# lashhw/rtcuda

Measured on AMD Instinct MI355X. Metric: Msamples/s at 1920x1080, bun_zipper.ply, higher is better.
Workload: dtype f32

## Files before the change

### rtcuda_amd/api.py

```python
from __future__ import annotations

import ctypes
import dataclasses
import os
import subprocess

import numpy as np

from .scenes import SceneArrays

_PKG = os.path.dirname(os.path.abspath(__file__))
LIB_PATH = os.path.join(_PKG, os.environ.get("RT_LIB_NAME", "librtcuda_amd.so"))
CSRC = os.path.join(_PKG, "csrc")

W = 1 << 20
FLAG_TIME_KERNELS = 1
FLAG_DETERMINISTIC = 2
FLAG_RNG_PER_SAMPLE = 4
FLAG_REFERENCE_WALK = 8
SCENE_DEVICE_BVH = 1
FLAG_WATERTIGHT = 16
AOV_CHANNELS = 11
AOV_ALBEDO, AOV_NORMAL, AOV_EMISSION, AOV_DEPTH, AOV_HITS = 0, 3, 6, 9, 10

EXPORTS = [
    "rt_scene_create", "rt_scene_destroy", "rt_scene_info", "rt_scene_build_info", "rt_scene_update", "rt_scene_update_device",
    "rt_scene_refit_info", "rt_scene_create_flags", "rt_scene_rebuild", "rt_scene_rebuild_device", "rt_scene_set_materials",
    "rt_scene_set_lights", "rt_scene_set_triangles", "rt_scene_set_triangles_device", "rt_scene_create_device", "rt_camera_make", "rt_render", "rt_render_multi",
    "rt_render_shard", "rt_render_shard_fixed", "rt_render_rays_device", "rt_render_rays_fixed_device",
    "rt_render_rays_keyed_device", "rt_render_rays_keyed_fixed_device", "rt_post_process", "rt_post_process_fixed", "rt_trace_closest", "rt_trace_any",
    "rt_trace_closest_flags", "rt_trace_any_flags", "rt_query_closest_device", "rt_query_any_device", "rt_query_last_counters",
    "rt_render_aov_fixed", "rt_render_aov_rays_fixed_device", "rt_aov_resolve",
    "rt_denoise_scratch_bytes", "rt_denoise_default_params", "rt_denoise_fixed",
    "rt_denoise_dual_scratch_bytes", "rt_denoise_dual_default_params", "rt_denoise_dual_fixed",
    "rt_render_motion", "rt_temporal_default_params", "rt_temporal_accumulate_fixed",
    "rt_temporal_moments_default_params", "rt_temporal_accumulate_moments_fixed", "rt_denoise_variance_fixed",
    "rt_xorwow_states", "rt_shutdown", "rt_peer_access_log", "rt_last_error", "rt_version", "rt_build_id",
]
TOOLS_LIB_PATH = os.path.join(_PKG, "librtcuda_amd_tools.so")
TOOLS_EXPORTS = ["rt_measure_copy_bandwidth", "rt_calibrate_valu", "rt_calibrate_valu_packed", "rt_probe_issue", "rt_split_probe",
                 "rt_scene_tree_copy", "rt_shade_table", "rt_shade_records", "rt_denoise_pass_time",
                 "rt_denoise_dual_pass_time"]


class RtError(RuntimeError):
    pass


class RtStats(ctypes.Structure):
    _fields_ = [
        ("camera_rays", ctypes.c_int64), ("shade_events", ctypes.c_int64), ("closest_rays", ctypes.c_int64),
        ("any_rays", ctypes.c_int64), ("emission_adds", ctypes.c_int64), ("shadow_adds", ctypes.c_int64),
        ("rr_draws", ctypes.c_int64), ("iterations", ctypes.c_int64), ("bvh_nodes", ctypes.c_int64),
        ("bvh_depth", ctypes.c_int64), ("seconds_render", ctypes.c_double), ("seconds_rng_init", ctypes.c_double),
        ("seconds_trace", ctypes.c_double), ("seconds_reference_tree", ctypes.c_double), ("seconds_advance", ctypes.c_double),
        ("launches_trace", ctypes.c_int64), ("reserved", ctypes.c_int64 * 7),
    ]

    def as_dict(self) -> dict:
        d = {n: getattr(self, n) for n, _ in self._fields_ if n != "reserved"}
        d["lds_top_records"] = int(self.reserved[2])
        d["slot_chunk"] = max((int(self.reserved[1]) & 0xffffffff) - 1, 0)
        d["slot_head"] = int(self.reserved[1]) >> 32
        d["literal_retraces"], d["reference_lost_hits"], d["exact_ties"] = (int(self.reserved[k]) for k in (4, 5, 6))
        return d


class RtDenoiseParams(ctypes.Structure):
    _fields_ = [("passes", ctypes.c_int32), ("sigma_color", ctypes.c_float), ("sigma_depth", ctypes.c_float),
                ("normal_power_log2", ctypes.c_int32), ("flags", ctypes.c_uint32)]


class RtDenoiseDualParams(ctypes.Structure):
    _fields_ = [("passes", ctypes.c_int32), ("sigma_variance", ctypes.c_float), ("sigma_depth", ctypes.c_float),
                ("normal_power_log2", ctypes.c_int32), ("flags", ctypes.c_uint32)]


class RtTemporalParams(ctypes.Structure):
    _fields_ = [("max_history", ctypes.c_int32), ("alpha_min", ctypes.c_float), ("depth_tolerance", ctypes.c_float),
                ("normal_cos_min", ctypes.c_float), ("flags", ctypes.c_uint32)]


class RtTemporalMomentsParams(ctypes.Structure):
    _fields_ = [("max_history", ctypes.c_int32), ("alpha_min", ctypes.c_float), ("depth_tolerance", ctypes.c_float),
                ("normal_cos_min", ctypes.c_float), ("emission_tolerance", ctypes.c_float), ("variance_min_history", ctypes.c_int32),
                ("flags", ctypes.c_uint32)]


def build(verbose: bool = False) -> str:
    out = None if verbose else subprocess.DEVNULL
    subprocess.check_call(["make", "-C", CSRC], stdout=out)
    return LIB_PATH


_lib = None


def _preload_hip_runtime() -> None:
    candidates = []
    try:
        import torch
        candidates.append(os.path.join(os.path.dirname(torch.__file__), "lib", "libamdhip64.so"))
    except ImportError:
        pass
    candidates += ["/opt/rocm/lib/libamdhip64.so", "libamdhip64.so"]
    for c in candidates:
        if os.path.isabs(c) and not os.path.exists(c):
            continue
        try:
            ctypes.CDLL(c, mode=ctypes.RTLD_GLOBAL)
            return
        except OSError:
            continue
    raise ImportError("no HIP runtime (libamdhip64.so) could be loaded")


def lib():
    global _lib
    if _lib is not None:
        return _lib
    if not os.path.exists(LIB_PATH):
        raise ImportError(
            f"{LIB_PATH} not found: the HIP library is the product and there is no fallback. "
            f"Build it with `make -C {CSRC}` (or python -c 'import __graft_entry__ as g; g.build()').")
    _preload_hip_runtime()
    _lib = _bind(ctypes.CDLL(LIB_PATH))
    return _lib


def _bind(L):
    vp, ci, cf = ctypes.c_void_p, ctypes.c_int, ctypes.c_float
    L.rt_last_error.restype = ctypes.c_char_p
    L.rt_version.restype = ctypes.c_char_p
    L.rt_build_id.restype = ctypes.c_char_p
    L.rt_scene_create.argtypes = [vp, ci, vp, vp, vp, ci, vp, ci, ctypes.POINTER(vp)]
    L.rt_scene_destroy.argtypes = [vp]
    L.rt_scene_destroy.restype = None
    L.rt_scene_info.argtypes = [vp, vp]
    L.rt_scene_build_info.argtypes = [vp, ctypes.POINTER(ci), ctypes.POINTER(ctypes.c_double)]
    L.rt_scene_update.argtypes = [vp, vp, ci]
    L.rt_scene_update_device.argtypes = [vp, vp, ci, vp]
    L.rt_scene_refit_info.argtypes = [vp, ctypes.POINTER(ctypes.c_int64), ctypes.POINTER(ctypes.c_double),
                                      ctypes.POINTER(ctypes.c_double)]
    L.rt_scene_create_flags.argtypes = [vp, ci, vp, vp, vp, ci, vp, ci, ctypes.c_uint32, ctypes.POINTER(vp)]
    L.rt_scene_rebuild.argtypes = [vp, vp, ci]
    L.rt_scene_rebuild_device.argtypes = [vp, vp, ci, vp]
    L.rt_scene_set_materials.argtypes = [vp, vp, ci]
    L.rt_scene_set_lights.argtypes = [vp, vp, ci, vp]
    L.rt_scene_set_triangles.argtypes = [vp, vp, ci, vp, vp, vp, ci, vp, ci]
    L.rt_scene_set_triangles_device.argtypes = [vp, vp, ci, vp, vp, vp, ci, vp, ci, vp]
    L.rt_scene_create_device.argtypes = [vp, ci, vp, vp, vp, ci, vp, ci, vp, ctypes.POINTER(vp)]
    L.rt_camera_make.argtypes = [vp, vp, vp, cf, cf, vp]
    L.rt_render.argtypes = [vp, vp, ci, ci, ci, ci, ctypes.c_uint64, ctypes.c_uint32, vp, ctypes.POINTER(RtStats)]
    L.rt_render_multi.argtypes = [vp, vp, ci, ci, ci, ci, ctypes.c_uint64, ctypes.c_uint32, vp, ci, vp, ctypes.POINTER(RtStats)]
    L.rt_render_shard.argtypes = [vp, vp, ci, ci, ci, ci, ctypes.c_uint64, ci, ci, ctypes.c_uint32, vp, vp,
                                  ctypes.POINTER(RtStats)]
    L.rt_post_process.argtypes = [vp, ci, ci, vp]
    L.rt_render_shard_fixed.argtypes = L.rt_render_shard.argtypes
    L.rt_post_process_fixed.argtypes = [vp, vp, ci, ci, vp]
    L.rt_render_rays_device.argtypes = [vp, ctypes.c_int64, vp, vp, vp, ci, ci, ci, ctypes.c_uint64, ctypes.c_uint32, vp, vp,
                                        ctypes.POINTER(RtStats)]
    L.rt_render_rays_fixed_device.argtypes = L.rt_render_rays_device.argtypes
    L.rt_render_rays_keyed_device.argtypes = [vp, ctypes.c_int64, vp, vp, vp, ci, ci, ci, ctypes.c_uint64, ctypes.c_uint64, ctypes.c_uint32,
                                              ctypes.c_uint32, vp, vp, ctypes.POINTER(RtStats)]
    L.rt_render_rays_keyed_fixed_device.argtypes = L.rt_render_rays_keyed_device.argtypes
    L.rt_render_aov_fixed.argtypes = [vp, vp, ci, ci, ci, ctypes.c_uint64, ci, ci, ctypes.c_uint32, vp, vp, vp, ctypes.POINTER(RtStats)]
    L.rt_render_aov_rays_fixed_device.argtypes = [vp, ctypes.c_int64, vp, vp, vp, ci, ci, ctypes.c_uint64, ctypes.c_uint32, ctypes.c_uint32,
                                                  vp, vp, vp, ctypes.POINTER(RtStats)]
    L.rt_aov_resolve.argtypes = [vp, vp, ci, ci, vp]
    L.rt_denoise_scratch_bytes.argtypes = [ci, ci]
    L.rt_denoise_scratch_bytes.restype = ctypes.c_int64
    L.rt_denoise_default_params.argtypes = [ctypes.POINTER(RtDenoiseParams)]
    L.rt_denoise_fixed.argtypes = [vp, ci, vp, ci, ci, ci, ctypes.POINTER(RtDenoiseParams), vp, vp, vp]
    L.rt_denoise_dual_scratch_bytes.argtypes = [ci, ci]
    L.rt_denoise_dual_scratch_bytes.restype = ctypes.c_int64
    L.rt_denoise_dual_default_params.argtypes = [ctypes.POINTER(RtDenoiseDualParams)]
    L.rt_denoise_dual_fixed.argtypes = [vp, ci, vp, ci, vp, ci, ci, ci, ctypes.POINTER(RtDenoiseDualParams), vp, vp, vp]
    L.rt_render_motion.argtypes = [vp, vp, ci, ci, vp, vp, ctypes.c_uint32, vp, vp, ctypes.POINTER(RtStats)]
    L.rt_temporal_default_params.argtypes = [ctypes.POINTER(RtTemporalParams)]
    L.rt_temporal_accumulate_fixed.argtypes = [vp, ci, vp, ci, vp, ci, vp, vp, vp, vp, vp, ci, ci, ci, ctypes.POINTER(RtTemporalParams),
                                               vp, vp, vp, vp]
    L.rt_temporal_moments_default_params.argtypes = [ctypes.POINTER(RtTemporalMomentsParams)]
    L.rt_temporal_accumulate_moments_fixed.argtypes = [vp, ci, vp, ci, vp, ci, vp, vp, vp, vp, vp, ci, vp, vp, ci, ci,
                                                       ctypes.POINTER(RtTemporalMomentsParams), vp, vp, vp, vp, vp, vp]
    L.rt_denoise_variance_fixed.argtypes = [vp, ci, vp, vp, ci, ci, ci, ctypes.POINTER(RtDenoiseDualParams), vp, vp, vp]
    L.rt_trace_closest.argtypes = [vp, ci, vp, vp, vp, vp, vp, vp, vp]
    L.rt_trace_any.argtypes = [vp, ci, vp, vp, vp, vp, vp]
    L.rt_trace_closest_flags.argtypes = [vp, ctypes.c_uint32, ci, vp, vp, vp, vp, vp, vp, vp]
    L.rt_trace_any_flags.argtypes = [vp, ctypes.c_uint32, ci, vp, vp, vp, vp, vp]
    L.rt_query_closest_device.argtypes = [vp, ctypes.c_uint32, ci, vp, vp, vp, vp, vp, vp, vp, vp]
    L.rt_query_any_device.argtypes = [vp, ctypes.c_uint32, ci, vp, vp, vp, vp, vp, vp]
    L.rt_query_last_counters.argtypes = [vp, vp]
    L.rt_xorwow_states.argtypes = [ctypes.c_uint64, ctypes.c_uint32, ctypes.c_uint32, ci, vp, vp]
    L.rt_shutdown.restype = None
    L.rt_peer_access_log.restype = ctypes.c_char_p
    return L


_tools = None


def tools_lib():
    global _tools
    if _tools is not None:
        return _tools
    if not os.path.exists(TOOLS_LIB_PATH):
        raise ImportError(f"{TOOLS_LIB_PATH} not found: build it with `make -C {CSRC}`")
    _preload_hip_runtime()
    L = _bind(ctypes.CDLL(TOOLS_LIB_PATH))
    vp, ci = ctypes.c_void_p, ctypes.c_int
    L.rt_measure_copy_bandwidth.argtypes = [ctypes.c_int64, ci, ctypes.POINTER(ctypes.c_double)]
    L.rt_calibrate_valu.argtypes = [ci, ci, ctypes.POINTER(ctypes.c_double), ctypes.POINTER(ctypes.c_double)]
    L.rt_calibrate_valu_packed.argtypes = [ci, ci, ci, ctypes.POINTER(ctypes.c_double)]
    L.rt_probe_issue.argtypes = [ci, ci, ci, ctypes.POINTER(ctypes.c_double), ctypes.POINTER(ctypes.c_double)]
    L.rt_split_probe.argtypes = [vp, vp, ci, ci, ci, ci, ctypes.c_uint64, ctypes.c_int64, vp, ci]
    L.rt_scene_tree_copy.argtypes = [vp, vp, ctypes.c_int64, vp, ctypes.c_int64, vp]
# ... 913 lines not shown
```

### rtcuda_amd/csrc/rt_device.h

```cpp
#ifndef RT_DEVICE_H
#define RT_DEVICE_H

#include <hip/hip_runtime.h>
#include <stdint.h>

#include "rt_pinned_math.h"

#define RT_DEV __device__ __forceinline__
#ifdef RT_ISA_MARKS
#define RT_MARK(name) __asm__ volatile("; RT_MARK " name)
#else
#define RT_MARK(name)
#endif

namespace rt {

constexpr float kInvPi = 0.31830988618379067153f;
constexpr float kTwoPi = 6.28318530717958647692f;
constexpr int kRrStart = 4;
constexpr float kRrThreshold = 1.f;
constexpr float kFltMax = 3.402823466e+38f;
constexpr float kFltEps = 1.192092896e-07f;

struct V3 {
    float x, y, z;
};
RT_DEV V3 mk(float x, float y, float z) { return V3{x, y, z}; }
RT_DEV V3 neg(V3 a) { return mk(-a.x, -a.y, -a.z); }
RT_DEV V3 add(V3 a, V3 b) { return mk(a.x + b.x, a.y + b.y, a.z + b.z); }
RT_DEV V3 sub(V3 a, V3 b) { return mk(a.x - b.x, a.y - b.y, a.z - b.z); }
RT_DEV V3 mul(V3 a, V3 b) { return mk(a.x * b.x, a.y * b.y, a.z * b.z); }
RT_DEV V3 scale(V3 a, float t) { return mk(a.x * t, a.y * t, a.z * t); }
RT_DEV V3 divf(V3 a, float t) {
    float inv_t = 1.f / t;
    return mk(a.x * inv_t, a.y * inv_t, a.z * inv_t);
}
RT_DEV float dot(V3 a, V3 b) { return a.x * b.x + a.y * b.y + a.z * b.z; }
RT_DEV V3 cross(V3 a, V3 b) {
    return mk(a.y * b.z - a.z * b.y, a.z * b.x - a.x * b.z, a.x * b.y - a.y * b.x);
}
RT_DEV float len2(V3 a) { return a.x * a.x + a.y * a.y + a.z * a.z; }
RT_DEV float len(V3 a) { return sqrtf(a.x * a.x + a.y * a.y + a.z * a.z); }
RT_DEV V3 unit(V3 a) {
    float inv_len = 1.f / len(a);
    return mk(a.x * inv_len, a.y * inv_len, a.z * inv_len);
}
RT_DEV float max3(V3 a) { return fmaxf(fmaxf(a.x, a.y), a.z); }
template <int STEPS = 1>
RT_DEV float rcp_exact_normal(float x) {
    float r = __builtin_amdgcn_rcpf(x);
#pragma unroll
    for (int k = 0; k < STEPS; k++) {
        const float e = fmaf(-x, r, 1.f);
        r = fmaf(e, r, r);
    }
    return r;
}
RT_DEV V3 reflect(V3 v, V3 n) { return sub(v, scale(n, 2.f * dot(v, n))); }
RT_DEV V3 refract4(V3 unit_v, V3 unit_n, float eta_ratio, float cos_theta) {
    V3 v_parallel = scale(add(unit_v, scale(unit_n, cos_theta)), eta_ratio);
    V3 v_perp = scale(unit_n, -sqrtf(1.f - len2(v_parallel)));
    return add(v_parallel, v_perp);
}

struct Rng {
    uint32_t d, v0, v1, v2, v3, v4;
};
RT_DEV uint32_t rng_next(Rng &s) {
    uint32_t t = s.v0 ^ (s.v0 >> 2);
    s.v0 = s.v1;
    s.v1 = s.v2;
    s.v2 = s.v3;
    s.v3 = s.v4;
    s.v4 = (s.v4 ^ (s.v4 << 4)) ^ (t ^ (t << 1));
    s.d += 362437u;
    return s.v4 + s.d;
}
RT_DEV Rng rng_sample_stream(uint32_t seed_lo, uint32_t seed_hi, unsigned long long key) {
    unsigned long long z = (((unsigned long long)seed_hi << 32) | seed_lo) + 0x9E3779B97F4A7C15ull * (key + 1ull);
    z = (z ^ (z >> 30)) * 0xBF58476D1CE4E5B9ull;
    z = (z ^ (z >> 27)) * 0x94D049BB133111EBull;
    z ^= z >> 31;
    const uint32_t s0 = (uint32_t)z ^ 0xaad26b49u, s1 = (uint32_t)(z >> 32) ^ 0xf7dcefddu;
    const uint32_t t0 = 1099087573u * s0, t1 = 2591861531u * s1;
    Rng r;
    r.d = 6615241u + t1 + t0;
    r.v0 = 123456789u + t0;
    r.v1 = 362436069u ^ t0;
    r.v2 = 521288629u + t1;
    r.v3 = 88675123u ^ t1;
    r.v4 = 5783321u + t0;
    return r;
}
RT_DEV float rng_uniform(Rng &s) { return (float)rng_next(s) * 2.3283064e-10f + (2.3283064e-10f / 2.0f); }

struct Tri {
    V3 p0, e1, e2, n;
};
RT_DEV Tri load_tri(const float4 *__restrict__ tris, int k) {
    const float4 *q = (const float4 *)((const char *)tris + __umul24((unsigned)k, 48u));
    float4 a = q[0];
    float4 b = q[1];
    float4 c = q[2];
    Tri t;
    t.p0 = mk(a.x, a.y, a.z);
    t.e1 = mk(a.w, b.x, b.y);
    t.e2 = mk(b.z, b.w, c.x);
    t.n = mk(c.y, c.z, c.w);
    return t;
}
RT_DEV bool tri_intersect(const Tri &tr, V3 o, V3 d, float tmax, float &t_out, float &u_out, float &v_out) {
    V3 c = sub(tr.p0, o);
    V3 r = cross(d, c);
    float inv_det = 1.f / dot(d, tr.n);
    float u = inv_det * dot(tr.e2, r);
    float v = inv_det * dot(tr.e1, r);
    float t = inv_det * dot(c, tr.n);
    t_out = t;
    u_out = u;
    v_out = v;
    return u >= 0.0f && v >= 0.0f && (u + v) <= 1.0f && 0 < t && t <= tmax;
}
RT_DEV V3 tri_point(const Tri &tr, float u, float v) { return add(sub(tr.p0, scale(tr.e1, u)), scale(tr.e2, v)); }
RT_DEV float tri_area(const Tri &tr) { return 0.5f * len(tr.n); }

RT_DEV V3 offset_ray_origin(V3 p, V3 n) {
    const float int_scale = 256.f;
    const float float_scale = 1.f / 65536.f;
    const float origin = 1.f / 32.f;
    int ox = (int)(int_scale * n.x);
    int oy = (int)(int_scale * n.y);
    int oz = (int)(int_scale * n.z);
    float px = __int_as_float(__float_as_int(p.x) + (p.x < 0 ? -ox : ox));
    float py = __int_as_float(__float_as_int(p.y) + (p.y < 0 ? -oy : oy));
    float pz = __int_as_float(__float_as_int(p.z) + (p.z < 0 ? -oz : oz));
    return mk(fabsf(p.x) < origin ? p.x + float_scale * n.x : px,
              fabsf(p.y) < origin ? p.y + float_scale * n.y : py,
              fabsf(p.z) < origin ? p.z + float_scale * n.z : pz);
}
RT_DEV float power_heuristic(float f_pdf, float g_pdf_float) {
    int g = (int)g_pdf_float;
    float f2 = f_pdf * f_pdf;
    return f2 / (f2 + (float)(g * g));
}
RT_DEV bool same_hemisphere(V3 wo, V3 wi, V3 n) { return dot(wo, n) * dot(wi, n) < 0.f; }
RT_DEV V3 uniform_sample_sphere(Rng &rs) {
    float z = 1 - 2 * rng_uniform(rs);
    float r = sqrtf(1 - z * z);
    float phi = kTwoPi * rng_uniform(rs);
    float x, y;
    rt_sincosf(phi, &y, &x);
    return mk(r * x, r * y, z);
}

struct Material {
    float ax, ay, az;
    float ior;
    int type;
};
RT_DEV bool mat_get_f(const Material &m, V3 wo, V3 wi, V3 n, V3 &f, float &pdf) {
    if (m.type == 0) {
        if (same_hemisphere(wo, wi, n)) {
            f = scale(mk(m.ax, m.ay, m.az), kInvPi);
            pdf = dot(wi, n) * kInvPi;
            return true;
        }
    }
    return false;
}
RT_DEV V3 mat_sample_f(const Material &m, V3 wo, Rng &rs, V3 &n, V3 &wi, float &pdf, int &again_draws) {
    again_draws = 0;
    if (m.type == 0 || m.type == 1) {
        if (dot(wo, n) > 0.f) n = neg(n);
        if (m.type == 0) {
            again_draws = 2;
            wi = unit(add(n, uniform_sample_sphere(rs)));
            pdf = dot(wi, n) * kInvPi;
            return scale(mk(m.ax, m.ay, m.az), kInvPi);
        } else {
            wi = reflect(wo, n);
            pdf = 1.f;
            return divf(mk(m.ax, m.ay, m.az), dot(wi, n));
        }
    } else {
        float cos_theta = dot(wo, n);
        bool front = cos_theta < 0.f;
        if (front) cos_theta = -cos_theta;
        float inv_cos = 1.f / cos_theta;
        float eta = front ? 1.f / m.ior : m.ior;
        float sin_theta = sqrtf(1.f - cos_theta * cos_theta);
        bool cannot_refract = eta * sin_theta > 1.f;
        if (cannot_refract) {
            if (!front) n = neg(n);
            wi = reflect(wo, n);
            pdf = 1.f;
            return mk(inv_cos, inv_cos, inv_cos);
        }
        again_draws = 1;
        float r0 = (1 - m.ior) / (1 + m.ior);
        r0 = r0 * r0;
        float reflectance = r0 + (1 - r0) * rt_pow5f(1 - cos_theta);
        if (rng_uniform(rs) < reflectance) {
            if (!front) n = neg(n);
            wi = reflect(wo, n);
            pdf = reflectance;
            float v = pdf * inv_cos;
            return mk(v, v, v);
        } else {
            if (!front) n = neg(n);
            wi = refract4(wo, n, eta, cos_theta);
            n = neg(n);
            pdf = 1.f - reflectance;
            float v = pdf * eta * eta / dot(wi, n);
            return mk(v, v, v);
        }
    }
}
struct Light {
    int type;
    float px, py, pz;
    int tri;
    float lx, ly, lz;
};

struct Camera {
    V3 lookfrom, upper_left, horizontal, vertical;
};
RT_DEV void camera_get_ray(const Camera &c, float x, float y, V3 &o, V3 &d) {
    V3 dir = sub(add(add(c.upper_left, scale(c.horizontal, x)), scale(c.vertical, y)), c.lookfrom);
    o = c.lookfrom;
    d = unit(dir);
}

}
#endif
```

### rtcuda_amd/csrc/rt_frame_kernels.inc

```
#ifndef RT_CHUNK_RELEASE_WAIT
#define RT_CHUNK_RELEASE_WAIT 1
#endif

template <bool LDS_TABLES>
__global__ void __launch_bounds__(kBlock)
RT_K_ADVANCE(DScene sc, DPools p, RT_FRAME_SRC cam, AdvanceParams ap, float *__restrict__ fb, DCounters *__restrict__ ctr,
             DWaveRow *__restrict__ rows, unsigned int *__restrict__ lock_shades) {
    if (ap.lockstep >= 3 && lock_shades[ap.lockstep - 2] == 0u) return;
    __shared__ float s_tab[LDS_TABLES ? kTabDwordsMax : 1];
    const int i = blockIdx.x * blockDim.x + threadIdx.x;
    const bool in_range = i < ap.n;
    SlotState st;
    st.bounces = kDone;
    st.hit_info = -1;
    st.pixel = 0;
    st.gen = 0;
    st.rs = Rng{0, 0, 0, 0, 0, 0};
    st.beta = st.wo = st.isect_p = st.isect_n = mk(0, 0, 0);
    if (in_range) {
        st.bounces = p.bounces(i);
        st.hit_info = p.hit_info(i);
        st.pixel = p.pixel(i);
        st.gen = p.gen(i);
        st.rs = Rng{p.rd(i), p.r0(i), p.r1(i), p.r2(i), p.r3(i), p.r4(i)};
// ... 80 lines not shown
    }
}

template <bool LDS_TABLES, bool WIDE, int MIN_WAVES, bool DRAW_CIDS = false, bool LITERAL = false, bool VERIFY = false>
__global__ void __launch_bounds__(kBlock, MIN_WAVES)
RT_K_PATHS(DScene sc, DPools p, RT_FRAME_SRC cam_arg, AdvanceParams ap_arg, float *__restrict__ fb, DWaveRow *__restrict__ rows,
           int stack_cap, int *overflow, int adv_batch, int debug_no_deposit, unsigned long long *prof, int top_n,
           int prio_period, int rot_wave, int rot_set, int gen_batch, int tri_follow, unsigned int *__restrict__ next_cid,
           unsigned long long *__restrict__ vstat) {
    constexpr bool SPLIT_GEN = MIN_WAVES != 2;
    asm volatile("s_nop 0\n\ts_nop 0");
    extern __shared__ int s_lds[];
    int *stack = s_lds + threadIdx.x;
    float *park = (float *)(s_lds + (stack_cap + 1) * kBlock) + threadIdx.x;
    int *over = overflow + (blockIdx.x * kBlock + threadIdx.x) % kOverStride;
    int *cold = s_lds + (stack_cap + 10) * kBlock + threadIdx.x;
    float *acc = (float *)(s_lds + (stack_cap + 23) * kBlock) + threadIdx.x;
    float *s_tab = (float *)(s_lds + (stack_cap + 26) * kBlock);
    const float *tab = sc.tables;
    const float4 *s_top = (const float4 *)(s_tab + (LDS_TABLES ? ((sc.tab_dwords + 3) & ~3) : 0));
    constexpr bool CHUNKS = RT_PATHS_CHUNKS && SPLIT_GEN && !DRAW_CIDS;
    __shared__ __attribute__((aligned(16))) unsigned s_task[CHUNKS ? 8 : 1];
    __shared__ unsigned s_sem[CHUNKS ? rtchunks::kSemWords : 1];
    const unsigned chunk_g0 = (CHUNKS && top_n > 0) ? (unsigned)top_n & ((1u << rtplan::kChunkHeadShift) - 1u) : 0u;
    const unsigned chunk_head0 = (CHUNKS && top_n > 0) ? (unsigned)top_n >> rtplan::kChunkHeadShift : 0u;
    if (CHUNKS) {
        for (unsigned k = threadIdx.x; k < rtchunks::kSemWords; k += kBlock) s_sem[k] = rtchunks::kSemWordInit;
        if (threadIdx.x == 0) {
            const rtchunks::Multiple m = rtchunks::multiple_of(chunk_g0 ? chunk_g0 : 1u);
            s_task[0] = 0u;
            s_task[1] = chunk_g0;
            s_task[2] = m.inv;
            s_task[3] = m.shift;
            s_task[4] = m.limit;
            s_task[5] = chunk_head0;
        }
    }
    const bool chunk_start = CHUNKS && chunk_g0 && chunk_head0 == 0u;
    if (MIN_WAVES != 2) top_n = 0;
    for (int k = threadIdx.x; k < top_n * 4; k += kBlock) ((float4 *)s_top)[k] = sc.nodes[k];
    if (LDS_TABLES) {
        for (int k = threadIdx.x; k < sc.tab_dwords; k += kBlock) s_tab[k] = sc.tables[k];
        tab = s_tab;
    }
    struct Uniforms {
        RT_FRAME_SRC cam;
        AdvanceParams ap;
    };
    static_assert(sizeof(Uniforms) % 4 == 0, "dword copy");
    Uniforms *s_uni = (Uniforms *)(s_top + 4 * (size_t)top_n);
    {
        Uniforms u;
        u.cam = cam_arg;
        u.ap = ap_arg;
        const int *srcw = (const int *)&u;
        for (int k = threadIdx.x; k < (int)(sizeof(Uniforms) / 4); k += kBlock) ((int *)s_uni)[k] = srcw[k];
    }
    __syncthreads();
    const RT_FRAME_SRC &cam = s_uni->cam;
    const AdvanceParams &ap = s_uni->ap;
    const int ap_n = ap_arg.n, ap_max_bounces = ap_arg.max_bounces, ap_fb_fixed = ap_arg.fb_fixed;
    constexpr bool draw_cids = DRAW_CIDS && SPLIT_GEN;
    int cid_next = 0, cid_end = 0;
    const int lanes_in_grid = (int)(gridDim.x * blockDim.x);
    auto slot_of = [&](int set, unsigned lane_in_wg) {
        return rtchunks::slot_of((unsigned)set, blockIdx.x * blockDim.x + lane_in_wg, (unsigned)lanes_in_grid, (unsigned)rot_wave, (unsigned)rot_set);
    };
    int slot_set = 0;
    int i = slot_of(0, threadIdx.x);
    int bounces = kDone, pixel = 0, gen = 0;
    Rng rs{0, 0, 0, 0, 0, 0};
    V3 beta = mk(0, 0, 0);
    auto load_slot = [&](int k) {
        bounces = p.bounces(k);
        pixel = p.pixel(k);
        gen = p.gen(k);
        rs = Rng{p.rd(k), p.r0(k), p.r1(k), p.r2(k), p.r3(k), p.r4(k)};
        beta = mk(p.br(k), p.bg(k), p.bb(k));
    };
    auto store_slot = [&](int k) {
        p.bounces(k) = bounces;
        p.pixel(k) = pixel;
        p.gen(k) = gen;
        p.hit_info(k) = -1;
        p.stmax(k) = -1.f;
        p.br(k) = beta.x;
        p.bg(k) = beta.y;
        p.bb(k) = beta.z;
        p.rd(k) = rs.d;
        p.r0(k) = rs.v0;
        p.r1(k) = rs.v1;
        p.r2(k) = rs.v2;
        p.r3(k) = rs.v3;
        p.r4(k) = rs.v4;
    };
    auto cold_save = [&]() {
        cold[0 * kBlock] = bounces;
        cold[1 * kBlock] = pixel;
        cold[2 * kBlock] = gen;
        cold[3 * kBlock] = (int)rs.d;
        cold[4 * kBlock] = (int)rs.v0;
        cold[5 * kBlock] = (int)rs.v1;
        cold[6 * kBlock] = (int)rs.v2;
        cold[7 * kBlock] = (int)rs.v3;
        cold[8 * kBlock] = (int)rs.v4;
        cold[9 * kBlock] = __float_as_int(beta.x);
        cold[10 * kBlock] = __float_as_int(beta.y);
        cold[11 * kBlock] = __float_as_int(beta.z);
    };
    auto cold_load = [&]() {
        bounces = cold[0 * kBlock];
        pixel = cold[1 * kBlock];
        gen = cold[2 * kBlock];
        rs = Rng{(uint32_t)cold[3 * kBlock], (uint32_t)cold[4 * kBlock], (uint32_t)cold[5 * kBlock],
                 (uint32_t)cold[6 * kBlock], (uint32_t)cold[7 * kBlock], (uint32_t)cold[8 * kBlock]};
        beta = mk(__int_as_float(cold[9 * kBlock]), __int_as_float(cold[10 * kBlock]), __int_as_float(cold[11 * kBlock]));
    };
    int phase = PH_IDLE;
    int tri = -1;
    V3 o = mk(0, 0, 0), d = mk(0, 0, 0), inv = mk(0, 0, 0);
    float tmax = 0.f, hu = 0.f, hv = 0.f;
    int cur = kEntryDone, sp = 0;
    auto next_slot = [&](int first_phase) {
        cold_load();
        store_slot(i);
        phase = PH_IDLE;
        tri = -1;
        slot_set++;
        i = slot_of(slot_set, threadIdx.x);
        if (i < ap_n) {
            load_slot(i);
            if (bounces != kDone && bounces != kParked) {
                phase = first_phase;
                cold_save();
                cold[12 * kBlock] = -1;
            } else {
                i = ap_n;
            }
        }
    };
    int pend = kEntryDone;
    acc[0 * kBlock] = acc[1 * kBlock] = acc[2 * kBlock] = 0.f;
    if (chunk_start) {
        i = ap_n;
        phase = PH_GEN;
        cold[12 * kBlock] = -1;
    } else if (i < ap_n) {
        load_slot(i);
        phase = (bounces != kDone && bounces != kParked) ? (SPLIT_GEN ? PH_GEN : PH_ADV) : PH_IDLE;
        cold_save();
        cold[12 * kBlock] = -1;
    }
    unsigned long long n_gen = 0, n_shade = 0, n_traced = 0, n_shadow = 0, n_emit = 0, n_deposit = 0, n_rr = 0;
#ifdef RT_TRACE_PROFILE
    unsigned long long pf[16] = {0, 0, 0, 0, 0, 0, 0, 0, 0, 0, 0, 0, 0, 0, 0, 0};
    unsigned long long pf_gen_cycles = 0, pf_fin_cycles = 0, pf_fin_lanes = 0, pf_fin_iters = 0;
    unsigned long long pf_handovers = 0, pf_handover_blocks = 0;
    const unsigned long long pf_t0 = __builtin_readcyclecounter();
    unsigned long long pf_last_work = 0;
#endif

    unsigned prio_tick = 0;
    const unsigned prio_rank = (4u * blockIdx.x) / gridDim.x;
    while (true) {
        RT_MARK("loop.head");
        if (prio_period && (prio_tick++ & ((1u << prio_period) - 1u)) == 0u) {
            unsigned lvl = ((prio_tick >> prio_period) + prio_rank) & 3u;
            lvl = max(lvl, prio_rank >> 1);
            switch (lvl) {
                case 0: __builtin_amdgcn_s_setprio(0); break;
                case 1: __builtin_amdgcn_s_setprio(1); break;
                case 2: __builtin_amdgcn_s_setprio(2); break;
                default: __builtin_amdgcn_s_setprio(3); break;
            }
        }
        bool trav = phase == PH_ANY || phase == PH_CLOSEST;
        bool want_node = trav && cur >= 0;
        bool want_tri = trav && ((cur != kEntryDone && cur < 0) || (kSpeculate && pend != kEntryDone));
        int n_adv = wave_count((phase == PH_ADV));
        const int n_genw = wave_count((phase == PH_GEN));
        int n_node = wave_count((want_node));
        int n_tri = wave_count((want_tri));
        if (n_adv + n_genw + n_node + n_tri == 0) break;
        auto retake = [&]() {
            trav = phase == PH_ANY || phase == PH_CLOSEST;
            want_node = trav && cur >= 0;
            want_tri = trav && ((cur != kEntryDone && cur < 0) || (kSpeculate && pend != kEntryDone));
            n_adv = wave_count((phase == PH_ADV));
            n_node = wave_count((want_node));
            n_tri = wave_count((want_tri));
        };
        const bool run_adv = n_adv > 0 && ((n_adv >= adv_batch && 2 * n_adv >= n_node && 2 * n_adv >= n_tri) || n_node + n_tri == 0);
        if (SPLIT_GEN && !run_adv && n_genw > 0 && (n_genw >= gen_batch || n_node + n_tri == 0)) {
            RT_MARK("gen.begin");
#ifdef RT_TRACE_PROFILE
            pf[12]++; pf[15] += n_genw;
            const unsigned long long pf_tg = __builtin_readcyclecounter();
#endif
            AdvanceOut out;
            out.did_gen = out.new_ray = false;
            out.ray_o = o;
            out.ray_d = d;
            bool hand_back = false;
            long long my_cid = -1;
            if (draw_cids) {
                const unsigned long long m = wave_ballot(phase == PH_GEN);
                const int need = (int)__popcll(m), rank = (int)prefix_popc(m);
                int served = 0;
                while (served < need) {
                    if (cid_next == cid_end) {
                        unsigned base = 0;
                        if (lane_id() == 0) base = atomicAdd(next_cid, (unsigned)kCidChunk);
                        static_assert(0x7ffff000u + (unsigned)kCidChunk < 0x7fffffffu, "cid_end must not overflow int");
                        cid_next = (int)min(__builtin_amdgcn_readfirstlane(base), 0x7ffff000u);
                        cid_end = cid_next + kCidChunk;
                    }
                    const int take = min(need - served, cid_end - cid_next);
                    if (phase == PH_GEN && rank >= served && rank < served + take) my_cid = cid_next + (rank - served);
                    cid_next += take;
                    served += take;
                }
            }
            const unsigned chunk_g = CHUNKS ? __builtin_amdgcn_readfirstlane(s_task[1]) : 0u;
            const bool chunk_was_gen = CHUNKS && phase == PH_GEN;
            const int chunk_acc_pixel = CHUNKS ? cold[1 * kBlock] : 0;
            if (CHUNKS && chunk_g) {
                const rtchunks::Multiple chunk_m{s_task[2], s_task[3], s_task[4]};
                const unsigned chunk_head = __builtin_amdgcn_readfirstlane(s_task[5]);
                bool need = phase == PH_GEN && i >= ap_n;
                const bool at_end = phase == PH_GEN && i < ap_n && slot_set >= (int)chunk_head &&
                                    rtchunks::chunk_ends((unsigned)cold[2 * kBlock], chunk_m, cold[0 * kBlock] == kChunkFresh);
                if (wave_ballot(need || at_end)) {
#ifdef RT_TRACE_PROFILE
                    bool pf_released = false;
#endif
                    if (at_end) {
                        cold_load();
                        const bool ends = gen == ap.last_gen || (long long)gen * kW + (ap.slot_lo + i) >= ap.cam_end;
                        if (!ends) {
                            bounces = ap_max_bounces;
                            store_slot(i);
                            const rtchunks::Owner own = rtchunks::owner_of((unsigned)i, (unsigned)lanes_in_grid, (unsigned)rot_wave, (unsigned)rot_set);
                            const unsigned idx = (own.set - chunk_head) * rtchunks::kLanes + (own.lane_in_grid & (rtchunks::kLanes - 1u));
#if RT_CHUNK_RELEASE_WAIT
                            __builtin_amdgcn_s_waitcnt(0x0f70);
#endif
                            const unsigned old = __hip_atomic_fetch_add(&s_sem[rtchunks::sem_word(idx) & (rtchunks::kSemWords - 1u)], rtchunks::sem_unit(idx),
                                                                        __ATOMIC_RELEASE, __HIP_MEMORY_SCOPE_WORKGROUP);
                            if (!rtchunks::runner_keeps(rtchunks::sem_value(old, idx))) {
                                i = ap_n;
                                need = true;
                            }
#ifdef RT_TRACE_PROFILE
                            pf_released = true;
#endif
                        }
                    }
#ifdef RT_TRACE_PROFILE
                    pf_handovers += wave_count(pf_released);
                    pf_handover_blocks += wave_ballot(pf_released) != 0 ? 1 : 0;
#endif
                    const unsigned chunk_sets = (unsigned)ap_n / (unsigned)lanes_in_grid - chunk_head;
                    const unsigned chunk_tasks = rtchunks::task_count(chunk_sets, (unsigned)ap.last_gen, (unsigned)chunk_g);
                    unsigned long long m;
                    while ((m = wave_ballot(need)) != 0ull) {
                        unsigned base = 0;
                        if (lane_id() == 0) base = atomicAdd(&s_task[0], (unsigned)__popcll(m));
                        const unsigned t = __builtin_amdgcn_readfirstlane(base) + prefix_popc(m);
                        if (need) {
                            if (t >= chunk_tasks) {
                                need = false;
                                phase = PH_IDLE;
                            } else {
                                const rtchunks::Entry e = rtchunks::task_entry(t, chunk_sets);
                                const int k = slot_of((int)(e.set + chunk_head), e.lane);
                                const unsigned idx = e.set * rtchunks::kLanes + e.lane;
                                const unsigned old = k < ap_n ? __hip_atomic_fetch_sub(&s_sem[rtchunks::sem_word(idx) & (rtchunks::kSemWords - 1u)], rtchunks::sem_unit(idx),
                                                                                       __ATOMIC_ACQUIRE, __HIP_MEMORY_SCOPE_WORKGROUP)
                                                              : rtchunks::kSemBias;
                                if (rtchunks::taker_runs(rtchunks::sem_value(old, idx))) {
                                    i = k;
                                    load_slot(i);
                                    cold_save();
                                    cold[0 * kBlock] = kChunkFresh;
                                    cold[12 * kBlock] = -1;
                                    need = false;
                                }
                            }
                        }
                    }
                }
            }
            if (CHUNKS) {
                __builtin_amdgcn_s_waitcnt(0x0f70);
                if (chunk_was_gen) acc_flush(acc, fb, ap_fb_fixed, chunk_acc_pixel);
            }
            if (phase == PH_GEN) {
                SlotState st;
                st.gen = cold[2 * kBlock];
                st.rs = Rng{(uint32_t)cold[3 * kBlock], (uint32_t)cold[4 * kBlock], (uint32_t)cold[5 * kBlock],
                            (uint32_t)cold[6 * kBlock], (uint32_t)cold[7 * kBlock], (uint32_t)cold[8 * kBlock]};
                st.bounces = 0;
                st.pixel = 0;
                st.beta = mk(0, 0, 0);
                int pxy = cold[12 * kBlock];
                if (!CHUNKS) acc_flush(acc, fb, ap_fb_fixed, cold[1 * kBlock]);
                gen_core<true>(cam, ap, ap.slot_lo + i, st, out, &pxy, my_cid);
                cold[0 * kBlock] = st.bounces;
                cold[2 * kBlock] = st.gen;
                cold[3 * kBlock] = (int)st.rs.d;
                cold[4 * kBlock] = (int)st.rs.v0;
                cold[5 * kBlock] = (int)st.rs.v1;
                cold[6 * kBlock] = (int)st.rs.v2;
                cold[7 * kBlock] = (int)st.rs.v3;
                cold[8 * kBlock] = (int)st.rs.v4;
                if (out.new_ray) {
                    cold[1 * kBlock] = st.pixel;
                    cold[9 * kBlock] = __float_as_int(st.beta.x);
                    cold[10 * kBlock] = __float_as_int(st.beta.y);
                    cold[11 * kBlock] = __float_as_int(st.beta.z);
                    cold[12 * kBlock] = pxy;
                } else {
                    hand_back = true;
                }
            }
            const bool nr = out.new_ray;
            o = out.ray_o;
            d = out.ray_d;
            inv = inv_dir(d);
            phase = nr ? (int)PH_CLOSEST : phase;
            tmax = nr ? kFltMax : tmax;
            tri = nr ? -1 : tri;
            cur = nr ? 0 : cur;
            sp = nr ? 0 : sp;
            if (wave_ballot(hand_back)) {
                if (hand_back) {
                    if (draw_cids) {
                        phase = PH_IDLE;
                    } else if (CHUNKS && chunk_g && slot_set + 1 >= (int)s_task[5]) {
                        cold_load();
                        store_slot(i);
                        i = ap_n;
                        tri = -1;
                        slot_set = (int)s_task[5];
                    } else {
                        next_slot(PH_GEN);
                    }
                }
            }
            n_gen += wave_count((out.did_gen));
            n_traced += wave_count((out.new_ray));
#ifdef RT_TRACE_PROFILE
            pf_gen_cycles += __builtin_readcyclecounter() - pf_tg;
#endif
            retake();
            RT_MARK("gen.end");
        }
        if (run_adv) {
#ifdef RT_TRACE_PROFILE
            pf[0]++; pf[1] += n_adv;
            const unsigned long long pf_ta = __builtin_readcyclecounter();
#endif
            RT_MARK("adv.head");
            AdvanceOut out;
            out.did_gen = out.did_shade = out.has_shadow = out.did_emit = out.new_ray = false;
            out.rr_draws = 0;
            if (phase == PH_ADV) {
                cold_load();
                SlotState st;
                st.wo = d;
                st.hit_info = -1;
                st.isect_p = st.isect_n = mk(0, 0, 0);
                if (tri >= 0) {
                    Tri tr = load_tri(sc.tris, tri);
                    float4 sh = sc.tri_shade[(unsigned)tri];
                    RT_MARK("adv.verify");
                    if (VERIFY) {
                        bool bad = (__float_as_uint(hv) >> 31) != 0u;
                        if (bad) atomicAdd(&vstat[V_TIE], 1ull);
                        else bad = !ref_visible(sc, o, d, tr, tri, vstat);
                        if (bad) {
                            atomicAdd(&vstat[V_LITERAL], 1ull);
                            float tm = kFltMax;
                            tri = -1;
                            hu = hv = 0.f;
                            reference_walk<false>(sc, o, d, tm, tri, hu, hv, stack, over, stack_cap);
                            cold_load();
                            if (tri >= 0) {
                                tr = load_tri(sc.tris, tri);
                                sh = sc.tri_shade[(unsigned)tri];
                            }
                        }
                    }
                    RT_MARK("adv.hit_record");
                    if (!VERIFY || tri >= 0) {
                        st.isect_p = tri_point(tr, hu, hv);
                        st.isect_n = mk(sh.x, sh.y, sh.z);
                        st.hit_info = __float_as_int(sh.w);
                    }
                }
                st.bounces = bounces;
                st.pixel = pixel;
                st.gen = gen;
                st.rs = rs;
                st.beta = beta;
                advance_core<SPLIT_GEN, true, true>(sc, tab, cam, ap, ap.slot_lo + i, st, out, fb, acc);
                RT_MARK("adv.tail");
                bounces = st.bounces;
                pixel = st.pixel;
                gen = st.gen;
                rs = st.rs;
                beta = st.beta;
                if (out.has_shadow) {
                    park[0 * kBlock] = out.ray_o.x;
                    park[1 * kBlock] = out.ray_o.y;
                    park[2 * kBlock] = out.ray_o.z;
                    park[3 * kBlock] = out.ray_d.x;
                    park[4 * kBlock] = out.ray_d.y;
                    park[5 * kBlock] = out.ray_d.z;
                    park[6 * kBlock] = out.s_L.x;
                    park[7 * kBlock] = out.s_L.y;
                    park[8 * kBlock] = out.s_L.z;
                    o = out.s_o;
                    d = out.s_d;
                    phase = PH_ANY;
                    tmax = out.s_tmax;
                    tri = out.s_target;
                    hu = 0.f;
                } else if (out.new_ray) {
                    o = out.ray_o;
                    d = out.ray_d;
                    phase = PH_CLOSEST;
                    tmax = kFltMax;
                    tri = -1;
                } else if (SPLIT_GEN) {
                    phase = PH_GEN;
                    tri = -1;
                } else {
                    cold_save();
                    next_slot(PH_ADV);
                }
                if (phase == PH_ANY || phase == PH_CLOSEST) {
                    cur = 0;
                    sp = 0;
                }
                if (phase != PH_IDLE) cold_save();
            }
            inv = inv_dir(d);
            if (!SPLIT_GEN) n_gen += wave_count((out.did_gen));
            n_shade += wave_count((out.did_shade));
            n_traced += wave_count((out.new_ray));
            n_shadow += wave_count((out.has_shadow));
            n_emit += wave_count((out.did_emit));
            int rr = out.rr_draws;
            if (wave_ballot(rr != 0)) {
                for (int off = 32; off > 0; off >>= 1) rr += __shfl_xor(rr, off);
                n_rr += (unsigned long long)rr;
            }
#ifdef RT_TRACE_PROFILE
            pf[8] += __builtin_readcyclecounter() - pf_ta;
#endif
            retake();
            RT_MARK("adv.after");
        }
        const bool is_any = phase == PH_ANY;
        auto node_block = [&](bool want, int n_want) {
#ifdef RT_TRACE_PROFILE
            pf[2]++; pf[3] += n_want; pf[6] += n_adv;
            const unsigned long long pf_tn = __builtin_readcyclecounter();
#endif
            RT_MARK("node.begin");
            if (LITERAL) {
                if (want) {
                    if (is_any) reference_walk<true>(sc, o, d, tmax, tri, hu, hv, stack, over, stack_cap);
                    else reference_walk<false>(sc, o, d, tmax, tri, hu, hv, stack, over, stack_cap);
                    cur = kEntryDone;
                }
            } else if (want) {
                auto step_general = [&]() {
                    if (cur >= 0) {
                        inner_step<WIDE>(sc, o, inv, tmax, cur, sp, stack, over, stack_cap, s_top, top_n);
                    } else if (kSpeculate && cur != kEntryDone && pend == kEntryDone && sp > 0) {
                        pend = cur;
                        cur = stack_pop(stack, over, sp, stack_cap);
                    }
                };
                auto step = [&]() {
                    if (!WIDE || MIN_WAVES == 2) {
                        step_general();
                    } else if (wave_ballot(sp > stack_cap - 3) == 0ull) {
                        if (cur >= 0) {
                            inner_step<WIDE, true>(sc, o, inv, tmax, cur, sp, stack, over, stack_cap);
                        } else if (kSpeculate && cur != kEntryDone && pend == kEntryDone && sp > 0) {
                            pend = cur;
                            sp--;
                            cur = stack[sp * kBlock];
                        }
                    } else {
                        step_general();
                    }
                };
                if (kNodeCont == 0 || !WIDE) {
#pragma unroll
                    for (int rep = 0; rep < (WIDE ? kNodePerStepWide : kNodePerStep); rep++) step();
                } else {
#pragma unroll
                    for (int rep = 0; rep < kNodePerStepWide; rep++) step();
                    if (wave_count(cur >= 0) >= kNodeCont) {
#pragma unroll
                        for (int rep = 0; rep < kNodeExtra; rep++) step();
                    }
                }
            }
#ifdef RT_TRACE_PROFILE
            pf[9] += __builtin_readcyclecounter() - pf_tn;
#endif
            RT_MARK("node.end");
        };
        auto tri_block = [&](bool want, int n_want) {
#ifdef RT_TRACE_PROFILE
            pf[4]++; pf[5] += n_want; pf[7] += n_adv;
            const unsigned long long pf_tt = __builtin_readcyclecounter();
#endif
            RT_MARK("tri.begin");
            if (want) {
                int pd = pend, cu = cur;
                int ks[kTriPerStep] = {};
                bool act[kTriPerStep];
                Tri tr[kTriPerStep];
#pragma unroll
                for (int j = 0; j < kTriPerStep; j++) {
                    const bool fp = kSpeculate && pd != kEntryDone;
                    const bool leaf = cu != kEntryDone && cu < 0;
                    act[j] = fp || leaf;
                    const int enc = fp ? pd : cu;
                    ks[j] = act[j] ? (~enc) >> 3 : ks[0];
                    const bool more = ((~enc) & 7) > 1;
                    const int rest = more ? enc - 7 : kEntryDone;
                    int popped = kEntryDone;
                    if (act[j] && !fp && !more && sp > 0) popped = stack_pop(stack, over, sp, stack_cap);
                    pd = (act[j] && fp) ? rest : pd;
                    cu = (act[j] && !fp) ? (more ? rest : popped) : cu;
                    tr[j] = load_tri(sc.tris, ks[j]);
                }
                bool occluded = false;
                int occ_j = 0;
#pragma unroll
                for (int j = 0; j < kTriPerStep; j++) {
                    if (act[j] && !occluded) {
                        float t, u, v;
                        const bool hit = tri_intersect(tr[j], o, d, tmax, t, u, v);
                        occluded = hit && is_any && ks[j] != tri;
                        occ_j = occluded ? j : occ_j;
                        bool better = hit && !is_any;
                        if (VERIFY) {
                            const bool tie = better && t == tmax && tri >= 0;
                            v = __uint_as_float(__float_as_uint(v) | (tie ? 0x80000000u : 0u));
                        } else if (better && t == tmax && tri >= 0) {
                            better = sc.order[(unsigned)ks[j]] > sc.order[(unsigned)tri];
                        }
                        tmax = better ? t : tmax;
                        hu = occluded ? 1.f : (better ? u : hu);
                        hv = better ? v : hv;
                        tri = better ? ks[j] : tri;
                    }
                }
                pend = occluded ? kEntryDone : pd;
                cur = occluded ? kEntryDone : cu;
                if (VERIFY && occluded) {
                    static_assert(kTriPerStep == 2, "the occluder is picked from two records");
                    Tri tq;
                    tq.p0 = occ_j ? tr[1].p0 : tr[0].p0;
                    tq.e1 = occ_j ? tr[1].e1 : tr[0].e1;
                    tq.e2 = occ_j ? tr[1].e2 : tr[0].e2;
                    tq.n = tq.p0;
                    if (!ref_visible(sc, o, d, tq, occ_j ? ks[1] : ks[0], vstat)) hu = 2.f;
                }
            }
#ifdef RT_TRACE_PROFILE
            pf[10] += __builtin_readcyclecounter() - pf_tt;
#endif
            RT_MARK("tri.end");
        };
        {
            const bool run_node = n_node > 0 && n_node >= n_tri;
            bool w = want_tri;
            int nw = n_tri;
            if (run_node) {
                node_block(want_node, n_node);
                w = tri_follow > 0 && trav && ((cur != kEntryDone && cur < 0) || (kSpeculate && pend != kEntryDone));
                nw = wave_count(w);
                nw = (tri_follow > 0 && nw >= tri_follow) ? nw : 0;
            }
            if (nw > 0) tri_block(w, nw);
        }
        RT_MARK("fin.begin");
        const bool fin = trav && cur == kEntryDone && (!kSpeculate || pend == kEntryDone);
#ifdef RT_TRACE_PROFILE
        const unsigned long long pf_tf = __builtin_readcyclecounter();
        pf_fin_lanes += wave_count(fin);
        pf_fin_iters += wave_ballot(fin) != 0 ? 1 : 0;
#endif
        if (VERIFY) {
            const bool lit = fin && is_any && hu == 2.f;
            if (wave_ballot(lit)) {
                if (lit) {
                    atomicAdd(&vstat[V_LITERAL], 1ull);
                    float tm = tmax, no_v = 0.f;
                    int excluded = tri;
                    hu = 0.f;
                    reference_walk<true>(sc, o, d, tm, excluded, hu, no_v, stack, over, stack_cap);
                }
            }
        }
        n_deposit += wave_count((fin && is_any && hu == 0.f));
        if (fin) {
            if (is_any) {
                if (hu == 0.f && !debug_no_deposit)
                    acc_add(acc, park[6 * kBlock], park[7 * kBlock], park[8 * kBlock]);
                o = mk(park[0 * kBlock], park[1 * kBlock], park[2 * kBlock]);
                d = mk(park[3 * kBlock], park[4 * kBlock], park[5 * kBlock]);
                phase = PH_CLOSEST;
                inv = inv_dir(d);
                tmax = kFltMax;
                tri = -1;
                cur = 0;
                sp = 0;
            } else {
                const int b = cold[0 * kBlock];
                phase = (SPLIT_GEN && (tri < 0 || (b >= ap_max_bounces && b > 0))) ? PH_GEN : PH_ADV;
            }
        }
#ifdef RT_TRACE_PROFILE
        pf_fin_cycles += __builtin_readcyclecounter() - pf_tf;
        pf_last_work = phase != PH_IDLE ? pf_tf - pf_t0 : pf_last_work;
#endif
    }
#ifdef RT_TRACE_PROFILE
    if (prof && lane_id() == 0) { atomicAdd(&prof[17], pf_fin_cycles); atomicAdd(&prof[18], pf_fin_lanes); atomicAdd(&prof[19], pf_fin_iters); }
    const unsigned long long pf_life = __builtin_readcyclecounter() - pf_t0;
    unsigned long long pf_idle = pf_life - pf_last_work, pf_idle_max = pf_idle;
    for (int off = 32; off > 0; off >>= 1) {
        pf_idle += __shfl_xor(pf_idle, off);
        const unsigned long long other = __shfl_xor(pf_idle_max, off);
        pf_idle_max = other > pf_idle_max ? other : pf_idle_max;
    }
    if (prof && lane_id() == 0)
        { pf[11] = pf_life; for (int k = 0; k < 16; k++) atomicAdd(&prof[k], pf[k]); atomicMax(&prof[13], pf[11]); atomicAdd(&prof[14], 1ull); atomicAdd(&prof[16], pf_gen_cycles);
          atomicAdd(&prof[20], pf_idle); atomicAdd(&prof[21], pf_idle_max);
          atomicAdd(&prof[22], pf_handovers); atomicAdd(&prof[23], pf_handover_blocks);
          unsigned long long *rec = prof + 24 + kProfRec * (size_t)((blockIdx.x * kBlock + threadIdx.x) >> 6);
          rec[0] = __builtin_amdgcn_s_getreg((31 << 11) | 4);
          rec[1] = __builtin_amdgcn_s_getreg((31 << 11) | 20);
          rec[2] = pf[11];
          rec[3] = pf[0] + pf[2] + pf[4];
          rec[4] = pf_idle;
          rec[5] = pf_idle_max; }
#endif
    unsigned long long v[C_COUNT] = {n_gen, n_shade, n_traced, n_shadow, n_emit, n_deposit, n_rr, 0ull};
    row_add(rows, v);
}
```

### rtcuda_amd/csrc/rt_host_check.cpp

```cpp
#include <cfloat>
#include <cmath>
#include <cstdint>
#include <cstdio>
#include <cstring>
#include <cstdlib>
#include <vector>

#include "rt_bvh.h"
#include "rt_denoise.h"
#include "rt_launch_plan.h"
#include "rt_ploc.h"
#include "rt_ref_tree.h"
#include "rt_slot_chunks.h"
#include "rt_stats_merge.h"
#include "rt_temporal.h"

namespace {
struct V3 { float x, y, z; };
inline V3 sub(V3 a, V3 b) { return {a.x - b.x, a.y - b.y, a.z - b.z}; }
inline float dot(V3 a, V3 b) { return a.x * b.x + a.y * b.y + a.z * b.z; }
inline V3 cross(V3 a, V3 b) { return {a.y * b.z - a.z * b.y, a.z * b.x - a.x * b.z, a.x * b.y - a.y * b.x}; }
struct Tri { V3 p0, e1, e2, n; };
inline bool tri_hit(const Tri &tr, V3 o, V3 d, float tmax, float &t) {
    V3 c = sub(tr.p0, o);
    V3 r = cross(d, c);
    float inv_det = 1.f / dot(d, tr.n);
    float u = inv_det * dot(tr.e2, r);
    float v = inv_det * dot(tr.e1, r);
    if (u >= 0.0f && v >= 0.0f && (u + v) <= 1.0f) {
        float tt = inv_det * dot(c, tr.n);
        if (0 < tt && tt <= tmax) { t = tt; return true; }
    }
    return false;
}
inline bool box_hit(V3 o, V3 inv, const float *lo, const float *hi, float tmax, float &entry) {
    float ax = (lo[0] - o.x) * inv.x, bx = (hi[0] - o.x) * inv.x;
    float ay = (lo[1] - o.y) * inv.y, by = (hi[1] - o.y) * inv.y;
    float az = (lo[2] - o.z) * inv.z, bz = (hi[2] - o.z) * inv.z;
    float t_in = fmaxf(fmaxf(fminf(ax, bx), fminf(ay, by)), fminf(az, bz));
    float t_out = fminf(fminf(fmaxf(ax, bx), fmaxf(ay, by)), fmaxf(az, bz));
    entry = t_in;
    t_out = t_out * 1.000001f;
    return t_in <= t_out && t_out >= 0.f && t_in <= tmax * rtbvh::kCullTmaxWiden;
}
inline bool box_hit_fma(V3 o, V3 inv, const float *lo, const float *hi, float tmax, float &entry) {
    const float sx = -o.x * inv.x, sy = -o.y * inv.y, sz = -o.z * inv.z;
    float ax = fmaf(lo[0], inv.x, sx), bx = fmaf(hi[0], inv.x, sx);
    float ay = fmaf(lo[1], inv.y, sy), by = fmaf(hi[1], inv.y, sy);
    float az = fmaf(lo[2], inv.z, sz), bz = fmaf(hi[2], inv.z, sz);
    float t_in = fmaxf(fmaxf(fminf(ax, bx), fminf(ay, by)), fminf(az, bz));
    float t_out = fminf(fminf(fmaxf(ax, bx), fmaxf(ay, by)), fmaxf(az, bz));
    entry = t_in;
    t_out = t_out * 1.000001f;
    return fmaxf(t_in, 0.f) <= fminf(t_out, fminf(tmax * rtbvh::kCullTmaxWiden, FLT_MAX));
}
inline V3 inv_dir(V3 d) {
    auto clampinv = [](float x) { return 1.f / ((fabsf(x) < rtbvh::kCullDirFloor) ? copysignf(rtbvh::kCullDirFloor, x) : x); };
    return V3{clampinv(d.x), clampinv(d.y), clampinv(d.z)};
}
std::vector<Tri> leaf_order_triangles(const float *verts, const rtbvh::Result &r, int n) {
    std::vector<Tri> tris(n);
    for (int k = 0; k < n; k++) {
        const float *q = verts + 9 * (size_t)r.order[k];
        V3 p0{q[0], q[1], q[2]}, p1{q[3], q[4], q[5]}, p2{q[6], q[7], q[8]};
        tris[k].p0 = p0; tris[k].e1 = sub(p0, p1); tris[k].e2 = sub(p2, p0); tris[k].n = cross(tris[k].e1, tris[k].e2);
    }
    return tris;
}

struct WalkResult {
    int best = -1;
    float t = 0.f;
    bool occluded = false;
    long long nodes = 0, tris = 0, leaves = 0;
    int max_sp = 0;
    long long sp_hist[32] = {0};
    bool failed = false;
    bool unseen_occluder = false;
    float tie_t = -1.f;
    long long own_fail = 0, leaf_fail = 0;
};

struct RefSlab {
    bool nx, ny, nz;
    V3 inv, so;
    bool neg_zero;
};
inline bool is_neg_zero(float x) { uint32_t b; memcpy(&b, &x, 4); return b == 0x80000000u; }
inline RefSlab ref_slab(V3 o, V3 d) {
    RefSlab s;
    s.nx = d.x < 0; s.ny = d.y < 0; s.nz = d.z < 0;
    auto refinv = [](float x) { return 1.f / ((fabsf(x) < FLT_EPSILON) ? copysignf(FLT_EPSILON, x) : x); };
    s.inv = V3{refinv(d.x), refinv(d.y), refinv(d.z)};
    s.so = V3{(-o.x) * s.inv.x, (-o.y) * s.inv.y, (-o.z) * s.inv.z};
    s.neg_zero = is_neg_zero(d.x) || is_neg_zero(d.y) || is_neg_zero(d.z);
    return s;
}
inline bool ref_box(const RefSlab &s, const float *b, float &entry) {
    const float ex = s.inv.x * b[s.nx ? 1 : 0] + s.so.x;
    const float ey = s.inv.y * b[s.ny ? 3 : 2] + s.so.y;
    const float ez = s.inv.z * b[s.nz ? 5 : 4] + s.so.z;
    entry = fmaxf(ex, fmaxf(ey, ez));
    const float xx = s.inv.x * b[s.nx ? 0 : 1] + s.so.x;
    const float xy = s.inv.y * b[s.ny ? 2 : 3] + s.so.y;
    const float xz = s.inv.z * b[s.nz ? 4 : 5] + s.so.z;
    return entry <= fminf(xx, fminf(xy, xz));
}
struct RefView {
    rtref::Tree tree;
    std::vector<int> leaf_of;
    std::vector<int> parent;
    bool root_leaf = true;
};
inline void own_box(const Tri &tr, float *b) {
    const V3 p1 = sub(tr.p0, tr.e1), p2{tr.p0.x + tr.e2.x, tr.p0.y + tr.e2.y, tr.p0.z + tr.e2.z};
    b[0] = fminf(tr.p0.x, fminf(p1.x, p2.x)); b[1] = fmaxf(tr.p0.x, fmaxf(p1.x, p2.x));
    b[2] = fminf(tr.p0.y, fminf(p1.y, p2.y)); b[3] = fmaxf(tr.p0.y, fmaxf(p1.y, p2.y));
    b[4] = fminf(tr.p0.z, fminf(p1.z, p2.z)); b[5] = fmaxf(tr.p0.z, fmaxf(p1.z, p2.z));
}
inline bool ref_visible(const RefView &rv, const RefSlab &s, const Tri &tr, int caller_index, WalkResult &w) {
    float b[6], e;
    own_box(tr, b);
    if (ref_box(s, b, e) && !s.neg_zero) return true;
    w.own_fail++;
    if (rv.root_leaf) return true;
    int node = rv.leaf_of[(size_t)caller_index];
    bool vis = ref_box(s, rv.tree.nodes[(size_t)node].box.b, e);
    if (vis && s.neg_zero)
        for (node = rv.parent[(size_t)node]; vis && node > 0; node = rv.parent[(size_t)node])
            vis = ref_box(s, rv.tree.nodes[(size_t)node].box.b, e);
    if (!vis) w.leaf_fail++;
    return vis;
}
WalkResult walk_ray(const std::vector<rtbvh::Pair> &rec, bool wide, const std::vector<Tri> &tris, const std::vector<int32_t> &order,
                    int stack_entries, int mode, V3 o, V3 d, float tmax, int excl, const RefView *rv = nullptr) {
    WalkResult w;
    RefSlab slab{};
    if (rv) slab = ref_slab(o, d);
    std::vector<int> stack(stack_entries + 8);
    const V3 inv = inv_dir(d);
    int sp = 0, cur = tris.empty() ? rtbvh::kNoChild : 0;
    long long steps = 0;
    float t;
    while (cur != rtbvh::kNoChild && !w.occluded) {
        if (++steps > 1000000) { w.failed = true; break; }
        if (cur >= 0) {
            w.nodes++;
            w.sp_hist[sp < 31 ? sp : 31]++;
            const float *boxes[4];
            int links[4];
            int nk = 0;
            for (int half = 0; half < (wide ? 2 : 1); half++) {
                const rtbvh::Pair &p = rec[cur + half];
                boxes[nk] = p.lbox; links[nk++] = p.llink;
                boxes[nk] = p.rbox; links[nk++] = p.rlink;
            }
            float e[4];
            bool h[4];
            for (int k = 0; k < nk; k++)
                h[k] = (wide ? box_hit_fma(o, inv, boxes[k], boxes[k] + 3, tmax, e[k]) : box_hit(o, inv, boxes[k], boxes[k] + 3, tmax, e[k])) &&
// ... 589 lines not shown
    for (int k = 0; k < 32; k++) {
        out32[k] = g_sp_hist[k];
        if (reset) g_sp_hist[k] = 0;
    }
}
void rt_hostwalk_stats(long long *out4, int reset) {
    for (int k = 0; k < 4; k++) {
        out4[k] = g_walk_stats[k];
        if (reset) g_walk_stats[k] = 0;
    }
}
int rt_hostwalk_trace(void *h, int mode, int n_rays, const float *o3, const float *d3, const float *tmax_in, const int *excluded,
                      int *out_i, float *out_t) {
    const HostWalk &w = *(const HostWalk *)h;
    const rtbvh::Result &r = w.r;
    const std::vector<rtbvh::Pair> padded = w.wide ? padded_quads(r, n_rays, o3) : std::vector<rtbvh::Pair>();
    const std::vector<rtbvh::Pair> &rec = w.wide ? padded : r.pairs;
    const int stack_entries = w.wide ? r.stack_bound : r.pair_depth + 1;
    int failures = 0;
    long long st_nodes = 0, st_tris = 0, st_leaves = 0;
#pragma omp parallel for schedule(dynamic, 1024) reduction(+ : failures, st_nodes, st_tris, st_leaves)
    for (int i = 0; i < n_rays; i++) {
        V3 o{o3[3 * i], o3[3 * i + 1], o3[3 * i + 2]}, d{d3[3 * i], d3[3 * i + 1], d3[3 * i + 2]};
        const int excl = (mode == 1 && excluded[i] >= 0 && excluded[i] < w.n) ? w.inverse[excluded[i]] : -1;
        WalkResult res = walk_ray(rec, w.wide, w.tris, r.order, stack_entries, mode, o, d, tmax_in[i], excl);
        failures += res.failed ? 1 : 0;
        st_nodes += res.nodes; st_tris += res.tris; st_leaves += res.leaves;
#pragma omp critical
        for (int k = 0; k < 32; k++) g_sp_hist[k] += res.sp_hist[k];
        if (mode == 1) {
            out_i[i] = res.occluded ? 1 : 0;
        } else {
            out_i[i] = res.best >= 0 ? r.order[res.best] : -1;
            out_t[i] = res.t;
        }
    }
    g_walk_stats[0] += n_rays;
    g_walk_stats[1] += st_nodes;
    g_walk_stats[2] += st_tris;
    g_walk_stats[3] += st_leaves;
    return failures;
}
int rt_hostwalk_trace_verified(void *h, int mode, int n_rays, const float *o3, const float *d3, const float *tmax_in,
                               const int *excluded, int *out_i, float *out_t, long long *stats6) {
    const HostWalk &w = *(const HostWalk *)h;
    const rtbvh::Result &r = w.r;
    const std::vector<rtbvh::Pair> padded = w.wide ? padded_quads(r, n_rays, o3) : std::vector<rtbvh::Pair>();
    const std::vector<rtbvh::Pair> &rec = w.wide ? padded : r.pairs;
    const int stack_entries = w.wide ? r.stack_bound : r.pair_depth + 1;
    int failures = 0;
    long long own = 0, leafb = 0, ties = 0, negz = 0, lit = 0;
#pragma omp parallel for schedule(dynamic, 1024) reduction(+ : failures, own, leafb, ties, negz, lit)
    for (int i = 0; i < n_rays; i++) {
        V3 o{o3[3 * i], o3[3 * i + 1], o3[3 * i + 2]}, d{d3[3 * i], d3[3 * i + 1], d3[3 * i + 2]};
        const int excl = (mode == 1 && excluded[i] >= 0 && excluded[i] < w.n) ? w.inverse[excluded[i]] : -1;
        const RefSlab s = ref_slab(o, d);
        WalkResult res;
        negz += s.neg_zero ? 1 : 0;
        if (mode == 1) {
            res = walk_ray(rec, w.wide, w.tris, r.order, stack_entries, 1, o, d, tmax_in[i], excl, &w.ref);
            if (res.unseen_occluder) {
                lit++;
                const bool failed = res.failed;
                const long long of = res.own_fail, lf = res.leaf_fail;
                literal_walk(w, 1, o, d, tmax_in[i], excl, res);
                res.failed = failed; res.own_fail = of; res.leaf_fail = lf;
            }
        } else {
            res = walk_ray(rec, w.wide, w.tris, r.order, stack_entries, 0, o, d, tmax_in[i], -1);
            if (res.best >= 0) {
                const bool tie = res.tie_t == res.t;
                const bool seen = ref_visible(w.ref, s, w.tris[(size_t)res.best], r.order[(size_t)res.best], res);
                ties += tie ? 1 : 0;
                if (tie || !seen) {
                    lit++;
                    const bool failed = res.failed;
                    literal_walk(w, 0, o, d, tmax_in[i], -1, res);
                    res.failed = failed;
                }
            }
        }
        failures += res.failed ? 1 : 0;
        own += res.own_fail; leafb += res.leaf_fail;
        if (mode == 1) {
            out_i[i] = res.occluded ? 1 : 0;
        } else {
            out_i[i] = res.best >= 0 ? r.order[res.best] : -1;
            out_t[i] = res.t;
        }
    }
    if (stats6) { stats6[0] += n_rays; stats6[1] += own; stats6[2] += leafb; stats6[3] += ties; stats6[4] += negz; stats6[5] += lit; }
    return failures;
}
int rt_ref_tree_export(const float *tri9, int n, float *bounds6, int *count, int *link, int *prims, int *depth) {
    const rtref::Tree t = rtref::build(tri9, n);
    if (depth) *depth = t.depth;
    if (bounds6) {
        for (size_t i = 0; i < t.nodes.size(); i++) {
            memcpy(bounds6 + 6 * i, t.nodes[i].box.b, 24);
            count[i] = t.nodes[i].count;
            link[i] = t.nodes[i].link;
        }
        for (size_t i = 0; i < t.prims.size(); i++) prims[i] = t.prims[i];
    }
    return (int)t.nodes.size();
}
void rt_plan_paths_launch(int n, int cus, int wide, int n_nodes, int paths_cap, int lattice, int width, int spp, int64_t fixed_lds_bytes, int64_t *out10) {
    const rtplan::PathsLaunch p = rtplan::plan_paths_launch(n, cus, wide != 0, n_nodes, paths_cap, lattice != 0, width, spp, (size_t)fixed_lds_bytes);
    const int64_t v[10] = {p.blocks, p.few_blocks, (int64_t)p.lds_bytes, p.top_n, p.adv_batch, p.gen_batch, p.tri_follow, p.prio_rotate, p.rot_wave, p.rot_set};
    memcpy(out10, v, sizeof(v));
}
void rt_slot_chunk_tasks(int block, int sets, int lanes_in_grid, int rot_wave, int rot_set, uint32_t t0, int count, int32_t *slots, int32_t *levels) {
    for (int k = 0; k < count; k++) {
        const rtchunks::Entry e = rtchunks::task_entry(t0 + (uint32_t)k, (unsigned)sets);
        slots[k] = rtchunks::slot_of(e.set, (unsigned)block * rtchunks::kLanes + e.lane, (unsigned)lanes_in_grid, (unsigned)rot_wave, (unsigned)rot_set);
        levels[k] = (int32_t)e.level;
    }
}
int rt_slot_chunk_static_slot(int set, int lane_in_grid, int lanes_in_grid, int rot_wave, int rot_set) {
    return rtchunks::slot_of((unsigned)set, (unsigned)lane_in_grid, (unsigned)lanes_in_grid, (unsigned)rot_wave, (unsigned)rot_set);
}
uint32_t rt_slot_chunk_levels(uint32_t rays, uint32_t G) { return rtchunks::levels(rays, G); }
uint32_t rt_slot_chunk_task_count(uint32_t sets, uint32_t rays, uint32_t G) { return rtchunks::task_count(sets, rays, G); }
int rt_slot_chunk_ends(uint32_t gen, uint32_t G, int fresh) { return rtchunks::chunk_ends(gen, rtchunks::multiple_of(G), fresh != 0); }
int rt_slot_chunk_taker_runs(int old_sem) { return rtchunks::taker_runs(old_sem); }
int rt_slot_chunk_runner_keeps(int old_sem) { return rtchunks::runner_keeps(old_sem); }
int rt_plan_slot_chunk(int n, int cus, int chain) {
    return rtplan::slot_chunk_for(rtplan::plan_paths_launch(n, cus, true, 70000, 10, true, 1920, 256, 0), chain);
}
int rt_plan_slot_head(int n, int cus, int *sets_out) {
    const rtplan::PathsLaunch p = rtplan::plan_paths_launch(n, cus, true, 70000, 10, true, 1920, 256, 0);
    const int sets = n / (p.blocks * rtplan::kBlock);
    if (sets_out) *sets_out = sets;
    return rtplan::slot_head_for(p, sets);
}
int rt_plan_slot_chunk_if_resident(int chunk, int workgroups_per_cu) { return rtplan::slot_chunk_if_resident(chunk, workgroups_per_cu); }
void rt_slot_chunk_head_tasks(int block, int sets, int head, int lanes_in_grid, int rot_wave, int rot_set, uint32_t t0, int count, int32_t *slots, int32_t *levels, int32_t *idx) {
    for (int k = 0; k < count; k++) {
        const rtchunks::Entry e = rtchunks::task_entry(t0 + (uint32_t)k, (unsigned)(sets - head));
        slots[k] = rtchunks::slot_of(e.set + (unsigned)head, (unsigned)block * rtchunks::kLanes + e.lane, (unsigned)lanes_in_grid, (unsigned)rot_wave, (unsigned)rot_set);
        levels[k] = (int32_t)e.level;
        idx[k] = (int32_t)(e.set * rtchunks::kLanes + e.lane);
    }
}
void rt_slot_chunk_owner(int slot, int lanes_in_grid, int rot_wave, int rot_set, int32_t *out2) {
    const rtchunks::Owner o = rtchunks::owner_of((unsigned)slot, (unsigned)lanes_in_grid, (unsigned)rot_wave, (unsigned)rot_set);
    out2[0] = (int32_t)o.set;
    out2[1] = (int32_t)o.lane_in_grid;
}
uint32_t rt_slot_chunk_sem_word(uint32_t idx) { return rtchunks::sem_word(idx); }
uint32_t rt_slot_chunk_sem_unit(uint32_t idx) { return rtchunks::sem_unit(idx); }
int rt_slot_chunk_sem_value(uint32_t word, uint32_t idx) { return rtchunks::sem_value(word, idx); }
uint32_t rt_slot_chunk_sem_init() { return rtchunks::kSemWordInit; }
int hc_denoise(const int64_t *sum_fixed, int num_samples, const int64_t *aov_fixed, int aov_samples, int width, int height, int passes,
               float sigma_color, float sigma_depth, int normal_power_log2, float *rgb_out) {
    if (!sum_fixed || !aov_fixed || !rgb_out || width < 1 || height < 1 || num_samples < 1 || aov_samples < 1) return 1;
    if (passes < 0 || passes > DN_MAX_PASSES || normal_power_log2 < 0 || normal_power_log2 > DN_MAX_NORMAL_POWER_LOG2) return 1;
    if (!(std::isfinite(sigma_color) && sigma_color > 0.f && std::isfinite(sigma_depth) && sigma_depth > 0.f)) return 1;
    const float sc2 = sigma_color * sigma_color, sd2 = sigma_depth * sigma_depth;
    const float kz = 1.f / sd2;
    float kc[DN_MAX_PASSES];
    for (int i = 0; i < passes; i++) {
        kc[i] = (float)(1 << (2 * i)) / sc2;
        if (!(std::isfinite(kc[i]) && kc[i] > 0.f)) return 1;
    }
    if (!(std::isfinite(kz) && kz > 0.f)) return 1;
    const size_t n = (size_t)width * (size_t)height;
    const float inv_spp = 1.f / (float)num_samples, inv_aov = 1.f / (float)aov_samples;
    std::vector<DnPixel> px(n);
    std::vector<float> uv(4 * n, 0.f);
    for (size_t p = 0; p < n; p++) {
        dn_prepare(sum_fixed + 3 * p, aov_fixed + DN_AOV_CHANNELS * p, inv_spp, inv_aov, &px[p]);
        for (int k = 0; k < 3; k++) uv[4 * p + k] = px[p].u[k];
    }
    dn_walk<false>(uv, px, width, height, passes, kc, kz, normal_power_log2);
    for (size_t p = 0; p < n; p++) dn_finish(&uv[4 * p], px[p].d, px[p].e, rgb_out + 3 * p);
    return 0;
}
void hc_expnegf(const float *x, float *y, int n) {
    for (int k = 0; k < n; k++) y[k] = rt_expnegf(x[k]);
}
int hc_denoise_dual(const int64_t *sum_a, int samples_a, const int64_t *sum_b, int samples_b, const int64_t *aov_fixed, int aov_samples,
                    int width, int height, int passes, float sigma_variance, float sigma_depth, int normal_power_log2, float *rgb_out,
                    float *var_out) {
    if (!sum_a || !sum_b || !aov_fixed || !rgb_out || width < 1 || height < 1 || samples_a < 1 || samples_b < 1 || aov_samples < 1) return 1;
    if ((long long)samples_a + samples_b > 0x7fffffffll) return 1;
    if (passes < 0 || passes > DN_MAX_PASSES || normal_power_log2 < 0 || normal_power_log2 > DN_MAX_NORMAL_POWER_LOG2) return 1;
    if (!(std::isfinite(sigma_variance) && sigma_variance > 0.f && std::isfinite(sigma_depth) && sigma_depth > 0.f)) return 1;
    const float ks = sigma_variance * sigma_variance, sd2 = sigma_depth * sigma_depth;
    const float kz = 1.f / sd2;
    if (!(std::isfinite(ks) && ks > 0.f && std::isfinite(kz) && kz > 0.f)) return 1;
    const int ns = samples_a + samples_b;
    const float kv = (float)((double)samples_a * (double)samples_b / ((double)ns * (double)ns));
    const float inv_a = 1.f / (float)samples_a, inv_b = 1.f / (float)samples_b, inv_n = 1.f / (float)ns, inv_aov = 1.f / (float)aov_samples;
    const size_t n = (size_t)width * (size_t)height;
    std::vector<DnPixel> px(n);
    std::vector<float> uv(4 * n);
    for (size_t p = 0; p < n; p++) {
        uv[4 * p + 3] = dn_prepare_dual(sum_a + 3 * p, sum_b + 3 * p, aov_fixed + DN_AOV_CHANNELS * p, inv_a, inv_b, inv_n, inv_aov, kv, &px[p]);
        for (int k = 0; k < 3; k++) uv[4 * p + k] = px[p].u[k];
    }
    const float k[DN_MAX_PASSES] = {ks, ks, ks, ks, ks, ks, ks, ks};
    dn_walk<true>(uv, px, width, height, passes, k, kz, normal_power_log2);
    for (size_t p = 0; p < n; p++) {
        dn_finish(&uv[4 * p], px[p].d, px[p].e, rgb_out + 3 * p);
        if (var_out) var_out[p] = uv[4 * p + 3];
    }
    return 0;
}
int hc_motion_records(int n, const int32_t *tri, const float *u, const float *v, const float *prev_tris, int n_tris, const float *prev_cam12,
                      int width, int height, float *motion4) {
    if (n < 0 || !tri || !u || !v || !prev_tris || !prev_cam12 || !motion4 || width < 1 || height < 1) return 1;
    for (int p = 0; p < n; p++)
        if (tri[p] >= n_tris) return 1;
    TmCamera c;
    tm_camera(prev_cam12, width, height, &c);
    for (int p = 0; p < n; p++) {
        float *rec = motion4 + 4 * (size_t)p;
        const int32_t k = tri[p] < 0 ? -1 : tri[p];
        rec[0] = rec[1] = rec[2] = 0.f;
        if (k >= 0) {
            float P[3];
            tm_point_of_vertices(prev_tris + 9 * (size_t)k, u[p], v[p], P);
            tm_project(&c, P, rec);
        }
        memcpy(rec + 3, &k, 4);
    }
    return 0;
}
int hc_temporal_accumulate(const int64_t *sum_a, int samples_a, const int64_t *sum_b, int samples_b, const int64_t *aov_fixed, int aov_samples,
                           const float *motion4, const int64_t *hist_a_in, const int64_t *hist_b_in, const int32_t *len_in,
                           const int64_t *prev_aov_fixed, int prev_aov_samples, int width, int height, int max_history, float alpha_min,
                           float depth_tolerance, float normal_cos_min, int64_t *hist_a_out, int64_t *hist_b_out, int32_t *len_out) {
    if (!sum_a || !aov_fixed || !motion4 || !hist_a_out || !len_out || width < 1 || height < 1 || samples_a < 1 || aov_samples < 1) return 1;
    const bool two = sum_b != nullptr, history = hist_a_in != nullptr;
    if (two != (hist_b_out != nullptr) || (two && samples_b < 1)) return 1;
    if (!history && (hist_b_in || len_in || prev_aov_fixed)) return 1;
    if (history && (!len_in || !prev_aov_fixed || prev_aov_samples < 1 || two != (hist_b_in != nullptr))) return 1;
    if (max_history < 1 || !(alpha_min > 0.f && alpha_min <= 1.f) || !(std::isfinite(depth_tolerance) && depth_tolerance > 0.f)) return 1;
    if (!(normal_cos_min >= -1.f && normal_cos_min <= 1.f)) return 1;
    const float inv_a = 1.f / (float)samples_a, inv_b = two ? 1.f / (float)samples_b : 0.f, inv_aov = 1.f / (float)aov_samples;
    const float inv_prev = history ? 1.f / (float)prev_aov_samples : 0.f;
    for (int y = 0; y < height; y++)
        for (int x = 0; x < width; x++)
            tm_accumulate_pixel(x, y, width, height, sum_a, inv_a, sum_b, inv_b, aov_fixed, inv_aov, motion4 + 4 * ((size_t)y * width + x), hist_a_in,
                                hist_b_in, len_in, prev_aov_fixed, inv_prev, max_history, alpha_min, depth_tolerance, normal_cos_min, hist_a_out,
                                hist_b_out, len_out);
    return 0;
}
int hc_temporal_accumulate_moments(const int64_t *sum_a, int samples_a, const int64_t *sum_b, int samples_b, const int64_t *aov_fixed,
                                   int aov_samples, const float *motion4, const int64_t *hist_a_in, const int64_t *hist_b_in,
                                   const int32_t *len_in, const int64_t *prev_aov_fixed, int prev_aov_samples, const float *prev_motion4,
                                   const float *moments_in, int width, int height, int max_history, float alpha_min, float depth_tolerance,
                                   float normal_cos_min, float emission_tolerance, int variance_min_history, int64_t *hist_a_out,
                                   int64_t *hist_b_out, int32_t *len_out, float *moments_out, float *variance_out) {
    if (!sum_a || !aov_fixed || !motion4 || !hist_a_out || !len_out || width < 1 || height < 1 || samples_a < 1 || aov_samples < 1) return 1;
    const bool two = sum_b != nullptr, history = hist_a_in != nullptr, moments = moments_out != nullptr;
    if (two != (hist_b_out != nullptr) || (two && samples_b < 1)) return 1;
    if (!history && (hist_b_in || len_in || prev_aov_fixed || moments_in || prev_motion4)) return 1;
    if (history && (!len_in || !prev_aov_fixed || prev_aov_samples < 1 || two != (hist_b_in != nullptr))) return 1;
    if (moments != (variance_out != nullptr) || (moments_in && !moments)) return 1;
    if (moments && two && (long long)samples_a + samples_b > 0x7fffffffll) return 1;
    if (max_history < 1 || !(alpha_min > 0.f && alpha_min <= 1.f) || !(std::isfinite(depth_tolerance) && depth_tolerance > 0.f)) return 1;
    if (!(normal_cos_min >= -1.f && normal_cos_min <= 1.f) || !(emission_tolerance >= 0.f) || variance_min_history < 1) return 1;
    TmMoments t{};
    t.sum_a = sum_a, t.sum_b = sum_b, t.aov = aov_fixed, t.hist_a_in = hist_a_in, t.hist_b_in = hist_b_in, t.prev_aov = prev_aov_fixed;
    t.motion = motion4, t.prev_motion = prev_motion4, t.moments_in = moments_in, t.len_in = len_in;
    t.out_a = hist_a_out, t.out_b = hist_b_out, t.len_out = len_out, t.moments_out = moments_out, t.variance_out = variance_out;
    t.width = width, t.height = height, t.tiles_x = 0;
    t.max_history = max_history, t.variance_min_history = variance_min_history;
    t.use_emission = emission_tolerance <= 3.402823466e+38f;
    t.inv_a = 1.f / (float)samples_a;
    t.inv_b = two ? 1.f / (float)samples_b : 0.f;
    t.inv_n = 1.f / (float)(two && moments ? samples_a + samples_b : samples_a);
    t.inv_aov = 1.f / (float)aov_samples;
    t.inv_prev_aov = history ? 1.f / (float)prev_aov_samples : 0.f;
    t.alpha_min = alpha_min, t.depth_tolerance = depth_tolerance, t.normal_cos_min = normal_cos_min, t.emission_tolerance = emission_tolerance;
    for (int y = 0; y < height; y++)
        for (int x = 0; x < width; x++) tm_accumulate_moments_pixel(&t, x, y, motion4 + 4 * ((size_t)y * width + x));
    return 0;
}
int hc_denoise_variance(const int64_t *sum_fixed, int num_samples, const float *variance, const int64_t *aov_fixed, int aov_samples, int width,
                        int height, int passes, float sigma_variance, float sigma_depth, int normal_power_log2, float *rgb_out, float *var_out) {
    if (!sum_fixed || !variance || !aov_fixed || !rgb_out || width < 1 || height < 1 || num_samples < 1 || aov_samples < 1) return 1;
    if (passes < 0 || passes > DN_MAX_PASSES || normal_power_log2 < 0 || normal_power_log2 > DN_MAX_NORMAL_POWER_LOG2) return 1;
    if (!(std::isfinite(sigma_variance) && sigma_variance > 0.f && std::isfinite(sigma_depth) && sigma_depth > 0.f)) return 1;
    const float ks = sigma_variance * sigma_variance, sd2 = sigma_depth * sigma_depth;
    const float kz = 1.f / sd2;
    if (!(std::isfinite(ks) && ks > 0.f && std::isfinite(kz) && kz > 0.f)) return 1;
    const float inv_spp = 1.f / (float)num_samples, inv_aov = 1.f / (float)aov_samples;
    const size_t n = (size_t)width * (size_t)height;
    std::vector<DnPixel> px(n);
    std::vector<float> uv(4 * n);
    for (size_t p = 0; p < n; p++) {
        uv[4 * p + 3] = dn_prepare_var(sum_fixed + 3 * p, aov_fixed + DN_AOV_CHANNELS * p, variance[p], inv_spp, inv_aov, &px[p]);
        for (int k = 0; k < 3; k++) uv[4 * p + k] = px[p].u[k];
    }
    const float k[DN_MAX_PASSES] = {ks, ks, ks, ks, ks, ks, ks, ks};
    dn_walk<true>(uv, px, width, height, passes, k, kz, normal_power_log2);
    for (size_t p = 0; p < n; p++) {
        dn_finish(&uv[4 * p], px[p].d, px[p].e, rgb_out + 3 * p);
        if (var_out) var_out[p] = uv[4 * p + 3];
    }
    return 0;
}
void hc_merge_shard_stats(const rt_stats *sub, int n, int sub_shards, rt_stats *out) { *out = merge_shard_stats(sub, n, sub_shards != 0); }
// ... 2 lines not shown
```

### rtcuda_amd/csrc/rt_host_render.inc

```
struct Context {
    int device = -1;
    int n = 0;
    int lane = 0;
    DPools pools{};
    std::vector<void *> allocs;
    DCounters *d_ctr = nullptr;
    DCounters *h_ctr = nullptr;
    DWaveRow *d_rows = nullptr;
    int n_rows = 0;
    uint32_t *d_jump = nullptr;
    hipEvent_t ev_ring[4] = {nullptr, nullptr, nullptr, nullptr};
    hipEvent_t ev_a = nullptr, ev_b = nullptr, ev_c = nullptr;
    uint64_t rng_seed = 0;
    int rng_lo = -1;
    bool rng_valid = false;
    uint32_t *rng_backup = nullptr;
    std::vector<hipEvent_t> timing_events;
    unsigned int *d_lock = nullptr;
    int lock_cap = 0;
    int *d_over = nullptr;
    int over_levels = 0;
    std::mutex busy;
    Context() = default;
    Context(const Context &) = delete;
    Context &operator=(const Context &) = delete;
    ~Context() {
        int saved = 0;
        const bool hop = device >= 0 && hipGetDevice(&saved) == hipSuccess && saved != device && hipSetDevice(device) == hipSuccess;
        for (void *q : allocs) (void)hipFree(q);
        (void)hipFree(d_lock);
        (void)hipFree(d_over);
        if (h_ctr) (void)hipHostFree(h_ctr);
        for (hipEvent_t e : ev_ring) if (e) (void)hipEventDestroy(e);
        for (hipEvent_t e : {ev_a, ev_b, ev_c}) if (e) (void)hipEventDestroy(e);
        for (hipEvent_t e : timing_events) (void)hipEventDestroy(e);
        if (hop) (void)hipSetDevice(saved);
    }
};
std::mutex g_ctx_mutex;
std::vector<std::unique_ptr<Context>> g_contexts;

struct OutBuffer {
    int device = -1, slot = 0;
    void *ptr = nullptr;
    size_t bytes = 0;
};
constexpr int kMaxDevices = 64;
std::mutex g_dev_busy[kMaxDevices];
std::mutex g_out_mutex;
std::vector<OutBuffer> g_out_buffers;
void *out_buffer(int device, int slot, size_t bytes) {
    std::lock_guard<std::mutex> list_lock(g_out_mutex);
    for (OutBuffer &b : g_out_buffers)
        if (b.device == device && b.slot == slot) {
            if (b.bytes >= bytes) return b.ptr;
            (void)hipFree(b.ptr);
            b.ptr = nullptr;
            b.bytes = 0;
            if (hipMalloc(&b.ptr, bytes) != hipSuccess) return nullptr;
            b.bytes = bytes;
            return b.ptr;
        }
    OutBuffer b;
    b.device = device;
    b.slot = slot;
    if (hipMalloc(&b.ptr, bytes) != hipSuccess) return nullptr;
    b.bytes = bytes;
    g_out_buffers.push_back(b);
    return b.ptr;
}

void shutdown_impl() {
    int saved = 0;
    const bool have = hipGetDevice(&saved) == hipSuccess;
    {
        std::lock_guard<std::mutex> lock(g_ctx_mutex);
        g_contexts.clear();
    }
    {
        std::lock_guard<std::mutex> list_lock(g_out_mutex);
        for (OutBuffer &b : g_out_buffers) {
            if (hipSetDevice(b.device) == hipSuccess) (void)hipFree(b.ptr);
        }
        g_out_buffers.clear();
    }
    if (have) (void)hipSetDevice(saved);
}

template <typename T>
int dev_alloc(Context &c, T *&ptr, size_t count) {
    void *raw = nullptr;
    HIP_TRY(hipMalloc(&raw, count * sizeof(T)));
    c.allocs.push_back(raw);
    ptr = (T *)raw;
    return 0;
}

int get_context(int n, int lane, Context **out) {
    int dev = 0;
    HIP_TRY(hipGetDevice(&dev));
    std::lock_guard<std::mutex> lock(g_ctx_mutex);
    for (auto &c : g_contexts)
        if (c->device == dev && c->n == n && c->lane == lane) {
            *out = c.get();
            return 0;
        }
    auto c = std::make_unique<Context>();
    c->device = dev;
    c->n = n;
    c->lane = lane;
    DPools &p = c->pools;
    p.n = n;
    if (dev_alloc(*c, p.base, (size_t)A_COUNT * n)) return 1;
    if (dev_alloc(*c, c->rng_backup, (size_t)6 * n)) return 1;
    if (dev_alloc(*c, c->d_ctr, 1)) return 1;
    c->n_rows = ((n + kBlock - 1) / kBlock) * (kBlock / 64);
    if (dev_alloc(*c, c->d_rows, (size_t)c->n_rows)) return 1;
    if (dev_alloc(*c, c->d_jump, (size_t)20 * 800)) return 1;
    HIP_TRY(hipMemcpy(c->d_jump, jump_powers().data(), sizeof(uint32_t) * 20 * 800, hipMemcpyHostToDevice));
    HIP_TRY(hipHostMalloc((void **)&c->h_ctr, sizeof(DCounters) * 4, hipHostMallocDefault));
    for (auto &e : c->ev_ring) HIP_TRY(hipEventCreate(&e));
    HIP_TRY(hipEventCreate(&c->ev_a));
    HIP_TRY(hipEventCreate(&c->ev_b));
    HIP_TRY(hipEventCreate(&c->ev_c));
    *out = c.get();
    g_contexts.push_back(std::move(c));
    return 0;
}

int grid_for(int n) { return (n + kBlock - 1) / kBlock; }

static int lds_stack_cap(const rt_scene *scene, int limit) {
    int cap = std::min(limit, std::max(1, scene->stack_bound));
    if (const char *e = knob("RT_STACK_CAP")) cap = std::max(1, std::min(cap, atoi(e)));
    return cap;
}

using AdvanceKernel = decltype(&k_advance<false>);
using TraceKernel = decltype(&k_trace<false>);
using PathsKernel = decltype(&k_paths<false, false, 4, false, false, false>);

static AdvanceKernel advance_kernel(bool lds_tables) { return lds_tables ? k_advance<true> : k_advance<false>; }

static TraceKernel trace_kernel(bool literal, bool verify, bool wide) {
    if (literal) return k_trace<false, true>;
    if (verify) return wide ? k_trace<true, false, true> : k_trace<false, false, true>;
    return wide ? k_trace<true> : k_trace<false>;
}

template <bool LDS_TABLES, bool WIDE>
static PathsKernel paths_kernel_of(bool few_blocks, bool per_sample, bool literal, bool verify) {
    if (literal) return few_blocks ? k_paths<LDS_TABLES, false, 2, false, true, false> : k_paths<LDS_TABLES, false, 4, false, true, false>;
    if (per_sample && !few_blocks) return k_paths<LDS_TABLES, WIDE, 4, true, false, false>;
    if (few_blocks) return verify ? k_paths<LDS_TABLES, WIDE, 2, false, false, true> : k_paths<LDS_TABLES, WIDE, 2, false, false, false>;
    return verify ? k_paths<LDS_TABLES, WIDE, 4, false, false, true> : k_paths<LDS_TABLES, WIDE, 4, false, false, false>;
}
template <bool LDS_TABLES, bool WIDE>
static PathsKernel paths_chunked_kernel_of(bool literal, bool verify) {
    if (literal) return k_paths_chunked<LDS_TABLES, false, 4, false, true, false>;
    return verify ? k_paths_chunked<LDS_TABLES, WIDE, 4, false, false, true> : k_paths_chunked<LDS_TABLES, WIDE, 4, false, false, false>;
}
static PathsKernel paths_chunked_kernel(bool lds_tables, bool wide, bool literal, bool verify) {
    if (lds_tables) return (wide ? paths_chunked_kernel_of<true, true> : paths_chunked_kernel_of<true, false>)(literal, verify);
    return (wide ? paths_chunked_kernel_of<false, true> : paths_chunked_kernel_of<false, false>)(literal, verify);
}
static PathsKernel paths_kernel(bool lds_tables, bool wide, bool few_blocks, bool per_sample, bool literal, bool verify) {
    if (lds_tables) return (wide ? paths_kernel_of<true, true> : paths_kernel_of<true, false>)(few_blocks, per_sample, literal, verify);
    return (wide ? paths_kernel_of<false, true> : paths_kernel_of<false, false>)(few_blocks, per_sample, literal, verify);
}

using AdvanceRaysKernel = decltype(&k_advance_rays<false>);
using PathsRaysKernel = decltype(&k_paths_rays<false, true, 4, false, false, false>);
static AdvanceRaysKernel advance_rays_kernel(bool lds_tables) { return lds_tables ? k_advance_rays<true> : k_advance_rays<false>; }
template <bool LDS_TABLES>
static PathsRaysKernel paths_rays_kernel_of(bool few_blocks, bool verify) {
    if (few_blocks) return verify ? k_paths_rays<LDS_TABLES, true, 2, false, false, true> : k_paths_rays<LDS_TABLES, true, 2, false, false, false>;
    return verify ? k_paths_rays<LDS_TABLES, true, 4, false, false, true> : k_paths_rays<LDS_TABLES, true, 4, false, false, false>;
}
static PathsRaysKernel paths_rays_kernel(bool lds_tables, bool few_blocks, bool verify) {
    return (lds_tables ? paths_rays_kernel_of<true> : paths_rays_kernel_of<false>)(few_blocks, verify);
}

using PathsKeyedKernel = decltype(&k_paths_keyed<false, true, 4, true, false, false>);
static PathsKeyedKernel paths_keyed_kernel(bool lds_tables, bool few_blocks) {
    if (few_blocks) return lds_tables ? k_paths_keyed<true, true, 2, false, false, false> : k_paths_keyed<false, true, 2, false, false, false>;
    return lds_tables ? k_paths_keyed<true, true, 4, true, false, false> : k_paths_keyed<false, true, 4, true, false, false>;
}

int ensure_overflow(int *&ptr, int &have_levels, int levels) {
    levels = std::max(levels, 1);
    if (ptr && have_levels >= levels) return 0;
    if (ptr) {
        HIP_TRY(hipDeviceSynchronize());
        (void)hipFree(ptr);
        ptr = nullptr;
        have_levels = 0;
    }
    HIP_TRY(hipMalloc((void **)&ptr, sizeof(int) * (size_t)levels * kOverStride));
    have_levels = levels;
    return 0;
}

int ensure_rng(Context &c, uint64_t seed, int slot_lo, hipStream_t st, double *seconds) {
    const size_t bytes = sizeof(uint32_t) * (size_t)c.n;
    uint32_t *parts[6];
    for (int k = 0; k < 6; k++) parts[k] = (uint32_t *)c.pools.array(A_RD + k);
    *seconds = 0.0;
    if (!(c.rng_valid && c.rng_seed == seed && c.rng_lo == slot_lo)) {
        HIP_TRY(hipEventRecord(c.ev_a, st));
        hipLaunchKernelGGL(k_rng_init, dim3(grid_for(c.n)), dim3(kBlock), 0, st, c.pools, c.n, slot_lo,
                           xorwow_seed(seed), c.d_jump);
        HIP_TRY(hipGetLastError());
        for (int k = 0; k < 6; k++)
            HIP_TRY(hipMemcpyAsync(c.rng_backup + (size_t)k * c.n, parts[k], bytes, hipMemcpyDeviceToDevice, st));
        HIP_TRY(hipEventRecord(c.ev_b, st));
        HIP_TRY(hipEventSynchronize(c.ev_b));
        float ms = 0.f;
        HIP_TRY(hipEventElapsedTime(&ms, c.ev_a, c.ev_b));
        *seconds = ms * 1e-3;
        c.rng_valid = true;
        c.rng_seed = seed;
        c.rng_lo = slot_lo;
    } else {
        for (int k = 0; k < 6; k++)
            HIP_TRY(hipMemcpyAsync(parts[k], c.rng_backup + (size_t)k * c.n, bytes, hipMemcpyDeviceToDevice, st));
    }
    return 0;
}

struct RayFrame {
    RayTable table;
    long long n_rays;
    bool keyed = false;
    KeyedRayTable keyed_table{};
};
struct FrameRun {
    Context &c;
    const rt_scene *scene;
    const RayFrame *rays;
    hipStream_t st;
    float *d_sum;
    uint32_t flags;
    bool per_sample;
    HitMode mode;
    bool lds_tables = false, persistent = true, finished = false, ran_lockstep = false;
    int cus = 0, stack_cap = 0, top_records_in_lds = 0, slot_chunk = 0, slot_head = 0, lock_enqueued = 0;
    DScene sc{};
    Camera cam{};
    AdvanceParams ap{};
    TraceParams tpp{};
    size_t lds_bytes = 0, ev_used = 0;
    dim3 grid_trace;
    TraceKernel trace = nullptr;
    hipEvent_t ev_start = nullptr, ev_stop = nullptr;
    long long rounds = 0;
    float ms_paths = 0.f;
    double rng_seconds = 0.0, ref_tree_seconds = 0.0;
    ~FrameRun() {
        if (ev_start) (void)hipEventDestroy(ev_start);
        if (ev_stop) (void)hipEventDestroy(ev_stop);
    }
    void launch_advance() {
        const dim3 grid(grid_for(ap.n)), block(kBlock);
        if (rays) hipLaunchKernelGGL(advance_rays_kernel(lds_tables), grid, block, 0, st, sc, c.pools, rays->table, ap, d_sum, c.d_ctr, c.d_rows, c.d_lock);
        else hipLaunchKernelGGL(advance_kernel(lds_tables), grid, block, 0, st, sc, c.pools, cam, ap, d_sum, c.d_ctr, c.d_rows, c.d_lock);
    }
    void launch_trace() { hipLaunchKernelGGL(trace, grid_trace, dim3(kBlock), lds_bytes, st, sc, c.pools, tpp, stack_cap, c.d_over); }
    int run_persistent(), run_rounds(), run_lockstep(), frame_stats(rt_stats *stats);
    int next_event(hipEvent_t *out) {
        if (ev_used == c.timing_events.size()) {
            hipEvent_t e;
            HIP_TRY(hipEventCreate(&e));
            c.timing_events.push_back(e);
        }
        *out = c.timing_events[ev_used++];
        return 0;
    }
};

#ifdef RT_TRACE_PROFILE
static int report_paths_profile(unsigned long long *paths_prof, int paths_blocks) {
    unsigned long long h[24];
    HIP_TRY(hipMemcpy(h, paths_prof, 192, hipMemcpyDeviceToHost));
    fprintf(stderr, "k_paths cycles: ADV %.1f%% (%.0f / block) node %.1f%% (%.0f) tri %.1f%% (%.0f) rest %.1f%%\n",
            100.0 * h[8] / h[11], h[0] ? (double)h[8] / h[0] : 0.0, 100.0 * h[9] / h[11], h[2] ? (double)h[9] / h[2] : 0.0,
            100.0 * h[10] / h[11], h[4] ? (double)h[10] / h[4] : 0.0, 100.0 * (double)(h[11] - h[8] - h[9] - h[10]) / h[11]);
    fprintf(stderr, "k_paths GEN blocks: %llu avg lanes %.1f, %.1f %% of wave time (%.0f cycles / block; inside `rest` above)\n", h[12],
            h[12] ? (double)h[15] / h[12] : 0.0, 100.0 * h[16] / h[11], h[12] ? (double)h[16] / h[12] : 0.0);
    fprintf(stderr, "k_paths GEN cycles per wave %.0f; chunked deal: %.2f hand-overs per lane, made in %.2f %% of the GEN blocks\n", h[14] ? (double)h[16] / h[14] : 0.0,
            h[14] ? (double)h[22] / (64.0 * h[14]) : 0.0, h[12] ? 100.0 * h[23] / h[12] : 0.0);
    fprintf(stderr, "k_paths waves: %llu, mean lifetime %.0f cycles, longest %.0f cycles (x%.3f)\n", h[14], (double)h[11] / h[14], (double)h[13],
            (double)h[13] * h[14] / h[11]);
    fprintf(stderr, "k_paths lane-idle tail: %.2f %% of wave time x 64 lanes; a wave's first lane is idle for good %.2f %% of the wave's time before its exit\n",
            100.0 * h[20] / (64.0 * h[11]), 100.0 * h[21] / h[11]);
    fprintf(stderr, "k_paths fin section: %.1f %% of wave time, entered in %llu iterations (avg %.1f finished lanes), %.0f cycles each\n",
            100.0 * h[17] / h[11], h[19], h[19] ? (double)h[18] / h[19] : 0.0, h[19] ? (double)h[17] / h[19] : 0.0);
    fprintf(stderr, "k_paths profile: ADV blocks %llu avg lanes %.1f | node steps %llu avg lanes %.1f (ADV-waiting %.1f) | tri steps %llu avg lanes %.1f (ADV-waiting %.1f)\n",
            h[0], h[0] ? (double)h[1] / h[0] : 0.0, h[2], h[2] ? (double)h[3] / h[2] : 0.0, h[2] ? (double)h[6] / h[2] : 0.0, h[4],
            h[4] ? (double)h[5] / h[4] : 0.0, h[4] ? (double)h[7] / h[4] : 0.0);
    if (const char *dump = knob("RT_PROF_DUMP")) {
        std::vector<unsigned long long> recs(kProfRec * (size_t)paths_blocks * (kBlock / 64));
        HIP_TRY(hipMemcpy(recs.data(), paths_prof + 24, recs.size() * 8, hipMemcpyDeviceToHost));
        if (FILE *f = fopen(dump, "w")) {
            for (size_t k = 0; k < recs.size(); k += kProfRec)
                fprintf(f, "%zu %llu %llu %llu %llu %llu %llu\n", k / kProfRec, recs[k], recs[k + 1], recs[k + 2], recs[k + 3], recs[k + 4], recs[k + 5]);
            fclose(f);
        }
    }
    (void)hipFree(paths_prof);
    return 0;
}
static int report_trace_profile(unsigned long long *d_prof) {
    unsigned long long h[16];
    HIP_TRY(hipMemcpy(h, d_prof, sizeof(h), hipMemcpyDeviceToHost));
    fprintf(stderr, "trace profile: waves %llu outer_it %llu refills %llu | inner_it %llu avg_lanes %.1f | leaf_it %llu avg_lanes %.1f | "
                    "tri_it %llu avg_lanes %.1f | active lanes at loop top %.1f | finalised lanes per refill %.1f\n",
            h[10], h[0], h[1], h[2], h[2] ? (double)h[3] / h[2] : 0.0, h[4], h[4] ? (double)h[5] / h[4] : 0.0, h[6],
            h[6] ? (double)h[7] / h[6] : 0.0, h[0] ? (double)h[8] / h[0] : 0.0, h[1] ? (double)h[9] / h[1] : 0.0);
    (void)hipFree(d_prof);
    return 0;
}
#endif

int FrameRun::run_persistent() {
    const int paths_cap = lds_stack_cap(scene, kPathsLdsStack);
    const size_t fixed_lds = (lds_tables ? sizeof(float) * (size_t)((scene->tab_dwords + 3) & ~3) : 0) + sizeof(Camera) + sizeof(AdvanceParams);
    const rtplan::PathsLaunch p = rtplan::plan_paths_launch(c.n, cus, scene->wide, scene->n_nodes, paths_cap, !rays, ap.width, ap.spp, fixed_lds);
    top_records_in_lds = p.top_n;
    unsigned long long *paths_prof = nullptr;
#ifdef RT_TRACE_PROFILE
    const size_t prof_bytes = 192 + 8 * kProfRec * (size_t)(grid_for(c.n) * (kBlock / 64));
    HIP_TRY(hipMalloc((void **)&paths_prof, prof_bytes));
    HIP_TRY(hipMemset(paths_prof, 0, prof_bytes));
#endif
    auto launch_paths = [&](auto kernel, const auto &src, int top_n) {
        hipLaunchKernelGGL(kernel, dim3(p.blocks), dim3(kBlock), p.lds_bytes, st, sc, c.pools, src, ap, d_sum, c.d_rows, paths_cap, c.d_over,
                           p.adv_batch, (flags & 0x100u) ? 1 : 0, paths_prof, top_n, p.prio_rotate, p.rot_wave, p.rot_set, p.gen_batch, p.tri_follow, &c.d_ctr->pad2[0],
                           &c.d_ctr->vstat[0]);
    };
    HIP_TRY(hipEventRecord(c.ev_a, st));
    int chunk = (rays || p.few_blocks || per_sample || ap.last_gen < 1 || ap.n != c.n) ? 0 : rtplan::slot_chunk_for(p, ap.last_gen);
    const PathsKernel chunked = paths_chunked_kernel(lds_tables, scene->wide, mode.literal, mode.verify);
    if (chunk > 0) {
        int per_cu = 0;
        HIP_TRY(hipOccupancyMaxActiveBlocksPerMultiprocessor(&per_cu, chunked, kBlock, p.lds_bytes));
        chunk = rtplan::slot_chunk_if_resident(chunk, per_cu);
    }
    slot_head = chunk > 0 ? rtplan::slot_head_for(p, ap.n / (p.blocks * kBlock)) : 0;
    static_assert(rtplan::kDealtSetsMax == (int)rtchunks::kDealtSetsMax, "the plan deals what the semaphores hold");
    slot_chunk = chunk;
    if (rays && rays->keyed) launch_paths(paths_keyed_kernel(lds_tables, p.few_blocks), rays->keyed_table, p.top_n);
    else if (rays) launch_paths(paths_rays_kernel(lds_tables, p.few_blocks, mode.verify), rays->table, p.top_n);
    else if (chunk > 0) launch_paths(chunked, cam, chunk | (slot_head << rtplan::kChunkHeadShift));
    else launch_paths(paths_kernel(lds_tables, scene->wide, p.few_blocks, per_sample, mode.literal, mode.verify), cam, mode.literal ? 0 : p.top_n);
    HIP_TRY(hipGetLastError());
    HIP_TRY(hipEventRecord(c.ev_b, st));
    HIP_TRY(hipEventSynchronize(c.ev_b));
    HIP_TRY(hipEventElapsedTime(&ms_paths, c.ev_a, c.ev_b));
#ifdef RT_TRACE_PROFILE
    if (report_paths_profile(paths_prof, p.blocks)) return 1;
#endif
    finished = true;
    return 0;
}

int FrameRun::run_rounds() {
    const int kBatch = 8;
    const int kTimeStride = 4;
    const bool time_kernels = (flags & RT_FLAG_TIME_KERNELS) != 0;
    const long long generations = (ap.cam_end + kW - 1) / kW;
    const long long max_rounds = (generations + 1) * (long long)(ap.max_bounces + 2) + 64;
    int batch = 0;
    while (!finished && rounds < max_rounds) {
        for (int k = 0; k < kBatch; k++) {
            ap.round = (int)(rounds & 0x3fffffff);
            const bool timed = time_kernels && (rounds % kTimeStride) == 0;
            hipEvent_t e0 = nullptr, e1 = nullptr, e2 = nullptr, e3 = nullptr;
            if (timed && (next_event(&e0) || next_event(&e1) || next_event(&e2) || next_event(&e3))) return 1;
            if (timed) HIP_TRY(hipEventRecord(e0, st));
            launch_advance();
            if (timed) HIP_TRY(hipEventRecord(e1, st));
            launch_trace();
            if (timed) HIP_TRY(hipEventRecord(e2, st));
            if (timed) HIP_TRY(hipEventRecord(e3, st));
            rounds++;
        }
        HIP_TRY(hipGetLastError());
        HIP_TRY(hipMemcpyAsync(&c.h_ctr[batch & 3], c.d_ctr, sizeof(DCounters), hipMemcpyDeviceToHost, st));
        HIP_TRY(hipEventRecord(c.ev_ring[batch & 3], st));
        if (batch >= 1) {
            int prev = (batch - 1) & 3;
            HIP_TRY(hipEventSynchronize(c.ev_ring[prev]));
            if ((long long)c.h_ctr[prev].last_live_round < (long long)batch * kBatch - 1) finished = true;
        }
        batch++;
    }
    return 0;
}

int FrameRun::run_lockstep() {
    const int n_lock = ap.max_bounces + 2;
    ran_lockstep = finished && !per_sample;
    if (!ran_lockstep) return 0;
    if (n_lock > c.lock_cap) {
        HIP_TRY(hipStreamSynchronize(st));
        (void)hipFree(c.d_lock);
        c.d_lock = nullptr;
        c.lock_cap = 0;
        HIP_TRY(hipMalloc((void **)&c.d_lock, sizeof(unsigned) * (size_t)std::max(n_lock, 64)));
        c.lock_cap = std::max(n_lock, 64);
    }
    HIP_TRY(hipMemsetAsync(c.d_lock, 0, sizeof(unsigned) * (size_t)n_lock, st));
    while (lock_enqueued < n_lock) {
        const int hi = std::min(n_lock, lock_enqueued + kLockChunk);
        for (int j = lock_enqueued; j < hi; j++) {
            ap.round = (int)((rounds + j) & 0x3fffffff);
            ap.lockstep = 1 + j;
            launch_advance();
            tpp.lock_shades = c.d_lock;
            tpp.lock_round = j;
            launch_trace();
        }
        HIP_TRY(hipGetLastError());
        lock_enqueued = hi;
        if (hi < n_lock) {
            unsigned last = 1u;
            HIP_TRY(hipMemcpyAsync(&last, c.d_lock + (hi - 1), sizeof(unsigned), hipMemcpyDeviceToHost, st));
            HIP_TRY(hipStreamSynchronize(st));
            if (last == 0u && hi - 1 >= 1) break;
        }
    }
    return 0;
}

int FrameRun::frame_stats(rt_stats *stats) {
    if (ran_lockstep) {
        std::vector<unsigned> h_lock((size_t)lock_enqueued);
        HIP_TRY(hipMemcpy(h_lock.data(), c.d_lock, sizeof(unsigned) * (size_t)lock_enqueued, hipMemcpyDeviceToHost));
        int ran = lock_enqueued;
        for (int j = 1; j < lock_enqueued; j++)
            if (h_lock[(size_t)j] == 0u) {
                ran = j + 1;
                break;
            }
        rounds += ran;
    }
#ifdef RT_TRACE_PROFILE
    if (report_trace_profile(tpp.prof)) return 1;
#endif
    float ms_total = 0.f;
    HIP_TRY(hipEventElapsedTime(&ms_total, ev_start, ev_stop));
    DCounters h_final{};
    HIP_TRY(hipMemcpy(&h_final, c.d_ctr, sizeof(DCounters), hipMemcpyDeviceToHost));
    std::vector<DWaveRow> h_rows((size_t)c.n_rows);
    HIP_TRY(hipMemcpy(h_rows.data(), c.d_rows, sizeof(DWaveRow) * (size_t)c.n_rows, hipMemcpyDeviceToHost));
    unsigned long long fin[C_COUNT] = {0, 0, 0, 0, 0, 0, 0, 0};
    for (const DWaveRow &r : h_rows)
        for (int k = 0; k < C_COUNT; k++) fin[k] += r.c[k];
    const std::vector<hipEvent_t> &evs = c.timing_events;
    double t_adv = 0, t_ch = 0;
    long long n_sampled = (long long)(ev_used / 4);
    for (size_t q = 0; q + 3 < ev_used; q += 4) {
        float ms;
        HIP_TRY(hipEventElapsedTime(&ms, evs[q], evs[q + 1]));
        t_adv += ms;
        HIP_TRY(hipEventElapsedTime(&ms, evs[q + 1], evs[q + 2]));
        t_ch += ms;
        HIP_TRY(hipEventElapsedTime(&ms, evs[q + 2], evs[q + 3]));
    }
    if (!finished) return fail("rt_render_shard: round limit reached before the path pool drained");
    if (!stats) return 0;
    memset(stats, 0, sizeof(*stats));
    stats->camera_rays = (int64_t)fin[C_CAMERA];
    stats->shade_events = (int64_t)fin[C_SHADE];
    stats->closest_rays = (int64_t)fin[C_CLOSEST];
    stats->any_rays = (int64_t)fin[C_ANY];
    stats->emission_adds = (int64_t)fin[C_EMIT];
    stats->shadow_adds = (int64_t)fin[C_SHADOW_ADD];
    stats->rr_draws = (int64_t)fin[C_RR];
    stats->iterations = rounds;
    stats->bvh_nodes = scene->n_nodes;
    stats->bvh_depth = scene->max_depth;
    stats->seconds_render = ms_total * 1e-3;
    stats->seconds_rng_init = rng_seconds;
    double scale_up = n_sampled > 0 ? (double)rounds / (double)n_sampled : 0.0;
    stats->seconds_trace = t_ch * 1e-3 * scale_up;
    stats->seconds_reference_tree = ref_tree_seconds;
    stats->seconds_advance = t_adv * 1e-3 * scale_up;
    stats->launches_trace = rounds;
    stats->reserved[0] = n_sampled;
    if (persistent) {
        stats->seconds_trace = ms_paths * 1e-3;
        stats->seconds_advance = 0.0;
        stats->launches_trace = 1;
        stats->reserved[0] = 1;
        stats->reserved[1] = 1 + slot_chunk + ((int64_t)slot_head << 32);
        stats->reserved[2] = top_records_in_lds;
    }
    rare_path_counters(h_final.vstat, &stats->reserved[4]);
    return 0;
}

int render_shard_impl(const rt_scene *scene, const rt_camera *camera, int width, int height, int spp,
                      int max_bounces, uint64_t seed, int shard_index, int shard_count, uint32_t flags,
                      float *d_sum, hipStream_t st, rt_stats *stats, int ctx_lane = 0, const RayFrame *rays = nullptr) {
    if (!scene || (!camera && !rays) || !d_sum) return fail("rt_render_shard: null argument");
    if (width <= 0 || height <= 0 || spp <= 0 || max_bounces < 0) return fail("rt_render_shard: bad dimensions");
    if (max_bounces > (1 << 24)) return fail("rt_render_shard: max_bounces exceeds 16777216");
    if (shard_count <= 0 || kW % shard_count != 0 || shard_index < 0 || shard_index >= shard_count)
        return fail("rt_render_shard: shard_count must divide 1048576 and 0 <= shard_index < shard_count");
    if ((long long)width * height > (long long)(0x7fffffff / 3))
        return fail("rt_render_shard: width*height exceeds 715827882 pixels");
    if (!rays)
        if (int rc = ensure_origin_radius(scene, camera->lookfrom)) return rc;
    const bool per_sample = (flags & RT_FLAG_RNG_PER_SAMPLE) != 0;
    const HitMode mode = hit_mode(flags, per_sample);
    if (mode.literal && per_sample) return fail("rt_render_shard: RT_FLAG_REFERENCE_WALK is a parity mode and RT_FLAG_RNG_PER_SAMPLE is not: pick one");
    if (refuse_both_hit_flags("rt_render_shard", flags)) return 1;
    if (per_sample) {
        if (spp % shard_count != 0) return fail("rt_render_shard: RT_FLAG_RNG_PER_SAMPLE needs num_samples divisible by shard_count");
        spp /= shard_count;
    }
    const long long cam_end = rays ? rays->n_rays : (long long)width * height * spp;
    if (cam_end + 13LL * kW >= (1LL << 31))
        return fail("rt_render_shard: width*height*spp exceeds the reference's int32 camera-ray range");
    int dev = 0;
    HIP_TRY(hipGetDevice(&dev));
    if (dev != scene->device) return fail("rt_render_shard: scene was created on another device");
    double ref_tree_seconds = 0.0;
    if (mode.ref_tree()) {
        bool built = false;
        if (ensure_ref_tree(scene, &built)) return 1;
        if (built) ref_tree_seconds = scene->build_seconds_ref;
    }
    const int n = per_sample ? kW : kW / shard_count;
    const int slot_lo = per_sample ? 0 : shard_index * n;
    Context *cp = nullptr;
    if (get_context(n, ctx_lane, &cp)) return 1;
    Context &c = *cp;
    std::lock_guard<std::mutex> busy_lock(c.busy);
    FrameRun f{c, scene, rays, st, d_sum, flags, per_sample, mode};
    f.ref_tree_seconds = ref_tree_seconds;
    if (ensure_rng(c, seed, slot_lo, st, &f.rng_seconds)) return 1;

    f.sc = scene->dev();
    if (!rays) memcpy(&f.cam, camera, sizeof(Camera));
    {
        DCounters zero{};
        zero.last_live_round = -1;
        c.h_ctr[0] = zero;
        HIP_TRY(hipMemcpyAsync(c.d_ctr, &c.h_ctr[0], sizeof(DCounters), hipMemcpyHostToDevice, st));
        HIP_TRY(hipMemsetAsync(c.d_rows, 0, sizeof(DWaveRow) * (size_t)c.n_rows, st));
        HIP_TRY(hipStreamSynchronize(st));
    }
    f.stack_cap = lds_stack_cap(scene, kLdsStack);
    f.lds_bytes = sizeof(int) * (size_t)kBlock * (size_t)(f.stack_cap + 2);
    const int stack_need = std::max(scene->stack_bound, mode.ref_tree() ? 32 : 0);
    if (ensure_overflow(c.d_over, c.over_levels, stack_need - std::min(f.stack_cap, lds_stack_cap(scene, kPathsLdsStack)))) return 1;
    const int n_live = per_sample ? n : (int)std::max<long long>(1, std::min<long long>(n, cam_end - (long long)slot_lo));
    hipLaunchKernelGGL(k_pool_init, dim3(grid_for(n_live)), dim3(kBlock), 0, st, c.pools, n_live, max_bounces);
    HIP_TRY(hipGetLastError());

    AdvanceParams &ap = f.ap;
    ap.n = n_live;
    ap.slot_lo = slot_lo;
    ap.width = width;
    ap.height = height;
    ap.spp = spp;
    ap.max_bounces = max_bounces;
    ap.cam_end = cam_end;
    ap.last_gen = per_sample ? 0x7fffffff : (int)((cam_end + kW - 1) / kW) - 1;
    ap.per_sample = per_sample ? 1 : 0;
    ap.key_mul = per_sample ? shard_count : 1;
    ap.key_add = per_sample ? shard_index : 0;
    ap.seed_lo = (uint32_t)seed;
    ap.seed_hi = (uint32_t)(seed >> 32);
    ap.batch_mask = 7;
    ap.fb_fixed = (flags & kFlagFixedFb) ? 1 : 0;
    ap.w_over_spp = (kW % spp == 0 && !rays) ? kW / spp : 0;
    ap.dpx = ap.w_over_spp % width;
    ap.dpy = (ap.w_over_spp > 0 && width < 32768 && height < 32768) ? ap.w_over_spp / width : -1;
    f.lds_tables = scene->n_mats <= kLdsTable && scene->n_lights <= kLdsTable;

    HIP_TRY(hipEventCreate(&f.ev_start));
    HIP_TRY(hipEventCreate(&f.ev_stop));
    HIP_TRY(hipEventRecord(f.ev_start, st));

    int occ_c = 0;
    HIP_TRY(hipDeviceGetAttribute(&f.cus, hipDeviceAttributeMultiprocessorCount, dev));
    f.trace = trace_kernel(mode.literal, mode.verify, scene->wide);
    HIP_TRY(hipOccupancyMaxActiveBlocksPerMultiprocessor(&occ_c, f.trace, kBlock, f.lds_bytes));
    int per_cu = std::max(1, occ_c);
    if (const char *e = knob("RT_TRACE_BLOCKS_PER_CU")) per_cu = std::max(1, std::min(per_cu, atoi(e)));
    f.grid_trace = dim3(std::min(grid_for(n_live), std::max(1, f.cus * per_cu)));
    f.tpp.total = n_live;
    f.tpp.fb = d_sum;
    f.tpp.rows = c.d_rows;
    f.tpp.debug_no_deposit = (flags & 0x100u) ? 1 : 0;
    f.tpp.fb_fixed = (flags & kFlagFixedFb) ? 1 : 0;
    f.tpp.vstat = &c.d_ctr->vstat[0];
#ifdef RT_TRACE_PROFILE
    HIP_TRY(hipMalloc((void **)&f.tpp.prof, sizeof(unsigned long long) * 16));
    HIP_TRY(hipMemset(f.tpp.prof, 0, sizeof(unsigned long long) * 16));
#endif
    if (const char *e = knob("RT_PERSISTENT")) f.persistent = atoi(e) != 0;
    if (rays && !scene->wide) f.persistent = false;
    if (per_sample && !f.persistent) return fail("rt_render_shard: RT_FLAG_RNG_PER_SAMPLE runs on the persistent kernel only");
    if (f.persistent ? f.run_persistent() : f.run_rounds()) return 1;
    if (f.run_lockstep()) return 1;
    HIP_TRY(hipEventRecord(f.ev_stop, st));
    HIP_TRY(hipEventSynchronize(f.ev_stop));
    return f.frame_stats(stats);
}

template <class KERNEL>
static int resident_grid(KERNEL kernel, size_t lds_bytes, int cus, int n, int *grid) {
    int per_cu = 0;
    HIP_TRY(hipOccupancyMaxActiveBlocksPerMultiprocessor(&per_cu, kernel, kBlock, lds_bytes));
    const int resident = std::min(std::max(per_cu, 1) * std::max(cus, 1), kOverStride / kBlock);
    *grid = std::max(1, std::min(resident, (int)(((size_t)n + kBlock - 1) / kBlock)));
    return 0;
}

using QueryKernel = decltype(&k_query<Q_CLOSEST, false, false, false>);
template <int KIND>
static QueryKernel query_kernel(bool literal, bool verify, bool wide) {
    if (literal) return k_query<KIND, false, true, false>;
    if (verify) return wide ? k_query<KIND, true, false, true> : k_query<KIND, false, false, true>;
    return wide ? k_query<KIND, true, false, false> : k_query<KIND, false, false, false>;
}
template <int KIND>
static int run_query(const rt_scene *scene, HitMode mode, QueryParams qp, hipStream_t st, int64_t counters_out[3]) {
    rt_scene::QueryState &q = scene->query;
    if (KIND == Q_ANY && qp.excluded && !q.d_inverse && scene->n_tris > 0) {
        HIP_TRY(hipMalloc((void **)&q.d_inverse, sizeof(int) * (size_t)scene->n_tris));
        hipLaunchKernelGGL(k_query_inverse, dim3((scene->n_tris + 255) / 256), dim3(256), 0, st, scene->d_order, scene->n_tris, q.d_inverse);
    }
    const int stack_cap = lds_stack_cap(scene, kLdsStack);
    if (ensure_overflow(q.d_over, q.over_levels, std::max(scene->stack_bound, 32) - stack_cap)) return 1;
    qp.n_tris = scene->n_tris;
    qp.inverse = q.d_inverse;
    qp.vstat = q.d_words->vstat;
    const QueryKernel kernel = query_kernel<KIND>(mode.literal, mode.verify, scene->wide);
    const size_t lds = sizeof(int) * kBlock * (size_t)(stack_cap + 1);
    int grid = 0;
    if (resident_grid(kernel, lds, q.cus, qp.n, &grid)) return 1;
    hipLaunchKernelGGL(kernel, dim3(grid), dim3(kBlock), lds, st, scene->dev(), qp, stack_cap, q.d_over);
    HIP_TRY(hipGetLastError());
    HIP_TRY(hipMemcpyAsync(q.h_words->vstat, q.d_words->vstat, sizeof(q.h_words->vstat), hipMemcpyDeviceToHost, st));
    HIP_TRY(hipStreamSynchronize(st));
    rare_path_counters(q.h_words->vstat, counters_out);
    return 0;
}

template <int KIND>
static int query_impl(const rt_scene *scene, uint32_t flags, int n, const float *d_o, const float *d_d, const float *d_tmax,
                      const int32_t *d_excluded, int32_t *d_out_i, float *d_t, float *d_u, float *d_v, hipStream_t st) {
    const std::string w(KIND == Q_CLOSEST ? "rt_query_closest_device" : "rt_query_any_device");
    if (!scene) return fail(w + ": null scene");
    if (n < 0 || n > (1 << 30)) return fail(w + ": n = " + std::to_string(n) + " is outside 0 .. 2^30");
    if (flags & ~(uint32_t)(RT_FLAG_REFERENCE_WALK | RT_FLAG_WATERTIGHT)) return fail(w + ": flags other than RT_FLAG_REFERENCE_WALK / RT_FLAG_WATERTIGHT");
    if (refuse_both_hit_flags(w, flags)) return 1;
    if (n > 0 && (!d_o || !d_d || !d_out_i))
        return fail(w + ": null " + (!d_o ? "d_origin_xyz" : !d_d ? "d_dir_xyz" : KIND == Q_CLOSEST ? "d_hit_tri" : "d_occluded"));
    if (n == 0) return 0;
    const HitMode mode = hit_mode(flags);
    rt_scene::QueryState &q = scene->query;
    std::lock_guard<std::mutex> lock(q.mutex);
    DeviceGuard dev;
    if (dev.enter(scene->device)) return 1;
    if (ensure_query_state(scene, false)) return 1;
    if (mode.ref_tree() && ensure_ref_tree(scene)) return 1;
    if (int rc = validate_table(scene, w, n, d_o, d_d, nullptr, 0, st)) return rc;
    QueryParams qp{};
    qp.n = n;
    qp.o3 = d_o;
    qp.d3 = d_d;
    qp.tmax = d_tmax;
    qp.excluded = d_excluded;
    qp.out_i = d_out_i;
    qp.out_t = d_t;
    qp.out_u = d_u;
    qp.out_v = d_v;
    return run_query<KIND>(scene, mode, qp, st, q.counters);
}

template <int KIND>
static int trace_hook(const rt_scene *scene, uint32_t flags, int n, const float *origin_xyz, const float *dir_xyz, const float *tmax,
                      const int32_t *excluded_tri, int32_t *out_i, float *t, float *u, float *v) {
    const HitMode mode = hit_mode(flags);
    rt_scene::QueryState &q = scene->query;
    std::lock_guard<std::mutex> lock(q.mutex);
    DeviceGuard dev;
    if (dev.enter(scene->device)) return 1;
    if (ensure_query_state(scene, false)) return 1;
    if (mode.ref_tree() && ensure_ref_tree(scene)) return 1;
    {
        float need[3] = {0.f, 0.f, 0.f};
        for (int i = 0; i < n; i++)
            for (int a = 0; a < 3; a++)
                if (std::isfinite(origin_xyz[3 * (size_t)i + a])) need[a] = std::max(need[a], std::fabs(origin_xyz[3 * (size_t)i + a]));
        if (int rc = ensure_origin_radius(scene, need)) return rc;
    }
    DevScope tmp;
    QueryParams qp{};
    qp.n = n;
    if (stage(tmp, origin_xyz, 3 * (size_t)n, nullptr, qp.o3) || stage(tmp, dir_xyz, 3 * (size_t)n, nullptr, qp.d3) ||
        stage(tmp, tmax, (size_t)n, nullptr, qp.tmax) || (KIND == Q_ANY && stage(tmp, excluded_tri, (size_t)n, nullptr, qp.excluded)))
        return 1;
    if (tmp.alloc(qp.out_i, (size_t)n)) return 1;
    if (KIND == Q_CLOSEST && (tmp.alloc(qp.out_t, (size_t)n) || tmp.alloc(qp.out_u, (size_t)n) || tmp.alloc(qp.out_v, (size_t)n))) return 1;
    HIP_TRY(hipMemsetAsync(q.d_words, 0, sizeof(QueryWords), nullptr));
    HIP_TRY(hipStreamSynchronize(nullptr));
    int64_t counters[3];
    if (int rc = run_query<KIND>(scene, mode, qp, nullptr, counters)) return rc;
    HIP_TRY(hipMemcpy(out_i, qp.out_i, sizeof(int) * (size_t)n, hipMemcpyDeviceToHost));
    if (KIND == Q_CLOSEST) {
        HIP_TRY(hipMemcpy(t, qp.out_t, sizeof(float) * (size_t)n, hipMemcpyDeviceToHost));
        HIP_TRY(hipMemcpy(u, qp.out_u, sizeof(float) * (size_t)n, hipMemcpyDeviceToHost));
        HIP_TRY(hipMemcpy(v, qp.out_v, sizeof(float) * (size_t)n, hipMemcpyDeviceToHost));
    }
    return 0;
}
static int trace_closest_impl(const rt_scene *scene, uint32_t flags, int n, const float *origin_xyz, const float *dir_xyz, const float *tmax,
                              int32_t *hit_tri, float *t, float *u, float *v) {
    if (!scene || n < 0 || (n > 0 && (!origin_xyz || !dir_xyz || !tmax || !hit_tri || !t || !u || !v)))
        return fail("rt_trace_closest: bad argument");
    if (n == 0) return 0;
    return trace_hook<Q_CLOSEST>(scene, flags, n, origin_xyz, dir_xyz, tmax, nullptr, hit_tri, t, u, v);
}
static int trace_any_impl(const rt_scene *scene, uint32_t flags, int n, const float *origin_xyz, const float *dir_xyz, const float *tmax,
                          const int32_t *excluded_tri, int32_t *occluded) {
    if (!scene || n < 0 || (n > 0 && (!origin_xyz || !dir_xyz || !tmax || !excluded_tri || !occluded)))
        return fail("rt_trace_any: bad argument");
// ... 211 lines not shown
```

### rtcuda_amd/csrc/rtcuda_amd.hip

```cpp
#include <hip/hip_runtime.h>

#include <algorithm>
#include <chrono>
#include <cmath>
#include <cstdio>
#include <cstring>
#include <memory>
#include <mutex>
#include <thread>
#include <type_traits>
#include <string>
#include <vector>

#include "../../include/rtcuda_amd.h"
#include "rt_bvh.h"
#include "rt_denoise.h"
#include "rt_device.h"
#include "rt_launch_plan.h"
#include "rt_ploc.h"
#include "rt_ref_tree.h"
#include "rt_slot_chunks.h"
#include "rt_stats_merge.h"
#include "rt_temporal.h"

using namespace rt;

namespace {
thread_local std::string g_last_error;
std::string g_peer_log;
int fail(const std::string &msg) {
    g_last_error = msg;
    return 1;
}
#define HIP_TRY(expr)                                                                          \
    do {                                                                                       \
        hipError_t _e = (expr);                                                                \
        if (_e != hipSuccess)                                                                  \
            return fail(std::string(#expr) + ": " + hipGetErrorString(_e) + " (" __FILE__ ":" + \
                        std::to_string(__LINE__) + ")");                                       \
    } while (0)

using rtbvh::knob;

constexpr int kW = RT_NUM_WORKING_PATHS;
constexpr uint32_t kFlagFixedFb = 0x200u;
constexpr int kBlock = 256;
static_assert(rtplan::kBlock == kBlock && rtplan::kSlots == kW, "rt_launch_plan.h plans for this workgroup and this pool");
constexpr int kLdsStack = 16;
constexpr int kPathsLdsStack = 10;
constexpr int kOverStride = 1 << 20;
constexpr int kMaxStackBound = 160;
constexpr int kLockChunk = 16;
}

struct DScene {
    const float4 *nodes;
    const float4 *tris;
    const int2 *tri_info;
    const float4 *tri_shade;
    const int *order;
    const Material *mats;
    const Light *lights;
    int num_lights;
    int num_mats;
    const float *tables;
    int tab_dwords;
    const float4 *ref_nodes;
    const int *ref_prims;
    int ref_n_prims;
    const int *ref_leaf_of;
    const int *ref_parent;
    int ref_root_leaf;
};
__device__ __host__ inline int tab_off_lights(int n_mats) { return 5 * n_mats; }
__device__ __host__ inline int tab_off_ltri(int n_mats, int n_lights) { return 5 * n_mats + 8 * n_lights; }
__device__ __host__ inline int tab_off_lpre(int n_mats, int n_lights) { return 5 * n_mats + 20 * n_lights; }
constexpr int kTabPerMat = 5, kTabPerLight = 8 + 12 + 4;
inline int tab_dwords(int n_mats, int n_lights) { return kTabPerMat * n_mats + kTabPerLight * n_lights; }

enum { A_OX, A_OY, A_OZ, A_DX, A_DY, A_DZ, A_HPX, A_HPY, A_HPZ, A_HNX, A_HNY, A_HNZ, A_BR, A_BG, A_BB, A_SOX, A_SOY, A_SOZ, A_SDX, A_SDY, A_SDZ, A_STMAX, A_SLR, A_SLG, A_SLB, A_HIT_INFO, A_BOUNCES, A_PIXEL, A_GEN, A_STARGET, A_RD, A_R0, A_R1, A_R2, A_R3, A_R4, A_COUNT };
struct DPools {
    float *base;
    int n;
    __device__ __forceinline__ float &ox(int i) const { return base[(unsigned)(A_OX * n + i)]; }
    __device__ __forceinline__ float &oy(int i) const { return base[(unsigned)(A_OY * n + i)]; }
    __device__ __forceinline__ float &oz(int i) const { return base[(unsigned)(A_OZ * n + i)]; }
    __device__ __forceinline__ float &dx(int i) const { return base[(unsigned)(A_DX * n + i)]; }
    __device__ __forceinline__ float &dy(int i) const { return base[(unsigned)(A_DY * n + i)]; }
    __device__ __forceinline__ float &dz(int i) const { return base[(unsigned)(A_DZ * n + i)]; }
    __device__ __forceinline__ float &hpx(int i) const { return base[(unsigned)(A_HPX * n + i)]; }
    __device__ __forceinline__ float &hpy(int i) const { return base[(unsigned)(A_HPY * n + i)]; }
    __device__ __forceinline__ float &hpz(int i) const { return base[(unsigned)(A_HPZ * n + i)]; }
    __device__ __forceinline__ float &hnx(int i) const { return base[(unsigned)(A_HNX * n + i)]; }
    __device__ __forceinline__ float &hny(int i) const { return base[(unsigned)(A_HNY * n + i)]; }
    __device__ __forceinline__ float &hnz(int i) const { return base[(unsigned)(A_HNZ * n + i)]; }
    __device__ __forceinline__ float &br(int i) const { return base[(unsigned)(A_BR * n + i)]; }
    __device__ __forceinline__ float &bg(int i) const { return base[(unsigned)(A_BG * n + i)]; }
    __device__ __forceinline__ float &bb(int i) const { return base[(unsigned)(A_BB * n + i)]; }
    __device__ __forceinline__ float &sox(int i) const { return base[(unsigned)(A_SOX * n + i)]; }
    __device__ __forceinline__ float &soy(int i) const { return base[(unsigned)(A_SOY * n + i)]; }
    __device__ __forceinline__ float &soz(int i) const { return base[(unsigned)(A_SOZ * n + i)]; }
    __device__ __forceinline__ float &sdx(int i) const { return base[(unsigned)(A_SDX * n + i)]; }
    __device__ __forceinline__ float &sdy(int i) const { return base[(unsigned)(A_SDY * n + i)]; }
    __device__ __forceinline__ float &sdz(int i) const { return base[(unsigned)(A_SDZ * n + i)]; }
    __device__ __forceinline__ float &stmax(int i) const { return base[(unsigned)(A_STMAX * n + i)]; }
    __device__ __forceinline__ float &slr(int i) const { return base[(unsigned)(A_SLR * n + i)]; }
    __device__ __forceinline__ float &slg(int i) const { return base[(unsigned)(A_SLG * n + i)]; }
    __device__ __forceinline__ float &slb(int i) const { return base[(unsigned)(A_SLB * n + i)]; }
    __device__ __forceinline__ int &hit_info(int i) const { return ((int *)base)[(unsigned)(A_HIT_INFO * n + i)]; }
    __device__ __forceinline__ int &bounces(int i) const { return ((int *)base)[(unsigned)(A_BOUNCES * n + i)]; }
    __device__ __forceinline__ int &pixel(int i) const { return ((int *)base)[(unsigned)(A_PIXEL * n + i)]; }
    __device__ __forceinline__ int &gen(int i) const { return ((int *)base)[(unsigned)(A_GEN * n + i)]; }
    __device__ __forceinline__ int &starget(int i) const { return ((int *)base)[(unsigned)(A_STARGET * n + i)]; }
    __device__ __forceinline__ uint32_t &rd(int i) const { return ((uint32_t *)base)[(unsigned)(A_RD * n + i)]; }
    __device__ __forceinline__ uint32_t &r0(int i) const { return ((uint32_t *)base)[(unsigned)(A_R0 * n + i)]; }
    __device__ __forceinline__ uint32_t &r1(int i) const { return ((uint32_t *)base)[(unsigned)(A_R1 * n + i)]; }
    __device__ __forceinline__ uint32_t &r2(int i) const { return ((uint32_t *)base)[(unsigned)(A_R2 * n + i)]; }
    __device__ __forceinline__ uint32_t &r3(int i) const { return ((uint32_t *)base)[(unsigned)(A_R3 * n + i)]; }
    __device__ __forceinline__ uint32_t &r4(int i) const { return ((uint32_t *)base)[(unsigned)(A_R4 * n + i)]; }
    float *array(int k) const { return base + (size_t)k * n; }
};

struct DCounters {
    int last_live_round;
    unsigned int unused0;
    unsigned int pad2[2];
    unsigned long long vstat[4];
};
enum { V_OWN_FAIL = 0, V_LOST = 1, V_TIE = 2, V_LITERAL = 3 };
enum { C_CAMERA = 0, C_SHADE, C_CLOSEST, C_ANY, C_EMIT, C_SHADOW_ADD, C_RR, C_UNUSED, C_COUNT };
struct DWaveRow {
    unsigned long long c[C_COUNT];
};

constexpr int kDone = -0x7fffffff;
constexpr int kParked = -0x7ffffffe;
constexpr int kChunkFresh = 0x7ffffffe;

__device__ __forceinline__ unsigned lane_id() {
    return __builtin_amdgcn_mbcnt_hi(~0u, __builtin_amdgcn_mbcnt_lo(~0u, 0u));
}
__device__ __forceinline__ unsigned prefix_popc(unsigned long long mask) {
    return __builtin_amdgcn_mbcnt_hi((unsigned)(mask >> 32), __builtin_amdgcn_mbcnt_lo((unsigned)mask, 0u));
}
__device__ __forceinline__ unsigned long long wave_ballot(bool p) { return __builtin_amdgcn_ballot_w64(p); }
__device__ __forceinline__ int wave_count(bool p) { return (int)__builtin_popcountll(__builtin_amdgcn_ballot_w64(p)); }
__device__ __forceinline__ unsigned wave_index() { return (blockIdx.x * blockDim.x + threadIdx.x) >> 6; }
__device__ __forceinline__ void row_add(DWaveRow *rows, const unsigned long long (&v)[C_COUNT]) {
    unsigned l = lane_id();
    unsigned long long mine = 0;
#pragma unroll
    for (int k = 0; k < C_COUNT; k++) mine = (l == (unsigned)k) ? v[k] : mine;
    if (l < C_COUNT && mine != 0) atomicAdd(&rows[wave_index()].c[l], mine);
}

__global__ void k_rng_init(DPools p, int n, int slot_lo, Rng seed_state, const uint32_t *__restrict__ jump_pow) {
    int i = blockIdx.x * blockDim.x + threadIdx.x;
    if (i >= n) return;
    uint32_t slot = (uint32_t)(slot_lo + i);
    uint32_t v[5] = {seed_state.v0, seed_state.v1, seed_state.v2, seed_state.v3, seed_state.v4};
    for (int k = 0; k < 20; k++) {
        if (!((slot >> k) & 1u)) continue;
        const uint32_t *m = jump_pow + (size_t)k * 160 * 5;
        uint32_t r[5] = {0, 0, 0, 0, 0};
#pragma unroll
        for (int w = 0; w < 5; w++) {
            uint32_t bits = v[w];
            for (int b = 0; b < 32; b++) {
                uint32_t sel = 0u - ((bits >> b) & 1u);
                const uint32_t *row = m + (w * 32 + b) * 5;
                r[0] ^= row[0] & sel;
                r[1] ^= row[1] & sel;
                r[2] ^= row[2] & sel;
                r[3] ^= row[3] & sel;
                r[4] ^= row[4] & sel;
            }
        }
#pragma unroll
        for (int w = 0; w < 5; w++) v[w] = r[w];
    }
    p.rd(i) = seed_state.d;
    p.r0(i) = v[0];
    p.r1(i) = v[1];
    p.r2(i) = v[2];
    p.r3(i) = v[3];
    p.r4(i) = v[4];
}

__global__ void k_pool_init(DPools p, int n, int max_bounces) {
    int i = blockIdx.x * blockDim.x + threadIdx.x;
    if (i >= n) return;
    p.hit_info(i) = -1;
    p.bounces(i) = max_bounces;
    p.gen(i) = 0;
    p.pixel(i) = 0;
}

struct AdvanceParams {
    int n;
    int slot_lo;
    int width, height, spp, max_bounces;
    long long cam_end;
    int round;
    int batch_mask;
    int last_gen;
    int lockstep;
    int fb_fixed;
    int w_over_spp;
    int dpx, dpy;
    int per_sample, key_mul, key_add;
    uint32_t seed_lo, seed_hi;
};

constexpr int kLdsTable = 64;
constexpr int kTabDwordsMax = kLdsTable * (kTabPerMat + kTabPerLight);

__global__ void k_build_tri_shade(const float4 *__restrict__ tris, const int2 *__restrict__ tri_info, int n,
                                  float4 *__restrict__ out) {
    int k = blockIdx.x * blockDim.x + threadIdx.x;
    if (k >= n) return;
    Tri tr = load_tri(tris, k);
    V3 un = neg(unit(tr.n));
    int2 ml = tri_info[k];
    out[k] = make_float4(un.x, un.y, un.z, __int_as_float((ml.x & 0xffff) | ((ml.y + 1) << 16)));
}

__global__ void k_build_tables(const Material *mats, int n_mats, const Light *lights, int n_lights,
                               const float4 *tris, float *tab) {
    int t = blockIdx.x * blockDim.x + threadIdx.x;
    if (t < n_mats) {
        const float *src = (const float *)&mats[t];
        for (int k = 0; k < 5; k++) tab[5 * t + k] = src[k];
    }
    if (t < n_lights) {
        const float *src = (const float *)&lights[t];
        float *dl = tab + tab_off_lights(n_mats) + 8 * t;
        for (int k = 0; k < 8; k++) dl[k] = src[k];
        float *dt = tab + tab_off_ltri(n_mats, n_lights) + 12 * t;
        float *dp = tab + tab_off_lpre(n_mats, n_lights) + 4 * t;
        Light l = lights[t];
        if (l.type == 1) {
            Tri lt = load_tri(tris, l.tri);
            const float *q = (const float *)(tris + 3 * (size_t)l.tri);
            for (int k = 0; k < 12; k++) dt[k] = q[k];
            V3 un = unit(lt.n);
            dp[0] = 1.f / tri_area(lt);
            dp[1] = un.x;
            dp[2] = un.y;
            dp[3] = un.z;
        } else {
            for (int k = 0; k < 12; k++) dt[k] = 0.f;
            dp[0] = dp[1] = dp[2] = dp[3] = 0.f;
        }
    }
}

__device__ __forceinline__ Material tab_material(const float *tab, int i) {
    const float *q = tab + 5 * i;
    Material m;
    m.ax = q[0];
    m.ay = q[1];
    m.az = q[2];
    m.ior = q[3];
    m.type = __float_as_int(q[4]);
    return m;
}
__device__ __forceinline__ Light tab_light(const float *tab, int n_mats, int i) {
    const float *q = tab + tab_off_lights(n_mats) + 8 * i;
    Light l;
    l.type = __float_as_int(q[0]);
    l.px = q[1];
    l.py = q[2];
    l.pz = q[3];
    l.tri = __float_as_int(q[4]);
    l.lx = q[5];
    l.ly = q[6];
    l.lz = q[7];
    return l;
}

constexpr float kFixedScale = 1073741824.f;
__device__ __forceinline__ long long to_fixed(float x) {
    if (!(fabsf(x) <= 2147483648.f)) x = (x == x) ? copysignf(2147483648.f, x) : 0.f;
    return __float2ll_rn(x * kFixedScale);
}
__device__ __forceinline__ void deposit(float *__restrict__ fb, int fixed, int pixel, float r, float g, float b) {
    const unsigned k = (unsigned)(3 * pixel);
    if (fixed) {
        unsigned long long *f = (unsigned long long *)fb;
        atomicAdd(&f[k + 0], (unsigned long long)to_fixed(r));
        atomicAdd(&f[k + 1], (unsigned long long)to_fixed(g));
        atomicAdd(&f[k + 2], (unsigned long long)to_fixed(b));
    } else {
        atomicAdd(&fb[k + 0], r);
        atomicAdd(&fb[k + 1], g);
        atomicAdd(&fb[k + 2], b);
    }
}

__device__ __forceinline__ void acc_add(float *acc, float r, float g, float b) {
    acc[0 * kBlock] += r;
    acc[1 * kBlock] += g;
    acc[2 * kBlock] += b;
}
__device__ __forceinline__ void acc_flush(float *acc, float *__restrict__ fb, int fixed, int pixel) {
    const float r = acc[0 * kBlock], g = acc[1 * kBlock], b = acc[2 * kBlock];
    if (r != 0.f || g != 0.f || b != 0.f) {
        deposit(fb, fixed, pixel, r, g, b);
        acc[0 * kBlock] = 0.f;
        acc[1 * kBlock] = 0.f;
        acc[2 * kBlock] = 0.f;
    }
}

struct SlotState {
    int bounces, hit_info, pixel, gen;
    Rng rs;
    V3 beta, wo, isect_p, isect_n;
};
struct AdvanceOut {
    bool did_gen, did_shade, has_shadow, did_emit, new_ray;
    bool wants_gen;
    int rr_draws;
    V3 ray_o, ray_d;
    V3 s_o, s_d, s_L;
    float s_tmax;
    int s_target;
};

struct RayTable {
    const float *o3, *d3;
    const int *pixel;
};
struct KeyedRayTable {
    const float *o3, *d3;
    const int *pixel;
    unsigned long long key_first;
    uint32_t key_stride, rays_per_pixel;
    int pix_first;
    uint32_t rem_first;
};
static_assert(sizeof(KeyedRayTable) <= sizeof(Camera), "k_paths' dynamic LDS is sized for a Camera in the uniforms");
#ifndef RT_RAYS_NONTEMPORAL
#define RT_RAYS_NONTEMPORAL 1
#endif
template <class T>
__device__ __forceinline__ T table_load(const T *q) {
    return RT_RAYS_NONTEMPORAL ? __builtin_nontemporal_load(q) : *q;
}

template <bool NEVER_LOCKSTEP = false, class SRC>
__device__ __forceinline__ void gen_core(const SRC &cam, const AdvanceParams &ap, int slot_global, SlotState &st,
                                         AdvanceOut &out, int *pxy = nullptr, long long cid_given = -1) {
    const bool lockstep = NEVER_LOCKSTEP ? false : (ap.lockstep != 0);
    long long cid = cid_given >= 0 ? cid_given : (long long)st.gen * kW + slot_global;
    if (cid >= ap.cam_end) {
        st.bounces = kDone;
        return;
    }
    if (!lockstep && st.gen == ap.last_gen) {
        st.bounces = kParked;
        return;
    }
    st.gen = st.gen + 1;
    if constexpr (std::is_same<SRC, KeyedRayTable>::value) {
        const unsigned c = (unsigned)cid;
        const unsigned long long ck = (unsigned long long)c * cam.key_stride;
        st.rs = rng_sample_stream(ap.seed_lo, ap.seed_hi, cam.key_first + ck);
        rng_next(st.rs);
        rng_next(st.rs);
        const float *o3 = cam.o3 + 3 * (size_t)c, *d3 = cam.d3 + 3 * (size_t)c;
        out.ray_o = mk(table_load(o3), table_load(o3 + 1), table_load(o3 + 2));
        out.ray_d = mk(table_load(d3), table_load(d3 + 1), table_load(d3 + 2));
        if (cam.pixel) {
            st.pixel = table_load(cam.pixel + c);
        } else {
            const unsigned long long t = cam.rem_first + ck;
            const unsigned q = (t >> 32) ? (unsigned)(t / cam.rays_per_pixel) : (unsigned)t / cam.rays_per_pixel;
            st.pixel = cam.pix_first + (int)q;
        }
        out.new_ray = true;
        st.bounces = 0;
        st.beta = mk(1.f, 1.f, 1.f);
        out.did_gen = true;
        return;
    } else if constexpr (std::is_same<SRC, RayTable>::value) {
        const unsigned c = (unsigned)cid;
        rng_next(st.rs);
        rng_next(st.rs);
        const float *o3 = cam.o3 + 3 * (size_t)c, *d3 = cam.d3 + 3 * (size_t)c;
        out.ray_o = mk(table_load(o3), table_load(o3 + 1), table_load(o3 + 2));
        out.ray_d = mk(table_load(d3), table_load(d3 + 1), table_load(d3 + 2));
        st.pixel = cam.pixel ? table_load(cam.pixel + c) : (int)(c / (unsigned)ap.spp);
        out.new_ray = true;
        st.bounces = 0;
        st.beta = mk(1.f, 1.f, 1.f);
        out.did_gen = true;
        return;
    } else {
    int px, py;
    if (cid_given >= 0) {
        st.pixel = (int)((unsigned)cid / (unsigned)ap.spp);
        py = (int)((unsigned)st.pixel / (unsigned)ap.width);
        px = st.pixel - py * ap.width;
    } else if (pxy && ap.dpy >= 0 && *pxy >= 0) {
        px = (*pxy & 0xffff) + ap.dpx;
        py = (*pxy >> 16) + ap.dpy;
        if (px >= ap.width) {
            px -= ap.width;
            py++;
        }
        st.pixel = py * ap.width + px;
    } else {
        if (ap.w_over_spp) st.pixel = (st.gen - 1) * ap.w_over_spp + (int)((unsigned)slot_global / (unsigned)ap.spp);
        else st.pixel = (int)(cid / ap.spp);
        py = (int)((unsigned)st.pixel / (unsigned)ap.width);
        px = st.pixel - py * ap.width;
    }
    if (pxy) *pxy = px | (py << 16);
    if (ap.per_sample) st.rs = rng_sample_stream(ap.seed_lo, ap.seed_hi, (unsigned long long)cid * (unsigned)ap.key_mul + (unsigned)ap.key_add);
    float jx = rng_uniform(st.rs);
    float jy = rng_uniform(st.rs);
    camera_get_ray(cam, (px + jx) / ap.width, (py + jy) / ap.height, out.ray_o, out.ray_d);
    out.new_ray = true;
    st.bounces = 0;
    st.beta = mk(1.f, 1.f, 1.f);
    out.did_gen = true;
    }
}

template <bool DEFER_GEN, bool NEVER_LOCKSTEP = false, bool USE_ACC = false, class SRC>
__device__ __forceinline__ void advance_core(const DScene &sc, const float *tab, const SRC &cam,
                                             const AdvanceParams &ap, int slot_global, SlotState &st, AdvanceOut &out,
                                             float *__restrict__ fb, float *acc = nullptr) {
    const bool lockstep = NEVER_LOCKSTEP ? false : (ap.lockstep != 0);
    const int off_ltri = tab_off_ltri(sc.num_mats, sc.num_lights);
    const int off_lpre = tab_off_lpre(sc.num_mats, sc.num_lights);
    out.did_gen = out.did_shade = out.has_shadow = out.did_emit = out.new_ray = out.wants_gen = false;
    out.rr_draws = 0;
    const bool hit = st.hit_info >= 0;
    const int light_of_hit = hit ? ((st.hit_info >> 16) & 0xffff) - 1 : -1;
    RT_MARK("adv.init");
    if (st.bounces == 0 && hit && light_of_hit >= 0) {
        Light l = tab_light(tab, sc.num_mats, light_of_hit);
        if (USE_ACC) acc_add(acc, l.lx, l.ly, l.lz);
        else deposit(fb, ap.fb_fixed, st.pixel, l.lx, l.ly, l.lz);
        out.did_emit = true;
    }
    const bool cont = st.bounces < ap.max_bounces;
    if (cont && hit) {
        bool shade = true;
        if (st.bounces > kRrStart && max3(st.beta) < kRrThreshold) {
            const float pt = fmaxf(0.05f, 1 - max3(st.beta));
            shade = false;
            while (true) {
                out.rr_draws++;
                const bool kill = rng_uniform(st.rs) < pt;
                st.bounces = st.bounces + 1;
                if (!kill) {
                    st.beta = divf(st.beta, 1 - pt);
                    shade = true;
                    break;
                }
                if (lockstep || !(st.bounces < ap.max_bounces)) break;
            }
        } else {
            st.bounces = st.bounces + 1;
        }
        if (shade) out.did_shade = true;
        else if (lockstep) return;
    } else {
        if (cont && lockstep) {
            st.bounces = st.bounces + 1;
            return;
        }
    }
    if (!out.did_shade) {
        if (DEFER_GEN) {
            out.wants_gen = true;
            return;
        }
        if (USE_ACC) acc_flush(acc, fb, ap.fb_fixed, st.pixel);
        gen_core<NEVER_LOCKSTEP>(cam, ap, slot_global, st, out);
        return;
    }
    RT_MARK("adv.mat.sample_f");
    Material m = tab_material(tab, st.hit_info & 0xffff);
    V3 multiplier = scale(st.beta, (float)sc.num_lights);
    int again_draws;
    {
        V3 n = st.isect_n, wi;
        float pdf;
        V3 f = mat_sample_f(m, st.wo, st.rs, n, wi, pdf, again_draws);
        out.ray_o = offset_ray_origin(st.isect_p, n);
        out.ray_d = wi;
        out.new_ray = true;
        st.beta = mul(st.beta, divf(scale(f, dot(wi, n)), pdf));
    }
    RT_MARK("adv.mat.light_sample");
    if (sc.num_lights > 0) {
        int light_idx = min((int)(rng_uniform(st.rs) * sc.num_lights), sc.num_lights - 1);
        Light light = tab_light(tab, sc.num_mats, light_idx);
        V3 wi, Li;
        float lt, lpdf;
        if (light.type == 0) {
            wi = sub(mk(light.px, light.py, light.pz), st.isect_p);
            lt = len(wi);
            Li = divf(mk(light.lx, light.ly, light.lz), lt * lt);
            wi = divf(wi, lt);
            lpdf = 1.f;
        } else {
            const float *q = tab + off_ltri + 12 * light_idx;
            const float *pre = tab + off_lpre + 4 * light_idx;
            Tri lt_tri;
            lt_tri.p0 = mk(q[0], q[1], q[2]);
            lt_tri.e1 = mk(q[3], q[4], q[5]);
            lt_tri.e2 = mk(q[6], q[7], q[8]);
            lt_tri.n = mk(q[9], q[10], q[11]);
            lpdf = pre[0];
            V3 lun = mk(pre[1], pre[2], pre[3]);
            float a = sqrtf(rng_uniform(st.rs));
            float u2 = rng_uniform(st.rs);
            V3 tp = tri_point(lt_tri, 1 - a, u2 * a);
            wi = sub(tp, st.isect_p);
            lt = len(wi);
            wi = divf(wi, lt);
            Li = mk(light.lx, light.ly, light.lz);
            lpdf *= len2(sub(tp, st.isect_p)) / fabsf(dot(lun, wi));
        }
        RT_MARK("adv.mat.nee");
        V3 n = dot(st.isect_n, wi) > 0.f ? st.isect_n : neg(st.isect_n);
        V3 f;
        float spdf;
        if (mat_get_f(m, st.wo, wi, n, f, spdf)) {
            f = scale(f, dot(wi, n));
            out.s_o = offset_ray_origin(st.isect_p, n);
            out.s_d = wi;
            out.s_tmax = lt;
            out.s_target = light.type == 1 ? light.tri : -1;
            if (light.type == 0) {
                out.s_L = divf(mul(mul(multiplier, f), Li), lpdf);
            } else {
                float weight = power_heuristic(lpdf, spdf);
                out.s_L = divf(scale(mul(mul(multiplier, f), Li), weight), lpdf);
            }
            out.has_shadow = true;
        }
        RT_MARK("adv.mat.burn");
        if (light.type != 0) {
            if (again_draws >= 1) rng_next(st.rs);
            if (again_draws >= 2) rng_next(st.rs);
        }
    }
    RT_MARK("adv.mat.end");
}


#include "rt_walk.inc"
#include "rt_stream_kernels.inc"

enum { PH_ADV = 0, PH_ANY = 1, PH_CLOSEST = 2, PH_IDLE = 3, PH_GEN = 4 };
#ifndef RT_TRI_PER_STEP
#define RT_TRI_PER_STEP 2
#endif
constexpr int kCidChunk = 512;
constexpr int kTriPerStep = RT_TRI_PER_STEP;
#ifndef RT_NODE_PER_STEP
#define RT_NODE_PER_STEP 8
#endif
constexpr int kNodePerStep = RT_NODE_PER_STEP;
#ifndef RT_NODE_PER_STEP_WIDE
#define RT_NODE_PER_STEP_WIDE 2
#endif
constexpr int kNodePerStepWide = RT_NODE_PER_STEP_WIDE;
#ifndef RT_NODE_CONT
#define RT_NODE_CONT 36
#endif
#ifndef RT_NODE_EXTRA
#define RT_NODE_EXTRA 2
#endif
constexpr int kNodeCont = RT_NODE_CONT, kNodeExtra = RT_NODE_EXTRA;
#ifndef RT_SPECULATE
#define RT_SPECULATE 1
#endif

constexpr bool kSpeculate = RT_SPECULATE != 0;

#ifdef RT_TRACE_PROFILE
constexpr int kProfRec = 6;
#endif
#define RT_PATHS_CHUNKS 0
#define RT_FRAME_SRC Camera
#define RT_K_ADVANCE k_advance
#define RT_K_PATHS k_paths
#include "rt_frame_kernels.inc"
#undef RT_FRAME_SRC
#undef RT_K_ADVANCE
#undef RT_K_PATHS
#define RT_FRAME_SRC RayTable
#define RT_K_ADVANCE k_advance_rays
#define RT_K_PATHS k_paths_rays
#include "rt_frame_kernels.inc"
#undef RT_FRAME_SRC
#undef RT_K_ADVANCE
#undef RT_K_PATHS
#define RT_FRAME_SRC KeyedRayTable
#define RT_K_ADVANCE k_advance_keyed
#define RT_K_PATHS k_paths_keyed
#include "rt_frame_kernels.inc"
#undef RT_FRAME_SRC
#undef RT_K_ADVANCE
#undef RT_K_PATHS
#undef RT_PATHS_CHUNKS
#define RT_PATHS_CHUNKS 1
#define RT_FRAME_SRC Camera
#define RT_K_ADVANCE k_advance_chunked_unused
#define RT_K_PATHS k_paths_chunked
#include "rt_frame_kernels.inc"
#undef RT_FRAME_SRC
#undef RT_K_ADVANCE
#undef RT_K_PATHS
#undef RT_PATHS_CHUNKS

__global__ void k_post_process(float *fb, int n_values, float inv_spp) {
    int i = blockIdx.x * blockDim.x + threadIdx.x;
    if (i < n_values) fb[i] = sqrtf(fb[i] * inv_spp);
}

__global__ void k_post_process_fixed(const long long *__restrict__ sums, float *__restrict__ out, int n_values, float inv_spp) {
    int i = blockIdx.x * blockDim.x + threadIdx.x;
    if (i < n_values) out[i] = sqrtf((float)((double)sums[i] * (1.0 / 1073741824.0)) * inv_spp);
}

__global__ void k_accumulate_f32(float *__restrict__ dst, const float *__restrict__ src, int n) {
    int i = blockIdx.x * blockDim.x + threadIdx.x;
    if (i < n) dst[i] += src[i];
}
__global__ void k_accumulate_i64(long long *__restrict__ dst, const long long *__restrict__ src, int n) {
    int i = blockIdx.x * blockDim.x + threadIdx.x;
    if (i < n) dst[i] += src[i];
}

__global__ void k_test_draw(DPools p, int n, int draws, uint32_t *__restrict__ state6, float *__restrict__ uni) {
    int i = blockIdx.x * blockDim.x + threadIdx.x;
    if (i >= n) return;
    Rng rs{p.rd(i), p.r0(i), p.r1(i), p.r2(i), p.r3(i), p.r4(i)};
    for (int k = 0; k < draws; k++) uni[(size_t)i * draws + k] = rng_uniform(rs);
    state6[6 * (size_t)i + 0] = rs.d;
    state6[6 * (size_t)i + 1] = rs.v0;
    state6[6 * (size_t)i + 2] = rs.v1;
    state6[6 * (size_t)i + 3] = rs.v2;
    state6[6 * (size_t)i + 4] = rs.v3;
    state6[6 * (size_t)i + 5] = rs.v4;
}
#include "rt_build_kernels.inc"
#include "rt_denoise_kernels.inc"
#include "rt_temporal_kernels.inc"

#include "rt_host_scene.inc"
#include "rt_host_render.inc"
#include "rt_host_frame.inc"
#include "rt_host_denoise.inc"
#include "rt_host_temporal.inc"
}

extern "C" {

const char *rt_last_error(void) { return g_last_error.c_str(); }
const char *rt_peer_access_log(void) { return g_peer_log.c_str(); }
const char *rt_version(void) { return "rtcuda_amd 0.1 (gfx950)"; }
#ifndef RT_BUILD_ID
#define RT_BUILD_ID "unknown"
#endif
const char *rt_build_id(void) { return RT_BUILD_ID; }

int rt_scene_create(const float *tri_p0p1p2, int n_tris, const int32_t *tri_material, const int32_t *tri_light,
                    const rt_material *materials, int n_materials, const rt_light *lights, int n_lights,
                    rt_scene **out_scene) {
    return scene_create_impl(tri_p0p1p2, n_tris, tri_material, tri_light, materials, n_materials, lights, n_lights, 0u, out_scene);
}

int rt_scene_create_flags(const float *tri_p0p1p2, int n_tris, const int32_t *tri_material, const int32_t *tri_light,
                          const rt_material *materials, int n_materials, const rt_light *lights, int n_lights,
                          uint32_t scene_flags, rt_scene **out_scene) {
    return scene_create_impl(tri_p0p1p2, n_tris, tri_material, tri_light, materials, n_materials, lights, n_lights, scene_flags, out_scene);
}

void rt_scene_destroy(rt_scene *scene) { delete scene; }

int rt_scene_info(const rt_scene *scene, int64_t out[4]) {
    if (!scene || !out) return fail("rt_scene_info: null argument");
    out[0] = scene->n_nodes;
    out[1] = scene->n_tris;
    out[2] = scene->max_depth;
    out[3] = scene->n_leaves;
    return 0;
}

int rt_scene_build_info(const rt_scene *scene, int *builder, double *seconds) {
    if (!scene || !builder || !seconds) return fail("rt_scene_build_info: null argument");
    *builder = scene->builder;
    *seconds = scene->build_seconds;
    return 0;
}

int rt_scene_update(rt_scene *scene, const float *tri_p0p1p2, int n_tris) {
    return scene_update_impl(scene, tri_p0p1p2, n_tris, false, nullptr, "rt_scene_update");
}

int rt_scene_update_device(rt_scene *scene, const float *d_tri_p0p1p2, int n_tris, void *stream) {
    return scene_update_impl(scene, d_tri_p0p1p2, n_tris, true, (hipStream_t)stream, "rt_scene_update_device");
}

int rt_scene_rebuild(rt_scene *scene, const float *tri_p0p1p2, int n_tris) {
    return scene_rebuild_impl(scene, tri_p0p1p2, n_tris, false, nullptr, "rt_scene_rebuild");
}

int rt_scene_rebuild_device(rt_scene *scene, const float *d_tri_p0p1p2, int n_tris, void *stream) {
    return scene_rebuild_impl(scene, d_tri_p0p1p2, n_tris, true, (hipStream_t)stream, "rt_scene_rebuild_device");
}

int rt_scene_set_materials(rt_scene *scene, const rt_material *materials, int n_materials) {
    return scene_set_materials_impl(scene, materials, n_materials);
}

int rt_scene_set_lights(rt_scene *scene, const rt_light *lights, int n_lights, const int32_t *tri_light) {
    return scene_set_lights_impl(scene, lights, n_lights, tri_light);
}

int rt_scene_set_triangles(rt_scene *scene, const float *tri_p0p1p2, int n_tris, const int32_t *tri_material, const int32_t *tri_light,
                           const rt_material *materials, int n_materials, const rt_light *lights, int n_lights) {
    return scene_set_triangles_impl(scene, tri_p0p1p2, n_tris, tri_material, tri_light, materials, n_materials, lights, n_lights, false,
                                    nullptr, "rt_scene_set_triangles");
}

int rt_scene_set_triangles_device(rt_scene *scene, const float *d_tri_p0p1p2, int n_tris, const int32_t *d_tri_material,
                                  const int32_t *d_tri_light, const rt_material *materials, int n_materials, const rt_light *lights,
                                  int n_lights, void *stream) {
    return scene_set_triangles_impl(scene, d_tri_p0p1p2, n_tris, d_tri_material, d_tri_light, materials, n_materials, lights, n_lights,
                                    true, (hipStream_t)stream, "rt_scene_set_triangles_device");
}

int rt_scene_create_device(const float *d_tri_p0p1p2, int n_tris, const int32_t *d_tri_material, const int32_t *d_tri_light,
                           const rt_material *materials, int n_materials, const rt_light *lights, int n_lights, void *stream,
                           rt_scene **out_scene) {
    return scene_create_device_impl(d_tri_p0p1p2, n_tris, d_tri_material, d_tri_light, materials, n_materials, lights, n_lights,
                                    (hipStream_t)stream, out_scene);
}

int rt_scene_refit_info(const rt_scene *scene, int64_t *refits, double *seconds_last, double *sah_ratio) {
    if (!scene || !refits || !seconds_last || !sah_ratio) return fail("rt_scene_refit_info: null argument");
    *refits = scene->refits;
    *seconds_last = scene->refit_seconds;
    *sah_ratio = scene->sah_build > 0.0 ? scene->sah_now / scene->sah_build : 1.0;
    return 0;
}

int rt_camera_make(const float lookfrom[3], const float lookat[3], const float up[3], float vfov_deg,
                   float aspect_ratio, rt_camera *out) {
    if (!lookfrom || !lookat || !up || !out) return fail("rt_camera_make: null argument");
    const float pi = 3.14159265358979323846f;
    float vfov_rad = vfov_deg * (pi / 180.f);
    float vh = 2.f * tanf(vfov_rad * 0.5f);
    float vw = vh * aspect_ratio;
    auto sub3 = [](const float *a, const float *b, float *r) { r[0] = a[0] - b[0]; r[1] = a[1] - b[1]; r[2] = a[2] - b[2]; };
    auto dot3 = [](const float *a, const float *b) { return a[0] * b[0] + a[1] * b[1] + a[2] * b[2]; };
    auto unit3 = [&](float *a) {
        float inv = 1.f / sqrtf(a[0] * a[0] + a[1] * a[1] + a[2] * a[2]);
        a[0] *= inv; a[1] *= inv; a[2] *= inv;
    };
    float w[3], v[3], u[3];
    sub3(lookfrom, lookat, w);
    unit3(w);
    float duw = dot3(up, w);
    v[0] = up[0] - duw * w[0];
// ... 251 lines not shown
```

Measured before the change: 5120.

## Skip camera samples whose pixels fall outside the scene's projected bounds

```diff
diff --git a/rtcuda_amd/api.py b/rtcuda_amd/api.py
--- a/rtcuda_amd/api.py
+++ b/rtcuda_amd/api.py
@@ -61,7 +61,8 @@
         d = {n: getattr(self, n) for n, _ in self._fields_ if n != "reserved"}
         d["lds_top_records"] = int(self.reserved[2])
         d["slot_chunk"] = max((int(self.reserved[1]) & 0xffffffff) - 1, 0)
-        d["slot_head"] = int(self.reserved[1]) >> 32
+        d["slot_head"] = (int(self.reserved[1]) >> 32) & 0xffff
+        d["background_skip"] = (int(self.reserved[1]) >> 48) & 1
         d["literal_retraces"], d["reference_lost_hits"], d["exact_ties"] = (int(self.reserved[k]) for k in (4, 5, 6))
         return d
 
diff --git a/rtcuda_amd/csrc/rt_background.h b/rtcuda_amd/csrc/rt_background.h
--- /dev/null
+++ b/rtcuda_amd/csrc/rt_background.h
@@ -0,0 +1,112 @@
+#pragma once
+
+#include <cmath>
+
+namespace rtbg {
+
+struct Rect {
+    int x0, y0, x1, y1;
+};
+
+inline Rect background_rect(const float cam12[12], int width, int height, const float lo3[3], const float hi3[3],
+                            const float *radius3 = nullptr) {
+    const Rect whole{0, 0, width, height}, empty{0, 0, 0, 0};
+    if (width <= 0 || height <= 0) return empty;
+    double lf[3], w0[3], hz[3], vt[3];
+    for (int a = 0; a < 3; a++) {
+        lf[a] = cam12[a];
+        w0[a] = (double)cam12[3 + a] - (double)cam12[a];
+        hz[a] = cam12[6 + a];
+        vt[a] = cam12[9 + a];
+    }
+    for (int k = 0; k < 12; k++)
+        if (!std::isfinite(cam12[k])) return whole;
+    bool any_box = true;
+    for (int a = 0; a < 3; a++) {
+        if (std::isnan(lo3[a]) || std::isnan(hi3[a])) return whole;
+        if (!(lo3[a] <= hi3[a])) any_box = false;
+    }
+    if (!any_box) return empty;
+    for (int a = 0; a < 3; a++)
+        if (!std::isfinite(lo3[a]) || !std::isfinite(hi3[a])) return whole;
+    double n[3] = {hz[1] * vt[2] - hz[2] * vt[1], hz[2] * vt[0] - hz[0] * vt[2], hz[0] * vt[1] - hz[1] * vt[0]};
+    const double hh = hz[0] * hz[0] + hz[1] * hz[1] + hz[2] * hz[2], vv = vt[0] * vt[0] + vt[1] * vt[1] + vt[2] * vt[2];
+    const double hv = hz[0] * vt[0] + hz[1] * vt[1] + hz[2] * vt[2];
+    const double nn = n[0] * n[0] + n[1] * n[1] + n[2] * n[2];
+    const double wn = w0[0] * n[0] + w0[1] * n[1] + w0[2] * n[2];
+    const double ww = w0[0] * w0[0] + w0[1] * w0[1] + w0[2] * w0[2];
+    if (!(hh > 0.0) || !(vv > 0.0) || !std::isfinite(hh * vv) || !std::isfinite(nn) || !std::isfinite(wn)) return whole;
+    if (!(nn > 1e-12 * hh * vv)) return whole;
+    if (!(wn * wn > 1e-12 * nn * ww)) return whole;
+    {
+        double mag = 0.0;
+        for (int k = 0; k < 12; k++) mag = std::fmax(mag, std::fabs((double)cam12[k]));
+        const double err = std::ldexp(4.0 * mag, -20);
+        if (!(err < 0.25 * std::sqrt(hh) / width) || !(err < 0.25 * std::sqrt(vv) / height)) return whole;
+    }
+    double dist = 0.0;
+    for (int a = 0; a < 3; a++) dist += std::fmax(std::fabs(lo3[a]), std::fabs(hi3[a])) + std::fabs(lf[a]);
+    double blo[3], bhi[3];
+    for (int a = 0; a < 3; a++) {
+        const double big = std::fmax(std::fabs((double)lo3[a]), std::fabs((double)hi3[a]));
+        double rad = 4.0 * std::fmax(big, std::fabs(lf[a]));
+        if (radius3 && std::isfinite(radius3[a])) rad = std::fmax(rad, std::fabs((double)radius3[a]));
+        const double m = 1e-4 * ((double)hi3[a] - (double)lo3[a]) + std::ldexp(rad, -22) + std::ldexp(big, -20) + std::ldexp(2.0 * dist, -17);
+        blo[a] = (double)lo3[a] - m;
+        bhi[a] = (double)hi3[a] + m;
+    }
+    double u0 = INFINITY, u1 = -INFINITY, v0 = INFINITY, v1 = -INFINITY;
+    int behind = 0;
+    for (int k = 0; k < 8; k++) {
+        double q[3];
+        for (int a = 0; a < 3; a++) q[a] = (((k >> a) & 1) ? bhi[a] : blo[a]) - lf[a];
+        const double depth = (q[0] * n[0] + q[1] * n[1] + q[2] * n[2]) / wn;
+        const double qq = q[0] * q[0] + q[1] * q[1] + q[2] * q[2];
+        behind += (depth < 0.0 && depth * depth * ww > 1e-12 * qq) ? 1 : 0;
+    }
+    if (behind == 8) return empty;
+    for (int k = 0; k < 8; k++) {
+        double q[3];
+        for (int a = 0; a < 3; a++) q[a] = (((k >> a) & 1) ? bhi[a] : blo[a]) - lf[a];
+        const double depth = (q[0] * n[0] + q[1] * n[1] + q[2] * n[2]) / wn;
+        const double qq = q[0] * q[0] + q[1] * q[1] + q[2] * q[2];
+        if (!(depth > 0.0) || !(depth * depth * ww > 1e-12 * qq)) return whole;
+        double r[3];
+        for (int a = 0; a < 3; a++) r[a] = q[a] - depth * w0[a];
+        const double rh = r[0] * hz[0] + r[1] * hz[1] + r[2] * hz[2], rv = r[0] * vt[0] + r[1] * vt[1] + r[2] * vt[2];
+        const double b = (rh * vv - rv * hv) / nn, c = (rv * hh - rh * hv) / nn;
+        const double u = b / depth, v = c / depth;
+        if (!std::isfinite(u) || !std::isfinite(v)) return whole;
+        u0 = std::fmin(u0, u);
+        u1 = std::fmax(u1, u);
+        v0 = std::fmin(v0, v);
+        v1 = std::fmax(v1, v);
+    }
+    auto lo_px = [](double t, int size) { return (int)std::fmin(std::fmax(std::floor(t * size) - 1.0, 0.0), (double)size); };
+    auto hi_px = [](double t, int size) { return (int)std::fmin(std::fmax(std::ceil(t * size) + 1.0, 0.0), (double)size); };
+    const Rect r{lo_px(u0, width), lo_px(v0, height), hi_px(u1, width), hi_px(v1, height)};
+    if (r.x0 >= r.x1 || r.y0 >= r.y1) return empty;
+    return r;
+}
+
+template <class PAIR>
+inline bool root_bounds(const PAIR *root2, int absent, float lo3[3], float hi3[3]) {
+    bool any = false;
+    for (int a = 0; a < 3; a++) {
+        lo3[a] = INFINITY;
+        hi3[a] = -INFINITY;
+    }
+    for (int k = 0; k < 4; k++) {
+        const PAIR &p = root2[k >> 1];
+        if (((k & 1) ? p.rlink : p.llink) == absent) continue;
+        const float *b = (k & 1) ? p.rbox : p.lbox;
+        any = true;
+        for (int a = 0; a < 3; a++) {
+            lo3[a] = std::fmin(lo3[a], b[a]);
+            hi3[a] = std::fmax(hi3[a], b[3 + a]);
+        }
+    }
+    return any;
+}
+
+}
diff --git a/rtcuda_amd/csrc/rt_device.h b/rtcuda_amd/csrc/rt_device.h
--- a/rtcuda_amd/csrc/rt_device.h
+++ b/rtcuda_amd/csrc/rt_device.h
@@ -92,7 +92,8 @@
     r.v4 = 5783321u + t0;
     return r;
 }
-RT_DEV float rng_uniform(Rng &s) { return (float)rng_next(s) * 2.3283064e-10f + (2.3283064e-10f / 2.0f); }
+RT_DEV float rng_to_uniform(uint32_t draw) { return (float)draw * 2.3283064e-10f + (2.3283064e-10f / 2.0f); }
+RT_DEV float rng_uniform(Rng &s) { return rng_to_uniform(rng_next(s)); }
 
 struct Tri {
     V3 p0, e1, e2, n;
diff --git a/rtcuda_amd/csrc/rt_frame_kernels.inc b/rtcuda_amd/csrc/rt_frame_kernels.inc
--- a/rtcuda_amd/csrc/rt_frame_kernels.inc
+++ b/rtcuda_amd/csrc/rt_frame_kernels.inc
@@ -256,6 +256,7 @@
         cold[12 * kBlock] = -1;
     }
     unsigned long long n_gen = 0, n_shade = 0, n_traced = 0, n_shadow = 0, n_emit = 0, n_deposit = 0, n_rr = 0;
+    unsigned n_bg_lane = 0;
 #ifdef RT_TRACE_PROFILE
     unsigned long long pf[16] = {0, 0, 0, 0, 0, 0, 0, 0, 0, 0, 0, 0, 0, 0, 0, 0};
     unsigned long long pf_gen_cycles = 0, pf_fin_cycles = 0, pf_fin_lanes = 0, pf_fin_iters = 0;
@@ -399,6 +400,104 @@
                 __builtin_amdgcn_s_waitcnt(0x0f70);
                 if (chunk_was_gen) acc_flush(acc, fb, ap_fb_fixed, chunk_acc_pixel);
             }
+#if RT_PATHS_BG
+            {
+                static_assert((kW & (kW - 1)) == 0, "a slot's camera rays are counted with a shift");
+                const bool was_gen = phase == PH_GEN;
+                const int f_width = __builtin_amdgcn_readfirstlane(ap.width), f_dpx = __builtin_amdgcn_readfirstlane(ap.dpx);
+                const int f_dpy = __builtin_amdgcn_readfirstlane(ap.dpy), f_last_gen = __builtin_amdgcn_readfirstlane(ap.last_gen);
+                const int f_cam_end = __builtin_amdgcn_readfirstlane((int)ap.cam_end);
+                const int f_slot_lo = __builtin_amdgcn_readfirstlane(ap.slot_lo);
+                const int f_x0 = __builtin_amdgcn_readfirstlane(ap.bg_x0), f_y0 = __builtin_amdgcn_readfirstlane(ap.bg_y0);
+                const unsigned f_w = (unsigned)__builtin_amdgcn_readfirstlane(ap.bg_w), f_h = (unsigned)__builtin_amdgcn_readfirstlane(ap.bg_h);
+                const bool can_loop = !draw_cids && f_dpy >= 0;
+                const rtchunks::Multiple bg_m{CHUNKS ? __builtin_amdgcn_readfirstlane(s_task[2]) : 1u, CHUNKS ? __builtin_amdgcn_readfirstlane(s_task[3]) : 0u,
+                                              CHUNKS ? __builtin_amdgcn_readfirstlane(s_task[4]) : 0u};
+                const bool dealt = CHUNKS && chunk_g && slot_set >= (int)__builtin_amdgcn_readfirstlane(s_task[5]);
+                Rng g_rs{0, 0, 0, 0, 0, 0};
+                int g_gen = 0, g_stop = 0, px = 0, py = 0;
+                uint32_t draw_x = 0, draw_y = 0;
+                bool looking = false, made = false;
+                if (was_gen) {
+                    g_gen = cold[2 * kBlock];
+                    g_rs = Rng{(uint32_t)cold[3 * kBlock], (uint32_t)cold[4 * kBlock], (uint32_t)cold[5 * kBlock],
+                               (uint32_t)cold[6 * kBlock], (uint32_t)cold[7 * kBlock], (uint32_t)cold[8 * kBlock]};
+                    const int pxy = cold[12 * kBlock];
+                    if (!CHUNKS) acc_flush(acc, fb, ap_fb_fixed, cold[1 * kBlock]);
+                    const int slot = f_slot_lo + i;
+                    if (draw_cids) g_stop = my_cid >= (long long)f_cam_end ? g_gen : 0x7fffffff;
+                    else g_stop = min(f_last_gen, (f_cam_end - slot + (kW - 1)) >> __builtin_ctz((unsigned)kW));
+                    looking = g_gen < g_stop;
+                    px = pxy & 0xffff;
+                    py = pxy >> 16;
+                    if (looking && (pxy < 0 || !can_loop)) {
+                        SlotState t;
+                        t.gen = g_gen + 1;
+                        int qx, qy;
+                        gen_pixel(ap, slot, t, nullptr, my_cid, my_cid >= 0 ? my_cid : (long long)g_gen * kW + slot, qx, qy);
+                        px = qx - f_dpx;
+                        py = qy - f_dpy;
+                        if (px < 0) {
+                            px += f_width;
+                            py--;
+                        }
+                    }
+                }
+                if (looking) {
+                    bool bg;
+                    do {
+                        g_gen++;
+                        px += f_dpx;
+                        py += f_dpy;
+                        if (px >= f_width) {
+                            px -= f_width;
+                            py++;
+                        }
+                        bg = (unsigned)(px - f_x0) >= f_w || (unsigned)(py - f_y0) >= f_h;
+                        if (draw_cids) {
+                            if (!bg) {
+                                g_rs = rng_sample_stream(ap.seed_lo, ap.seed_hi, (unsigned long long)my_cid * (unsigned)ap.key_mul + (unsigned)ap.key_add);
+                                draw_x = rng_next(g_rs);
+                                draw_y = rng_next(g_rs);
+                            }
+                        } else {
+                            draw_x = rng_next(g_rs);
+                            draw_y = rng_next(g_rs);
+                        }
+                        n_bg_lane += bg ? 1u : 0u;
+                    } while (bg && can_loop && g_gen < g_stop && !(dealt && rtchunks::chunk_ends((unsigned)g_gen, bg_m, false)));
+                    made = !bg;
+                }
+                if (made) {
+                    camera_get_ray(cam, (px + rng_to_uniform(draw_x)) / ap.width, (py + rng_to_uniform(draw_y)) / ap.height, out.ray_o, out.ray_d);
+                    out.new_ray = true;
+                    out.did_gen = true;
+                }
+                if (was_gen) {
+                    int b = 0;
+                    if (!made && g_gen >= g_stop) {
+                        const long long cid = my_cid >= 0 ? my_cid : (long long)g_gen * kW + (f_slot_lo + i);
+                        b = cid >= ap.cam_end ? kDone : kParked;
+                        hand_back = true;
+                    }
+                    cold[0 * kBlock] = b;
+                    cold[2 * kBlock] = g_gen;
+                    cold[3 * kBlock] = (int)g_rs.d;
+                    cold[4 * kBlock] = (int)g_rs.v0;
+                    cold[5 * kBlock] = (int)g_rs.v1;
+                    cold[6 * kBlock] = (int)g_rs.v2;
+                    cold[7 * kBlock] = (int)g_rs.v3;
+                    cold[8 * kBlock] = (int)g_rs.v4;
+                    cold[12 * kBlock] = px | (py << 16);
+                    if (made) {
+                        cold[1 * kBlock] = py * f_width + px;
+                        cold[9 * kBlock] = __float_as_int(1.f);
+                        cold[10 * kBlock] = __float_as_int(1.f);
+                        cold[11 * kBlock] = __float_as_int(1.f);
+                    }
+                }
+            }
+#else
             if (phase == PH_GEN) {
                 SlotState st;
                 st.gen = cold[2 * kBlock];
@@ -428,6 +527,7 @@
                     hand_back = true;
                 }
             }
+#endif
             const bool nr = out.new_ray;
             o = out.ray_o;
             d = out.ray_d;
@@ -469,6 +569,7 @@
             AdvanceOut out;
             out.did_gen = out.did_shade = out.has_shadow = out.did_emit = out.new_ray = false;
             out.rr_draws = 0;
+            out.bg_skipped = 0;
             if (phase == PH_ADV) {
                 cold_load();
                 SlotState st;
@@ -508,7 +609,7 @@
                 st.gen = gen;
                 st.rs = rs;
                 st.beta = beta;
-                advance_core<SPLIT_GEN, true, true>(sc, tab, cam, ap, ap.slot_lo + i, st, out, fb, acc);
+                advance_core<SPLIT_GEN, true, true, RT_PATHS_BG != 0>(sc, tab, cam, ap, ap.slot_lo + i, st, out, fb, acc);
                 RT_MARK("adv.tail");
                 bounces = st.bounces;
                 pixel = st.pixel;
@@ -552,6 +653,14 @@
             }
             inv = inv_dir(d);
             if (!SPLIT_GEN) n_gen += wave_count((out.did_gen));
+            if (!SPLIT_GEN && RT_PATHS_BG) {
+                int bg = out.bg_skipped;
+                if (wave_ballot(bg != 0)) {
+                    for (int off = 32; off > 0; off >>= 1) bg += __shfl_xor(bg, off);
+                    n_gen += (unsigned long long)bg;
+                    n_traced += (unsigned long long)bg;
+                }
+            }
             n_shade += wave_count((out.did_shade));
             n_traced += wave_count((out.new_ray));
             n_shadow += wave_count((out.has_shadow));
@@ -761,6 +870,14 @@
           rec[4] = pf_idle;
           rec[5] = pf_idle_max; }
 #endif
+#if RT_PATHS_BG
+    if (SPLIT_GEN) {
+        unsigned long long bg = n_bg_lane;
+        for (int off = 32; off > 0; off >>= 1) bg += __shfl_xor(bg, off);
+        n_gen += bg;
+        n_traced += bg;
+    }
+#endif
     unsigned long long v[C_COUNT] = {n_gen, n_shade, n_traced, n_shadow, n_emit, n_deposit, n_rr, 0ull};
     row_add(rows, v);
 }
diff --git a/rtcuda_amd/csrc/rt_host_check.cpp b/rtcuda_amd/csrc/rt_host_check.cpp
--- a/rtcuda_amd/csrc/rt_host_check.cpp
+++ b/rtcuda_amd/csrc/rt_host_check.cpp
@@ -6,6 +6,7 @@
 #include <cstdlib>
 #include <vector>
 
+#include "rt_background.h"
 #include "rt_bvh.h"
 #include "rt_denoise.h"
 #include "rt_launch_plan.h"
@@ -901,6 +902,15 @@
 uint32_t rt_slot_chunk_sem_unit(uint32_t idx) { return rtchunks::sem_unit(idx); }
 int rt_slot_chunk_sem_value(uint32_t word, uint32_t idx) { return rtchunks::sem_value(word, idx); }
 uint32_t rt_slot_chunk_sem_init() { return rtchunks::kSemWordInit; }
+int rt_background_rect(const float cam12[12], int width, int height, const float lo[3], const float hi[3], int out4[4]) {
+    if (!cam12 || !lo || !hi || !out4 || width <= 0 || height <= 0) return 1;
+    const rtbg::Rect r = rtbg::background_rect(cam12, width, height, lo, hi);
+    out4[0] = r.x0;
+    out4[1] = r.y0;
+    out4[2] = r.x1;
+    out4[3] = r.y1;
+    return 0;
+}
 int hc_denoise(const int64_t *sum_fixed, int num_samples, const int64_t *aov_fixed, int aov_samples, int width, int height, int passes,
                float sigma_color, float sigma_depth, int normal_power_log2, float *rgb_out) {
     if (!sum_fixed || !aov_fixed || !rgb_out || width < 1 || height < 1 || num_samples < 1 || aov_samples < 1) return 1;
diff --git a/rtcuda_amd/csrc/rt_host_render.inc b/rtcuda_amd/csrc/rt_host_render.inc
--- a/rtcuda_amd/csrc/rt_host_render.inc
+++ b/rtcuda_amd/csrc/rt_host_render.inc
@@ -148,23 +148,39 @@
     return wide ? k_trace<true> : k_trace<false>;
 }
 
-template <bool LDS_TABLES, bool WIDE>
-static PathsKernel paths_kernel_of(bool few_blocks, bool per_sample, bool literal, bool verify) {
-    if (literal) return few_blocks ? k_paths<LDS_TABLES, false, 2, false, true, false> : k_paths<LDS_TABLES, false, 4, false, true, false>;
-    if (per_sample && !few_blocks) return k_paths<LDS_TABLES, WIDE, 4, true, false, false>;
-    if (few_blocks) return verify ? k_paths<LDS_TABLES, WIDE, 2, false, false, true> : k_paths<LDS_TABLES, WIDE, 2, false, false, false>;
-    return verify ? k_paths<LDS_TABLES, WIDE, 4, false, false, true> : k_paths<LDS_TABLES, WIDE, 4, false, false, false>;
-}
-template <bool LDS_TABLES, bool WIDE>
-static PathsKernel paths_chunked_kernel_of(bool literal, bool verify) {
-    if (literal) return k_paths_chunked<LDS_TABLES, false, 4, false, true, false>;
-    return verify ? k_paths_chunked<LDS_TABLES, WIDE, 4, false, false, true> : k_paths_chunked<LDS_TABLES, WIDE, 4, false, false, false>;
-}
-static PathsKernel paths_chunked_kernel(bool lds_tables, bool wide, bool literal, bool verify) {
+#define RT_PATHS_KERNELS_OF(NAME, K_PATHS)                                                                                          \
+    template <bool LDS_TABLES, bool WIDE>                                                                                             \
+    static PathsKernel NAME(bool few_blocks, bool per_sample, bool literal, bool verify) {                                            \
+        if (literal) return few_blocks ? K_PATHS<LDS_TABLES, false, 2, false, true, false> : K_PATHS<LDS_TABLES, false, 4, false, true, false>; \
+        if (per_sample && !few_blocks) return K_PATHS<LDS_TABLES, WIDE, 4, true, false, false>;                                       \
+        if (few_blocks) return verify ? K_PATHS<LDS_TABLES, WIDE, 2, false, false, true> : K_PATHS<LDS_TABLES, WIDE, 2, false, false, false>; \
+        return verify ? K_PATHS<LDS_TABLES, WIDE, 4, false, false, true> : K_PATHS<LDS_TABLES, WIDE, 4, false, false, false>;         \
+    }
+RT_PATHS_KERNELS_OF(paths_kernel_of, k_paths)
+RT_PATHS_KERNELS_OF(paths_bg_kernel_of, k_paths_bg)
+#undef RT_PATHS_KERNELS_OF
+#define RT_PATHS_CHUNKED_KERNELS_OF(NAME, K_PATHS)                                                                                  \
+    template <bool LDS_TABLES, bool WIDE>                                                                                             \
+    static PathsKernel NAME(bool literal, bool verify) {                                                                              \
+        if (literal) return K_PATHS<LDS_TABLES, false, 4, false, true, false>;                                                        \
+        return verify ? K_PATHS<LDS_TABLES, WIDE, 4, false, false, true> : K_PATHS<LDS_TABLES, WIDE, 4, false, false, false>;         \
+    }
+RT_PATHS_CHUNKED_KERNELS_OF(paths_chunked_kernel_of, k_paths_chunked)
+RT_PATHS_CHUNKED_KERNELS_OF(paths_chunked_bg_kernel_of, k_paths_chunked_bg)
+#undef RT_PATHS_CHUNKED_KERNELS_OF
+static PathsKernel paths_chunked_kernel(bool lds_tables, bool wide, bool literal, bool verify, bool bg) {
+    if (bg) {
+        if (lds_tables) return (wide ? paths_chunked_bg_kernel_of<true, true> : paths_chunked_bg_kernel_of<true, false>)(literal, verify);
+        return (wide ? paths_chunked_bg_kernel_of<false, true> : paths_chunked_bg_kernel_of<false, false>)(literal, verify);
+    }
     if (lds_tables) return (wide ? paths_chunked_kernel_of<true, true> : paths_chunked_kernel_of<true, false>)(literal, verify);
     return (wide ? paths_chunked_kernel_of<false, true> : paths_chunked_kernel_of<false, false>)(literal, verify);
 }
-static PathsKernel paths_kernel(bool lds_tables, bool wide, bool few_blocks, bool per_sample, bool literal, bool verify) {
+static PathsKernel paths_kernel(bool lds_tables, bool wide, bool few_blocks, bool per_sample, bool literal, bool verify, bool bg) {
+    if (bg) {
+        if (lds_tables) return (wide ? paths_bg_kernel_of<true, true> : paths_bg_kernel_of<true, false>)(few_blocks, per_sample, literal, verify);
+        return (wide ? paths_bg_kernel_of<false, true> : paths_bg_kernel_of<false, false>)(few_blocks, per_sample, literal, verify);
+    }
     if (lds_tables) return (wide ? paths_kernel_of<true, true> : paths_kernel_of<true, false>)(few_blocks, per_sample, literal, verify);
     return (wide ? paths_kernel_of<false, true> : paths_kernel_of<false, false>)(few_blocks, per_sample, literal, verify);
 }
@@ -245,6 +261,7 @@
     HitMode mode;
     bool lds_tables = false, persistent = true, finished = false, ran_lockstep = false;
     int cus = 0, stack_cap = 0, top_records_in_lds = 0, slot_chunk = 0, slot_head = 0, lock_enqueued = 0;
+    bool ran_bg = false;
     DScene sc{};
     Camera cam{};
     AdvanceParams ap{};
@@ -340,7 +357,9 @@
     };
     HIP_TRY(hipEventRecord(c.ev_a, st));
     int chunk = (rays || p.few_blocks || per_sample || ap.last_gen < 1 || ap.n != c.n) ? 0 : rtplan::slot_chunk_for(p, ap.last_gen);
-    const PathsKernel chunked = paths_chunked_kernel(lds_tables, scene->wide, mode.literal, mode.verify);
+    const bool bg = !rays && (long long)ap.bg_w * ap.bg_h < (long long)ap.width * ap.height;
+    ran_bg = bg;
+    const PathsKernel chunked = paths_chunked_kernel(lds_tables, scene->wide, mode.literal, mode.verify, bg);
     if (chunk > 0) {
         int per_cu = 0;
         HIP_TRY(hipOccupancyMaxActiveBlocksPerMultiprocessor(&per_cu, chunked, kBlock, p.lds_bytes));
@@ -352,7 +371,7 @@
     if (rays && rays->keyed) launch_paths(paths_keyed_kernel(lds_tables, p.few_blocks), rays->keyed_table, p.top_n);
     else if (rays) launch_paths(paths_rays_kernel(lds_tables, p.few_blocks, mode.verify), rays->table, p.top_n);
     else if (chunk > 0) launch_paths(chunked, cam, chunk | (slot_head << rtplan::kChunkHeadShift));
-    else launch_paths(paths_kernel(lds_tables, scene->wide, p.few_blocks, per_sample, mode.literal, mode.verify), cam, mode.literal ? 0 : p.top_n);
+    else launch_paths(paths_kernel(lds_tables, scene->wide, p.few_blocks, per_sample, mode.literal, mode.verify, bg), cam, mode.literal ? 0 : p.top_n);
     HIP_TRY(hipGetLastError());
     HIP_TRY(hipEventRecord(c.ev_b, st));
     HIP_TRY(hipEventSynchronize(c.ev_b));
@@ -494,7 +513,7 @@
         stats->seconds_advance = 0.0;
         stats->launches_trace = 1;
         stats->reserved[0] = 1;
-        stats->reserved[1] = 1 + slot_chunk + ((int64_t)slot_head << 32);
+        stats->reserved[1] = 1 + slot_chunk + ((int64_t)slot_head << 32) + ((int64_t)(ran_bg ? 1 : 0) << 48);
         stats->reserved[2] = top_records_in_lds;
     }
     rare_path_counters(h_final.vstat, &stats->reserved[4]);
@@ -580,6 +599,23 @@
     ap.w_over_spp = (kW % spp == 0 && !rays) ? kW / spp : 0;
     ap.dpx = ap.w_over_spp % width;
     ap.dpy = (ap.w_over_spp > 0 && width < 32768 && height < 32768) ? ap.w_over_spp / width : -1;
+    ap.bg_x0 = ap.bg_y0 = 0;
+    ap.bg_w = width;
+    ap.bg_h = height;
+    if (!rays && scene->wide) {
+        bool skip = true;
+        if (const char *e = knob("RT_BG_SKIP")) skip = atoi(e) != 0;
+        std::lock_guard<std::mutex> pad_lock(scene->pad_mutex);
+        if (skip && scene->h_quads.size() >= 2) {
+            float lo[3], hi[3];
+            rtbg::root_bounds(scene->h_quads.data(), (int)rtbvh::kNoChild, lo, hi);
+            const rtbg::Rect r = rtbg::background_rect((const float *)camera, width, height, lo, hi, scene->origin_radius);
+            ap.bg_x0 = r.x0;
+            ap.bg_y0 = r.y0;
+            ap.bg_w = r.x1 - r.x0;
+            ap.bg_h = r.y1 - r.y0;
+        }
+    }
     f.lds_tables = scene->n_mats <= kLdsTable && scene->n_lights <= kLdsTable;
 
     HIP_TRY(hipEventCreate(&f.ev_start));
diff --git a/rtcuda_amd/csrc/rtcuda_amd.hip b/rtcuda_amd/csrc/rtcuda_amd.hip
--- a/rtcuda_amd/csrc/rtcuda_amd.hip
+++ b/rtcuda_amd/csrc/rtcuda_amd.hip
@@ -13,6 +13,7 @@
 #include <vector>
 
 #include "../../include/rtcuda_amd.h"
+#include "rt_background.h"
 #include "rt_bvh.h"
 #include "rt_denoise.h"
 #include "rt_device.h"
@@ -210,6 +211,7 @@
     int dpx, dpy;
     int per_sample, key_mul, key_add;
     uint32_t seed_lo, seed_hi;
+    int bg_x0, bg_y0, bg_w, bg_h;
 };
 
 constexpr int kLdsTable = 64;
@@ -322,6 +324,7 @@
     bool did_gen, did_shade, has_shadow, did_emit, new_ray;
     bool wants_gen;
     int rr_draws;
+    int bg_skipped;
     V3 ray_o, ray_d;
     V3 s_o, s_d, s_L;
     float s_tmax;
@@ -349,20 +352,78 @@
     return RT_RAYS_NONTEMPORAL ? __builtin_nontemporal_load(q) : *q;
 }
 
-template <bool NEVER_LOCKSTEP = false, class SRC>
+template <bool NEVER_LOCKSTEP>
+__device__ __forceinline__ bool gen_begin(const AdvanceParams &ap, int slot_global, SlotState &st, long long cid_given, long long &cid) {
+    const bool lockstep = NEVER_LOCKSTEP ? false : (ap.lockstep != 0);
+    cid = cid_given >= 0 ? cid_given : (long long)st.gen * kW + slot_global;
+    if (cid >= ap.cam_end) {
+        st.bounces = kDone;
+        return false;
+    }
+    if (!lockstep && st.gen == ap.last_gen) {
+        st.bounces = kParked;
+        return false;
+    }
+    st.gen = st.gen + 1;
+    return true;
+}
+__device__ __forceinline__ void gen_pixel(const AdvanceParams &ap, int slot_global, SlotState &st, int *pxy, long long cid_given,
+                                          long long cid, int &px, int &py) {
+    if (cid_given >= 0) {
+        st.pixel = (int)((unsigned)cid / (unsigned)ap.spp);
+        py = (int)((unsigned)st.pixel / (unsigned)ap.width);
+        px = st.pixel - py * ap.width;
+    } else if (pxy && ap.dpy >= 0 && *pxy >= 0) {
+        px = (*pxy & 0xffff) + ap.dpx;
+        py = (*pxy >> 16) + ap.dpy;
+        if (px >= ap.width) {
+            px -= ap.width;
+            py++;
+        }
+        st.pixel = py * ap.width + px;
+    } else {
+        if (ap.w_over_spp) st.pixel = (st.gen - 1) * ap.w_over_spp + (int)((unsigned)slot_global / (unsigned)ap.spp);
+        else st.pixel = (int)(cid / ap.spp);
+        py = (int)((unsigned)st.pixel / (unsigned)ap.width);
+        px = st.pixel - py * ap.width;
+    }
+    if (pxy) *pxy = px | (py << 16);
+}
+__device__ __forceinline__ bool gen_background(const AdvanceParams &ap, int px, int py) {
+    return (unsigned)(px - ap.bg_x0) >= (unsigned)ap.bg_w || (unsigned)(py - ap.bg_y0) >= (unsigned)ap.bg_h;
+}
+__device__ __forceinline__ void gen_camera_ray(const Camera &cam, const AdvanceParams &ap, long long cid, int px, int py, SlotState &st,
+                                               AdvanceOut &out) {
+    if (ap.per_sample) st.rs = rng_sample_stream(ap.seed_lo, ap.seed_hi, (unsigned long long)cid * (unsigned)ap.key_mul + (unsigned)ap.key_add);
+    float jx = rng_uniform(st.rs);
+    float jy = rng_uniform(st.rs);
+    camera_get_ray(cam, (px + jx) / ap.width, (py + jy) / ap.height, out.ray_o, out.ray_d);
+    out.new_ray = true;
+    st.bounces = 0;
+    st.beta = mk(1.f, 1.f, 1.f);
+    out.did_gen = true;
+}
+
+template <bool NEVER_LOCKSTEP = false, bool BG_SKIP = false, class SRC>
 __device__ __forceinline__ void gen_core(const SRC &cam, const AdvanceParams &ap, int slot_global, SlotState &st,
                                          AdvanceOut &out, int *pxy = nullptr, long long cid_given = -1) {
-    const bool lockstep = NEVER_LOCKSTEP ? false : (ap.lockstep != 0);
-    long long cid = cid_given >= 0 ? cid_given : (long long)st.gen * kW + slot_global;
-    if (cid >= ap.cam_end) {
-        st.bounces = kDone;
+    long long cid;
+    if constexpr (BG_SKIP && std::is_same<SRC, Camera>::value) {
+        int px, py;
+        while (true) {
+            if (!gen_begin<NEVER_LOCKSTEP>(ap, slot_global, st, cid_given, cid)) return;
+            gen_pixel(ap, slot_global, st, pxy, cid_given, cid, px, py);
+            if (!gen_background(ap, px, py)) break;
+            if (!ap.per_sample) {
+                rng_next(st.rs);
+                rng_next(st.rs);
+            }
+            out.bg_skipped++;
+        }
+        gen_camera_ray(cam, ap, cid, px, py, st, out);
         return;
     }
-    if (!lockstep && st.gen == ap.last_gen) {
-        st.bounces = kParked;
-        return;
-    }
-    st.gen = st.gen + 1;
+    if (!gen_begin<NEVER_LOCKSTEP>(ap, slot_global, st, cid_given, cid)) return;
     if constexpr (std::is_same<SRC, KeyedRayTable>::value) {
         const unsigned c = (unsigned)cid;
         const unsigned long long ck = (unsigned long long)c * cam.key_stride;
@@ -398,38 +459,13 @@
         out.did_gen = true;
         return;
     } else {
-    int px, py;
-    if (cid_given >= 0) {
-        st.pixel = (int)((unsigned)cid / (unsigned)ap.spp);
-        py = (int)((unsigned)st.pixel / (unsigned)ap.width);
-        px = st.pixel - py * ap.width;
-    } else if (pxy && ap.dpy >= 0 && *pxy >= 0) {
-        px = (*pxy & 0xffff) + ap.dpx;
-        py = (*pxy >> 16) + ap.dpy;
-        if (px >= ap.width) {
-            px -= ap.width;
-            py++;
-        }
-        st.pixel = py * ap.width + px;
-    } else {
-        if (ap.w_over_spp) st.pixel = (st.gen - 1) * ap.w_over_spp + (int)((unsigned)slot_global / (unsigned)ap.spp);
-        else st.pixel = (int)(cid / ap.spp);
-        py = (int)((unsigned)st.pixel / (unsigned)ap.width);
-        px = st.pixel - py * ap.width;
-    }
-    if (pxy) *pxy = px | (py << 16);
-    if (ap.per_sample) st.rs = rng_sample_stream(ap.seed_lo, ap.seed_hi, (unsigned long long)cid * (unsigned)ap.key_mul + (unsigned)ap.key_add);
-    float jx = rng_uniform(st.rs);
-    float jy = rng_uniform(st.rs);
-    camera_get_ray(cam, (px + jx) / ap.width, (py + jy) / ap.height, out.ray_o, out.ray_d);
-    out.new_ray = true;
-    st.bounces = 0;
-    st.beta = mk(1.f, 1.f, 1.f);
-    out.did_gen = true;
-    }
-}
-
-template <bool DEFER_GEN, bool NEVER_LOCKSTEP = false, bool USE_ACC = false, class SRC>
+        int px, py;
+        gen_pixel(ap, slot_global, st, pxy, cid_given, cid, px, py);
+        gen_camera_ray(cam, ap, cid, px, py, st, out);
+    }
+}
+
+template <bool DEFER_GEN, bool NEVER_LOCKSTEP = false, bool USE_ACC = false, bool BG_SKIP = false, class SRC>
 __device__ __forceinline__ void advance_core(const DScene &sc, const float *tab, const SRC &cam,
                                              const AdvanceParams &ap, int slot_global, SlotState &st, AdvanceOut &out,
                                              float *__restrict__ fb, float *acc = nullptr) {
@@ -438,6 +474,7 @@
     const int off_lpre = tab_off_lpre(sc.num_mats, sc.num_lights);
     out.did_gen = out.did_shade = out.has_shadow = out.did_emit = out.new_ray = out.wants_gen = false;
     out.rr_draws = 0;
+    out.bg_skipped = 0;
     const bool hit = st.hit_info >= 0;
     const int light_of_hit = hit ? ((st.hit_info >> 16) & 0xffff) - 1 : -1;
     RT_MARK("adv.init");
@@ -481,7 +518,7 @@
             return;
         }
         if (USE_ACC) acc_flush(acc, fb, ap.fb_fixed, st.pixel);
-        gen_core<NEVER_LOCKSTEP>(cam, ap, slot_global, st, out);
+        gen_core<NEVER_LOCKSTEP, BG_SKIP>(cam, ap, slot_global, st, out);
         return;
     }
     RT_MARK("adv.mat.sample_f");
@@ -590,6 +627,7 @@
 constexpr int kProfRec = 6;
 #endif
 #define RT_PATHS_CHUNKS 0
+#define RT_PATHS_BG 0
 #define RT_FRAME_SRC Camera
 #define RT_K_ADVANCE k_advance
 #define RT_K_PATHS k_paths
@@ -621,6 +659,25 @@
 #undef RT_K_ADVANCE
 #undef RT_K_PATHS
 #undef RT_PATHS_CHUNKS
+#undef RT_PATHS_BG
+#define RT_PATHS_BG 1
+#define RT_PATHS_CHUNKS 0
+#define RT_FRAME_SRC Camera
+#define RT_K_ADVANCE k_advance_bg_unused
+#define RT_K_PATHS k_paths_bg
+#include "rt_frame_kernels.inc"
+#undef RT_K_ADVANCE
+#undef RT_K_PATHS
+#undef RT_PATHS_CHUNKS
+#define RT_PATHS_CHUNKS 1
+#define RT_K_ADVANCE k_advance_chunked_bg_unused
+#define RT_K_PATHS k_paths_chunked_bg
+#include "rt_frame_kernels.inc"
+#undef RT_FRAME_SRC
+#undef RT_K_ADVANCE
+#undef RT_K_PATHS
+#undef RT_PATHS_CHUNKS
+#undef RT_PATHS_BG
 
 __global__ void k_post_process(float *fb, int n_values, float inv_spp) {
     int i = blockIdx.x * blockDim.x + threadIdx.x;
```

New measurement: 5212 (median of 6 runs). +1.8%, better.
